# gbouritsas/GSN

Hardware: AMD Instinct MI355X
Metric: graphs/sec (orbit-count + GSN-e fwd), ZINC-shape batch; % HBM roofline (higher is better)
Workload: dtype int64 counts + f32 message passing (matrix products: fp16x3 -- two fp16 planes per fp32 operand, three plane products, f32 accumulate); 1 GPU; ZINC-shape x65536 graphs/GPU (N=1521515, E=3116498): integer atom / bond codes in -> cycle_graph k<=6 GSN-e (id_scope=local) orbit count (int64 identifiers written) + one-hot encoding (atoms, bonds and identifiers as exact fp16 operand rows: the layer kernel's input form; no fp32 one-hot tensor is materialised) + GSN_edge_sparse layer-0 forward (general, d_in=28, d_ef=4, d_id=12, d=128, bn, eval) ; inputs=int64 atom codes [N], bond codes [E], edge_index [2, E], graph pointers, outputs=int64 identifiers [E, 4], fp32 layer rows [N, 128], parallelism=graph-shard x1, no data-path collective

## Files before the change

gsn_amd/_abi.py:

```python
from __future__ import annotations

import ctypes
import os
import subprocess

_HERE = os.path.dirname(os.path.abspath(__file__))
LIB_PATH = os.environ.get("GSN_LIB_PATH") or os.path.join(_HERE, "lib", "libgsn_hip.so")
_lib = None

c_i64 = ctypes.c_int64
c_i32 = ctypes.c_int32
c_int = ctypes.c_int
c_vp = ctypes.c_void_p


class GsnError(RuntimeError):
    """A libgsn_hip.so entry point returned a negative status."""


class gsn_block(ctypes.Structure):
    _fields_ = [("data", c_vp), ("idx", c_vp), ("width", c_i64), ("idx32", c_vp)]


class gsn_chain_stage(ctypes.Structure):
    _fields_ = [("blocks", ctypes.POINTER(gsn_block)), ("n_blocks", c_int), ("W", c_vp), ("bias", c_vp), ("n_out", c_i64),
                ("bn_mean", c_vp), ("bn_scale", c_vp), ("bn_shift", c_vp), ("act", c_int)]


class gsn_self_block(ctypes.Structure):
    _fields_ = [("data", c_vp), ("width", c_i64), ("row_stride", c_i64)]


class gsn_pack16(ctypes.Structure):
    _fields_ = [("node_rows", c_vp), ("edge_rows", c_vp)]


class gsn_count_side(ctypes.Structure):
    _fields_ = [("csr_row", c_int), ("seg_ptr", c_vp), ("perm", c_vp), ("sorted_target", c_vp), ("sorted_other", c_vp),
                ("n_nodes", c_i64), ("n_edges", c_i64), ("node_codes", c_vp), ("node_code_cols", c_int), ("node_n_classes", c_int * 4),
                ("node_clamp", c_int), ("node_pack", c_vp), ("edge_codes", c_vp), ("edge_code_cols", c_int), ("edge_n_classes", c_int * 4),
                ("edge_clamp", c_int), ("edge_col0", c_int), ("code_status", c_vp)]


class gsn_count_keys(ctypes.Structure):
    _fields_ = [("nkey", c_vp), ("ekeys", c_vp), ("idmask", c_vp)]


class gsn_count_call(ctypes.Structure):
    _fields_ = [("plan_host", c_vp), ("plan_dev", c_vp), ("plan_words", c_i64), ("n_graphs", c_i64), ("node_ptr", c_vp), ("edge_ptr", c_vp),
                ("edge_index", c_vp), ("edge_row_stride", c_i64), ("ids_are_global", c_int), ("max_nodes", c_i64), ("max_edges", c_i64),
                ("out", c_vp), ("status", c_vp), ("n_classes", c_vp), ("clamp", c_int), ("pack", c_vp), ("pack_stride", c_i64),
                ("pack_col0", c_i64), ("side", ctypes.POINTER(gsn_count_side))]


class gsn_layer_pack16_call(ctypes.Structure):
    _fields_ = [("n_nodes", c_i64), ("n_edges", c_i64), ("seg_ptr", c_vp), ("edge", ctypes.POINTER(gsn_chain_stage)), ("x", c_vp), ("d_x", c_i64),
                ("node0", ctypes.POINTER(gsn_chain_stage)), ("node1", ctypes.POINTER(gsn_chain_stage)), ("prepared", c_vp),
                ("pack", ctypes.POINTER(gsn_pack16)), ("edge_rows", c_i64), ("out", c_vp)]


class gsn_code_slot(ctypes.Structure):
    _fields_ = [("codes", ctypes.c_void_p), ("idx", ctypes.c_void_p), ("stride", ctypes.c_int32), ("col", ctypes.c_int32),
                ("w_off", ctypes.c_int32), ("n_classes", ctypes.c_int32), ("clamp", ctypes.c_int32), ("reserved", ctypes.c_int32)]


class gsn_dgn_agg(ctypes.Structure):
    _fields_ = [("kind", c_i32), ("col", c_i32), ("alpha", ctypes.c_float), ("slot", c_i32)]


SIGNATURES = {
    "gsn_last_error": (ctypes.c_char_p, []),
    "gsn_propagate_last_route": (ctypes.c_char_p, []),
    "gsn_version": (c_int, []),
    "gsn_device_count": (c_int, []),
    "gsn_stream_capture_id": (c_i64, [c_vp]),
    "gsn_fingerprint_hip": (c_int, [c_int, c_vp, c_i64, c_vp, c_vp, c_vp]),
    "gsn_pattern_orbits": (c_int, [c_i64, c_vp, c_int, c_vp, c_vp, c_vp, c_vp, c_vp, c_vp, c_vp, c_vp]),
    "gsn_graph_vertex_orbits": (c_int, [c_i64, c_i64, c_vp, c_vp, c_vp]),
    "gsn_count_plan_build": (c_int, [c_int, c_int, c_int, c_i64, c_vp, c_vp, c_vp, c_i64, c_vp, c_vp]),
    "gsn_count_hip": (c_int, [c_vp, c_vp, c_i64, c_i64, c_vp, c_vp, c_vp, c_i64, c_int, c_vp, c_i64, c_i64, c_i64,
                              c_vp, c_vp, c_vp]),
    "gsn_count_sparse_hip": (c_int, [c_vp, c_vp, c_i64, c_i64, c_vp, c_vp, c_vp, c_i64, c_int, c_vp, c_i64, c_i64, c_i64,
                                     c_vp, c_vp, c_vp, c_i64, c_vp]),
    "gsn_count_sparse_workspace_bytes": (c_i64, [c_i64, c_i64, c_i64]),
    "gsn_count_encode_hip": (c_int, [c_vp, c_vp, c_i64, c_i64, c_vp, c_vp, c_vp, c_i64, c_int, c_vp, c_i64, c_i64, c_i64,
                                     c_vp, c_vp, c_vp, c_int, c_vp, c_vp]),
    "gsn_count_encode_pack16_hip": (c_int, [c_vp, c_vp, c_i64, c_i64, c_vp, c_vp, c_vp, c_i64, c_int, c_vp, c_i64, c_i64, c_i64,
                                            c_vp, c_vp, c_vp, c_int, c_vp, c_vp, c_i64, c_i64, c_vp]),
    "gsn_count_encode_pack16_side_hip": (c_int, [c_vp, c_vp, c_i64, c_i64, c_vp, c_vp, c_vp, c_i64, c_int, c_i64, c_i64, c_vp, c_vp, c_vp, c_int,
                                                 c_vp, c_i64, c_i64, ctypes.POINTER(gsn_count_side), c_vp]),
    "gsn_count_layer_step_hip": (c_int, [ctypes.POINTER(gsn_count_call), ctypes.POINTER(gsn_layer_pack16_call), c_vp, c_vp]),
    "gsn_count_encode_keys_side_hip": (c_int, [c_vp, c_vp, c_i64, c_i64, c_vp, c_vp, c_vp, c_i64, c_int, c_i64, c_i64, c_vp, c_vp, c_vp, c_int,
                                               c_i64, ctypes.POINTER(gsn_count_side), ctypes.POINTER(gsn_count_keys), c_vp]),
    "gsn_count_layer_step_keys_hip": (c_int, [ctypes.POINTER(gsn_count_call), ctypes.POINTER(gsn_layer_pack16_call), ctypes.POINTER(gsn_count_keys),
                                              c_vp, c_i64, c_vp, c_vp]),
    "gsn_layer_keys_byte_table": (c_int, [c_vp]),
    "gsn_pack16_rows_hip": (c_int, [c_vp, c_i64, c_i64, c_vp, c_i64, c_i64, c_i64, c_vp, c_vp]),
    "gsn_one_hot_pack16_hip": (c_int, [c_i64, c_int, c_vp, c_vp, c_int, c_vp, c_i64, c_i64, c_i64, c_vp, c_vp]),
    "gsn_csr_scratch_elems": (c_i64, [c_i64]),
    "gsn_csr_build_hip": (c_int, [c_i64, c_i64, c_vp, c_vp, c_vp, c_vp, c_vp, c_vp, c_vp, c_vp]),
    "gsn_linear_f16x3_kpad": (c_i64, [c_i64]),
    "gsn_linear_f16x3_mpad": (c_i64, [c_i64]),
    "gsn_linear_f16x3_scratch_bytes": (c_i64, [c_i64, c_i64]),
    "gsn_linear_f16x3_prepare_hip": (c_int, [c_vp, c_i64, c_i64, c_vp, c_vp, c_vp]),
    "gsn_linear_f16x3_prepare_strided_hip": (c_int, [c_vp, c_i64, c_i64, c_i64, c_i64, c_vp, c_vp, c_vp]),
    "gsn_linear_fwd_strided_hip": (c_int, [c_i64, c_int, ctypes.POINTER(gsn_block), c_vp, c_i64, c_i64, c_vp, c_i64, c_vp, c_vp, c_vp, c_int,
                                           c_vp, c_vp, c_vp]),
    "gsn_linear_splitk_plan": (c_int, [c_i64, c_i64, c_i64]),
    "gsn_linear_fwd_splitk_hip": (c_int, [c_i64, c_int, ctypes.POINTER(gsn_block), c_vp, c_i64, c_i64, c_vp, c_i64, c_vp, c_vp]),
    "gsn_linear_f16x3_fwd_hip": (c_int, [c_i64, c_int, c_vp, c_vp, c_vp, c_vp, c_i64, c_vp, c_vp, c_vp, c_int, c_vp, c_vp, c_vp]),
    "gsn_linear_f16x3_fwd_stats_hip": (c_int, [c_i64, c_int, c_vp, c_vp, c_vp, c_vp, c_i64, c_vp, c_vp, c_vp, c_vp]),
    "gsn_linear_f16x3_split_rows_hip": (c_int, [c_i64, c_int, c_vp, c_vp, c_vp]),
    "gsn_linear_f16x3_fwd_presplit_hip": (c_int, [c_i64, c_int, c_vp, c_vp, c_vp, c_vp, c_i64, c_vp, c_vp, c_vp, c_int, c_vp, c_vp, c_vp]),
    "gsn_wgrad_f16x3_hip": (c_int, [c_i64, c_i64, c_i64, c_vp, c_vp, c_vp, c_vp]),
    "gsn_linear_f16x3_fwd_stats_presplit_hip": (c_int, [c_i64, c_int, c_vp, c_vp, c_vp, c_vp, c_i64, c_vp, c_vp, c_vp, c_vp]),
    "gsn_bn_act_planes_hip": (c_int, [c_i64, c_i64, c_vp, c_vp, c_vp, c_vp, c_int, c_vp, c_vp, c_vp]),
    "gsn_edge_split_sum_hip": (c_int, [c_i64, c_i64, c_vp, c_vp, c_vp, c_vp, c_vp, c_i64, c_vp, c_i64, c_vp, c_i64, c_vp, c_i64, c_int, c_vp, c_vp]),
    "gsn_csr_build_graphs_hip": (c_int, [c_i64, c_vp, c_vp, c_i64, c_i64, c_i64, c_i64, c_vp, c_vp, c_vp, c_vp, c_vp, c_vp, c_vp, c_vp]),
    "gsn_segsum_prepare_hip": (c_int, [c_i64, c_i64, c_vp, c_vp, c_i64, c_vp, c_vp]),
    "gsn_segment_sum_rows_hip": (c_int, [c_i64, c_i64, c_vp, c_vp, c_vp, c_vp, c_vp, c_i64, c_i64, c_vp, c_vp]),
    "gsn_propagate_fwd_hip": (c_int, [c_int, c_i64, c_i64, c_vp, c_vp, c_vp, c_vp, c_vp, c_i64, c_vp, c_i64, c_int, c_vp,
                                      c_i64, c_vp, c_vp]),
    "gsn_propagate_bwd_hip": (c_int, [c_int, c_i64, c_i64, c_vp, c_vp, c_vp, c_vp, c_vp, c_i64, c_vp, c_i64, c_int,
                                      c_vp, c_i64, c_vp, c_vp, c_vp, c_vp, c_vp]),
    "gsn_propagate_self_fwd_hip": (c_int, [c_int, c_i64, c_i64, c_vp, c_vp, c_vp, c_vp, c_vp, c_i64, c_vp, c_i64, c_int, c_vp,
                                           c_i64, c_i64, c_i64, c_int, ctypes.POINTER(gsn_self_block), c_vp, c_vp, c_vp]),
    "gsn_add_gathered_hip": (c_int, [c_i64, c_i64, c_vp, c_vp, c_vp, c_i64, c_vp, c_vp]),
    "gsn_propagate_self_bwd_hip": (c_int, [c_int, c_i64, c_i64, c_vp, c_int, ctypes.POINTER(gsn_self_block), ctypes.POINTER(c_vp), c_vp, c_vp,
                                           c_vp, c_vp]),
    "gsn_propagate_pad_bwd_hip": (c_int, [c_int, c_i64, c_i64, c_vp, c_vp, c_vp, c_vp, c_vp, c_i64, c_vp, c_i64, c_int,
                                          c_vp, c_i64, c_i64, c_i64, c_vp, c_vp, c_vp, c_vp, c_vp]),
    "gsn_propagate_bwd_fold_self_hip": (c_int, [c_i64, c_i64, c_vp, c_vp, c_vp, c_vp, c_vp, c_i64, c_vp, c_i64, c_vp, c_i64, c_vp, c_vp, c_vp, c_vp,
                                                c_vp, c_vp, c_vp]),
    "gsn_linear_fwd_hip": (c_int, [c_i64, c_int, ctypes.POINTER(gsn_block), c_vp, c_vp, c_i64, c_vp, c_vp, c_vp, c_int,
                                   c_vp, c_vp, c_vp, c_vp]),
    "gsn_one_hot_hip": (c_int, [c_i64, c_int, c_vp, c_vp, c_int, c_vp, c_vp]),
    "gsn_column_range_hip": (c_int, [c_i64, c_int, c_vp, c_vp, c_vp, c_vp]),
    "gsn_column_ranks_hip": (c_int, [c_i64, c_int, c_vp, c_vp, c_vp, c_i64, c_vp, c_vp, c_vp, c_vp]),
    "gsn_unique_sort_scratch_bytes": (c_i64, [c_i64, c_i64]),
    "gsn_unique_sort_hip": (c_int, [c_i64, c_i64, c_vp, c_vp, c_vp, c_vp, c_vp, c_i64, c_vp]),
    "gsn_lookup_codes_hip": (c_int, [c_i64, c_i64, c_vp, c_vp, c_vp, c_int, c_vp, c_vp, c_vp, c_vp]),
    "gsn_embed_fwd_hip": (c_int, [c_i64, c_int, c_int, c_int, c_vp, c_vp, c_vp, c_vp, c_vp, c_vp]),
    "gsn_embed_bwd_hip": (c_int, [c_i64, c_int, c_int, c_int, c_vp, c_vp, c_vp, c_vp, c_vp]),
    "gsn_embed_bwd_flat_supported": (c_int, [c_i64, c_int, c_int, c_vp]),
    "gsn_embed_bwd_flat_hip": (c_int, [c_i64, c_int, c_int, c_int, c_vp, c_vp, c_vp, c_vp, c_vp, c_vp]),
    "gsn_code_stage_supported": (c_int, [c_int, c_i64, c_i64]),
    "gsn_code_stage_fwd_hip": (c_int, [c_i64, c_int, ctypes.POINTER(gsn_code_slot), c_vp, c_i64, c_vp, c_i64, c_vp, c_vp, c_vp,
                                       c_int, c_vp, c_vp, c_vp, c_vp, c_vp]),
    "gsn_bn_act_hip": (c_int, [c_i64, c_i64, c_vp, c_vp, c_vp, c_vp, c_int, c_vp, c_vp]),
    "gsn_bn_act_bwd_hip": (c_int, [c_i64, c_i64, c_vp, c_vp, c_vp, c_vp, c_vp, c_vp, c_int, c_int, c_vp, c_vp, c_vp, c_vp]),
    "gsn_fold_weights_fwd_hip": (c_int, [c_i64, c_i64, c_i64, c_i64, c_i64, c_vp, c_i64, c_vp, c_i64, c_vp, c_vp, c_vp]),
    "gsn_fold_weights_bwd_hip": (c_int, [c_i64, c_i64, c_i64, c_i64, c_vp, c_i64, c_vp, c_i64, c_vp, c_i64, c_vp, c_vp, c_vp, c_vp, c_vp]),
    "gsn_bn_act_bwd_from_h_hip": (c_int, [c_i64, c_i64, c_vp, c_vp, c_vp, c_vp, c_vp, c_vp, c_int, c_int, c_vp, c_vp, c_vp, c_vp]),
    "gsn_bn_act_bwd_planes_hip": (c_int, [c_i64, c_i64, c_vp, c_vp, c_vp, c_vp, c_vp, c_vp, c_int, c_int, c_vp, c_vp, c_vp, c_vp]),
    "gsn_wgrad_hip": (c_int, [c_i64, c_i64, c_vp, c_int, ctypes.POINTER(gsn_block), c_vp, c_vp]),
    "gsn_gather_cat_hip": (c_int, [c_i64, c_int, ctypes.POINTER(gsn_block), c_vp, c_vp]),
    "gsn_bn_finalize_hip": (c_int, [c_i64, c_i64, ctypes.c_double, ctypes.c_double, c_vp, c_vp, c_vp, c_vp, c_vp, c_vp, c_vp, c_vp, c_vp, c_vp]),
    "gsn_bn_finalize_act_hip": (c_int, [c_i64, c_i64, ctypes.c_double, ctypes.c_double, c_vp, c_vp, c_vp, c_vp, c_vp, c_vp, c_vp, c_vp, c_vp, c_vp,
                                        c_vp, c_int, c_vp, c_vp]),
    "gsn_bn_finalize_count_hip": (c_int, [c_i64, c_i64, ctypes.c_double, ctypes.c_double, c_vp, c_vp, c_vp, c_vp, c_vp, c_vp, c_vp, c_vp, c_vp, c_vp,
                                          c_vp]),
    "gsn_column_stats_hip": (c_int, [c_i64, c_i64, c_vp, c_vp, c_vp]),
    "gsn_mlp_chain_supported": (c_int, [c_int, ctypes.POINTER(gsn_chain_stage)]),
    "gsn_layer_fused_supported": (c_int, [ctypes.POINTER(gsn_chain_stage), c_i64, ctypes.POINTER(gsn_chain_stage), ctypes.POINTER(gsn_chain_stage)]),
    "gsn_layer_fused_prepared_bytes": (c_i64, [ctypes.POINTER(gsn_chain_stage), c_i64, ctypes.POINTER(gsn_chain_stage), ctypes.POINTER(gsn_chain_stage)]),
    "gsn_layer_fused_prepare_hip": (c_int, [ctypes.POINTER(gsn_chain_stage), c_i64, ctypes.POINTER(gsn_chain_stage), ctypes.POINTER(gsn_chain_stage),
                                            c_vp, c_vp]),
    "gsn_layer_fused_fwd_hip": (c_int, [c_i64, c_i64, c_vp, ctypes.POINTER(gsn_chain_stage), c_vp, c_i64, ctypes.POINTER(gsn_chain_stage),
                                        ctypes.POINTER(gsn_chain_stage), c_vp, c_vp, c_vp]),
    "gsn_layer_fused_pack16_supported": (c_int, [ctypes.POINTER(gsn_chain_stage), c_i64, ctypes.POINTER(gsn_chain_stage), ctypes.POINTER(gsn_chain_stage)]),
    "gsn_layer_fused_pack16_prepared_bytes": (c_i64, [ctypes.POINTER(gsn_chain_stage), c_i64, ctypes.POINTER(gsn_chain_stage), ctypes.POINTER(gsn_chain_stage)]),
    "gsn_layer_fused_pack16_prepare_hip": (c_int, [ctypes.POINTER(gsn_chain_stage), c_i64, ctypes.POINTER(gsn_chain_stage), ctypes.POINTER(gsn_chain_stage), c_vp, c_vp]),
    "gsn_layer_fused_fwd_pack16_hip": (c_int, [c_i64, c_i64, c_vp, ctypes.POINTER(gsn_chain_stage), c_vp, c_i64, ctypes.POINTER(gsn_chain_stage), ctypes.POINTER(gsn_chain_stage), c_vp, ctypes.POINTER(gsn_pack16), c_i64, c_vp, c_vp]),
    "gsn_layer_fused_workspace_bytes": (c_i64, [c_i64, ctypes.POINTER(gsn_chain_stage), c_i64, ctypes.POINTER(gsn_chain_stage), ctypes.POINTER(gsn_chain_stage)]),
    "gsn_layer_fused_fwd_ws_hip": (c_int, [c_i64, c_i64, c_vp, ctypes.POINTER(gsn_chain_stage), c_vp, c_i64, ctypes.POINTER(gsn_chain_stage),
                                           ctypes.POINTER(gsn_chain_stage), c_vp, c_vp, c_vp, c_i64, c_vp, c_vp, c_vp]),
    "gsn_layer_fused_graphs_supported": (c_int, [ctypes.POINTER(gsn_chain_stage), c_i64, ctypes.POINTER(gsn_chain_stage), ctypes.POINTER(gsn_chain_stage)]),
    "gsn_layer_fused_fwd_graphs_hip": (c_int, [c_i64, c_i64, c_vp, ctypes.POINTER(gsn_chain_stage), c_vp, c_i64, ctypes.POINTER(gsn_chain_stage),
                                               ctypes.POINTER(gsn_chain_stage), c_vp, c_i64, c_vp, c_i64, c_vp, c_vp]),
    "gsn_mlp_chain_fwd_hip": (c_int, [c_i64, c_int, ctypes.POINTER(gsn_chain_stage), c_vp, c_vp, c_vp, c_vp, c_vp]),
    "gsn_dgn_aggregate_fwd_hip": (c_int, [c_i64, c_i64, c_i64, c_vp, c_vp, c_vp, c_vp, c_vp, c_i64, c_i64, c_vp, c_i64, c_i64,
                                          ctypes.POINTER(gsn_dgn_agg), c_int, c_vp, c_int, ctypes.c_double, c_vp, c_vp]),
    "gsn_dgn_aggregate_bwd_hip": (c_int, [c_i64, c_i64, c_i64, c_vp, c_vp, c_vp, c_vp, c_vp, c_vp, c_vp, c_i64, c_i64, c_vp, c_i64,
                                          c_i64, ctypes.POINTER(gsn_dgn_agg), c_int, c_vp, c_int, ctypes.c_double, c_vp, c_vp, c_vp, c_vp]),
    "gsn_laplacian_eig_hip": (c_int, [c_i64, c_vp, c_vp, c_vp, c_i64, c_vp, c_i64, c_int, c_int, c_int, c_int, c_vp, c_vp, c_vp, c_vp, c_vp,
                                      c_i64, c_vp]),
    "gsn_laplacian_eig_scratch_floats": (c_i64, [c_int, c_i64]),
    "gsn_adam_step_hip": (c_int, [c_int, c_vp, c_i64, c_vp, c_int, c_vp, c_vp, c_vp, c_vp, c_vp, c_i64, c_vp]),
    "gsn_masked_loss_scratch_bytes": (c_i64, [c_int, c_i64, c_i64]),
    "gsn_masked_loss_fwd_hip": (c_int, [c_int, c_i64, c_i64, c_vp, c_vp, c_vp, c_vp, c_vp, c_i64, c_vp]),
    "gsn_masked_loss_bwd_hip": (c_int, [c_int, c_i64, c_i64, c_vp, c_vp, c_vp, c_vp, c_vp, c_vp]),
    "gsn_eval_accumulate_scratch_bytes": (c_i64, [c_int, c_i64, c_i64]),
    "gsn_eval_accumulate_hip": (c_int, [c_int, c_int, c_i64, c_i64, c_i64, c_vp, c_vp, c_i64, c_vp, c_vp, c_vp, c_vp, c_i64, c_vp, c_vp, c_i64, c_vp]),
    "gsn_rank_metrics_scratch_bytes": (c_i64, [c_i64, c_i64]),
    "gsn_rank_metrics_hip": (c_int, [c_i64, c_i64, c_vp, c_vp, c_vp, c_vp, c_vp, c_vp, c_i64, c_vp]),
}


def build(verbose: bool = False) -> str:
    cmd = ["make", "-C", os.path.join(_HERE, "csrc"), "-j8"]
    res = subprocess.run(cmd, stdout=subprocess.PIPE, stderr=subprocess.STDOUT, text=True)
    if res.returncode != 0:
        raise RuntimeError("building libgsn_hip.so failed:\n" + res.stdout)
    if verbose:
        print(res.stdout)
    return LIB_PATH


def lib():
    global _lib
    if _lib is None:
        if not os.path.exists(LIB_PATH):
            raise ImportError(
                "gsn_amd: %s not found. Build the HIP extension first (python -c 'import __graft_entry__ as g; "
                "g.build()' or make -C gsn_amd/csrc). There is no CPU fallback." % LIB_PATH)
        import torch
        handle = ctypes.CDLL(LIB_PATH)
        for name, (res, args) in SIGNATURES.items():
            fn = getattr(handle, name)
            fn.restype = res
            fn.argtypes = args
        if handle.gsn_version() != 1:
            raise ImportError("gsn_amd: libgsn_hip.so ABI version %d != 1" % handle.gsn_version())
        _lib = handle
    return _lib


def check(rc: int, what: str = "") -> None:
    if rc != 0:
        msg = lib().gsn_last_error()
        raise GsnError("%s failed (%d): %s" % (what or "libgsn_hip", rc, msg.decode() if msg else ""))


_GPU_SEEN = False


def require_gpu() -> None:
    global _GPU_SEEN
    if _GPU_SEEN:
        return
    import torch
    if not torch.cuda.is_available():
        raise RuntimeError("gsn_amd: no GPU visible to PyTorch-ROCm; the counting / message-passing kernels are "
                           "HIP-only (gfx950) and there is no CPU fallback.")
    _GPU_SEEN = True


def ptr(t) -> int:
    if t is None:
        return None
    if hasattr(t, "data_ptr"):
        return t.data_ptr()
    return t.ctypes.data


def current_stream() -> int:
    import torch
    return torch._C._cuda_getCurrentRawStream(torch._C._cuda_getDevice())


class _NullGuard:
    def __enter__(self):
        return self

    def __exit__(self, *exc):
        return False


_NULL_GUARD = _NullGuard()


def device_guard(device):
    import torch
    idx = device.index
    if idx is None or idx == torch._C._cuda_getDevice():
        return _NULL_GUARD
    return torch.cuda.device(device)
```

gsn_amd/_dense.py:

```python
from __future__ import annotations

import ctypes
import os

import torch

from . import _abi, flags
from ._caches import _note_cache
from ._runtime import _ACT_CODE, _MAX_BLOCKS, _f32c, _timed, _zeros



def _f16x3_weights(weight, w32):
    key = (weight._version, w32.data_ptr(), tuple(w32.shape))
    hit = getattr(weight, "_gsn_f16x3", None)
    if hit is not None and hit[0] == key:
        return hit[1], hit[2]
    n_out, k = w32.shape
    L = _abi.lib()
    kpad = int(L.gsn_linear_f16x3_kpad(k))
    planes = torch.empty(2 * n_out * kpad, dtype=torch.float16, device=w32.device)
    col_inv = torch.empty(n_out, dtype=torch.float32, device=w32.device)
    with _abi.device_guard(w32.device):
        if w32.is_contiguous():
            _abi.check(L.gsn_linear_f16x3_prepare_hip(w32.data_ptr(), n_out, k, planes.data_ptr(), col_inv.data_ptr(), _abi.current_stream()),
                       "gsn_linear_f16x3_prepare_hip")
        else:
            _abi.check(L.gsn_linear_f16x3_prepare_strided_hip(w32.data_ptr(), n_out, k, w32.stride(0), w32.stride(1), planes.data_ptr(), col_inv.data_ptr(),
                                                              _abi.current_stream()), "gsn_linear_f16x3_prepare_strided_hip")
    try:
        weight._gsn_f16x3 = (key, planes, col_inv)
        _note_cache(weight, "_gsn_f16x3")
    except (AttributeError, RuntimeError):
        pass
    return planes, col_inv


def _block_array(blocks, keep, widths_only=False):
    arr = (_abi.gsn_block * max(len(blocks), 1))()
    for b, (d, idx) in enumerate(blocks):
        arr[b].width = d.shape[1]
        if widths_only:
            arr[b].data = 1
            continue
        d = _f32c(d); keep.append(d)
        arr[b].data = d.data_ptr()
        arr[b].idx = None; arr[b].idx32 = None
        if idx is not None:
            idx = idx.contiguous(); keep.append(idx)
            if idx.dtype == torch.int32:
                arr[b].idx32 = idx.data_ptr()
            else:
                arr[b].idx = idx.data_ptr()
    keep.append(arr)
    return arr


def _f16x3_takes(m_rows, n_out, widths, aligned=True, direct=True, out=True, stats=False, bn=False, act=0):
    return (flags.LINEAR_F16X3 and out and (not stats or (flags.LINEAR_F16X3_STATS and not bn and act == 0 and n_out % 4 == 0))
            and m_rows > 0 and n_out > flags.LINEAR_F16X3_MIN_N and ((m_rows + 127) // 128) * ((n_out + 127) // 128) > flags.LINEAR_F16X3_MIN_TILES
            and direct and aligned and all(w % 4 == 0 for w in widths))


def _linear_hip(blocks, weight, bias, bn_mean, bn_scale, bn_shift, act, m_rows, out=True, stats=None, split_k=False, scratch_out=None, presplit=None):
    if len(blocks) > _MAX_BLOCKS:
        raise NotImplementedError("more than %d input blocks" % _MAX_BLOCKS)
    dev = weight.device
    keep = []
    arr = _block_array(blocks, keep)
    n_out = weight.shape[0]
    y = torch.empty((m_rows, n_out), dtype=torch.float32, device=dev) if out else None
    if m_rows == 0:
        return y
    w_view = (weight.dim() == 2 and weight.dtype is torch.float32 and not weight.is_contiguous() and weight.stride(0) == 1
              and weight.stride(1) >= weight.shape[0] and flags.STRIDED_WEIGHTS)
    w = (weight.detach() if weight.requires_grad else weight) if w_view else _f32c(weight)
    vecs = [None if v is None else _f32c(v) for v in (bias, bn_mean, bn_scale, bn_shift)]
    nb = len(blocks)
    takes16 = _f16x3_takes(m_rows, n_out, [d.shape[1] for d, _ in blocks], aligned=all((arr[i].data or 0) % 16 == 0 for i in range(nb)),
                           direct=all(idx is None for _, idx in blocks), out=out, stats=stats is not None, bn=bn_mean is not None, act=act)
    if presplit is not None and not takes16:
        raise RuntimeError("presplit rows given to a product that does not run on the fp16x3 kernel (_f16x3_takes decides)")
    if takes16:
        planes, col_inv = _f16x3_weights(weight, w)
        scratch = presplit if presplit is not None else torch.empty(int(_abi.lib().gsn_linear_f16x3_scratch_bytes(m_rows, w.shape[1])), dtype=torch.uint8, device=dev)
        name = "gsn_linear_f16x3_fwd%s%s_hip" % ("_stats" if stats is not None else "", "_presplit" if presplit is not None else "")
        epilogue = () if stats is not None else (_abi.ptr(vecs[1]), _abi.ptr(vecs[2]), _abi.ptr(vecs[3]), act)
        tail = () if stats is None else (stats.data_ptr(),)
        with _abi.device_guard(dev), _timed("linear_fwd", 2.0 * m_rows * w.shape[1] * n_out):
            rc = getattr(_abi.lib(), name)(m_rows, nb, arr, planes.data_ptr(), col_inv.data_ptr(), _abi.ptr(vecs[0]), n_out, *epilogue,
                                           scratch.data_ptr(), y.data_ptr(), *tail, _abi.current_stream())
        _abi.check(rc, name)
        if scratch_out is not None:
            scratch_out.append(scratch)
        return y
    if split_k and out and stats is None and act == 0 and bn_mean is None and bn_scale is None and flags.LINEAR_SPLITK:
        splits = int(_abi.lib().gsn_linear_splitk_plan(m_rows, w.shape[1], n_out))
        if splits > 1:
            y = _zeros(m_rows * n_out, torch.float32, dev).view(m_rows, n_out)
            with _abi.device_guard(dev), _timed("linear_fwd", 2.0 * m_rows * w.shape[1] * n_out):
                rc = _abi.lib().gsn_linear_fwd_splitk_hip(m_rows, len(blocks), arr, w.data_ptr(), w.stride(0) if w_view else 0, w.stride(1) if w_view else 0,
                                                          _abi.ptr(vecs[0]), n_out, y.data_ptr(), _abi.current_stream())
            _abi.check(rc, "gsn_linear_fwd_splitk_hip")
            return y
    if w_view:
        with _abi.device_guard(dev), _timed("linear_fwd", 2.0 * m_rows * w.shape[1] * n_out):
            rc = _abi.lib().gsn_linear_fwd_strided_hip(m_rows, len(blocks), arr, w.data_ptr(), w.stride(0), w.stride(1), _abi.ptr(vecs[0]), n_out,
                                                       _abi.ptr(vecs[1]), _abi.ptr(vecs[2]), _abi.ptr(vecs[3]), act, _abi.ptr(y), _abi.ptr(stats),
                                                       _abi.current_stream())
        if rc != -2:
            _abi.check(rc, "gsn_linear_fwd_strided_hip")
            return y
        w = w.contiguous()
    with _abi.device_guard(dev), _timed("linear_fwd", 2.0 * m_rows * w.shape[1] * n_out):
        rc = _abi.lib().gsn_linear_fwd_hip(m_rows, len(blocks), arr, w.data_ptr(), _abi.ptr(vecs[0]), n_out, _abi.ptr(vecs[1]),
                                           _abi.ptr(vecs[2]), _abi.ptr(vecs[3]), act, None, _abi.ptr(y), _abi.ptr(stats),
                                           _abi.current_stream())
    _abi.check(rc, "gsn_linear_fwd_hip")
    return y


class _Stage:
    __slots__ = ("blocks", "weight", "bias", "bn", "act", "bn_params", "bn_invstd")

    def __init__(self, weight, bias, bn=None, act="identity", blocks=()):
        self.blocks, self.weight, self.bias, self.bn, self.act = list(blocks), weight, bias, bn, act
        self.bn_params = None
        self.bn_invstd = None


def _launch_stages(stages, m_rows, stats=None, csr=None):
    L = _abi.lib()
    dev = stages[0].weight.device
    if m_rows == 0:
        n_last = stages[-1].weight.shape[0]
        if csr is not None:
            return torch.zeros((csr.seg_ptr.numel() - 1, n_last), dtype=torch.float32, device=dev)
        return torch.empty((0, n_last), dtype=torch.float32, device=dev) if stats is None else None
    y = None
    i = 0
    while i < len(stages):
        group = None
        for n in (2, 1):
            cand = stages[i:i + n]
            if len(cand) < n:
                continue
            carry = [(y, None)] if y is not None else []
            arr = (_abi.gsn_chain_stage * n)()
            keep = []
            for j, st in enumerate(cand):
                arr[j] = _stage_struct(st, st.blocks + carry if j == 0 else st.blocks, keep)
            if L.gsn_mlp_chain_supported(n, arr):
                group = (n, arr, keep, cand)
                break
        last_group = group is not None and i + group[0] == len(stages)
        if csr is not None and not (last_group and i == 0):
            return None
        if group is not None:
            n, arr, keep, cand = group
            want_stats = stats is not None and last_group
            n_out = cand[-1].weight.shape[0]
            seg = csr is not None and not want_stats
            if seg:
                n_seg = csr.seg_ptr.numel() - 1
                out = torch.empty((n_seg, n_out), dtype=torch.float32, device=dev)
                with _abi.device_guard(dev), _timed("segsum_prepare"):
                    _abi.check(L.gsn_segsum_prepare_hip(n_seg, m_rows, csr.seg_ptr.data_ptr(), csr.tgt.data_ptr(), n_out,
                                                        out.data_ptr(), _abi.current_stream()), "gsn_segsum_prepare_hip")
            else:
                out = None if want_stats else torch.empty((m_rows, n_out), dtype=torch.float32, device=dev)
            flops = sum(2.0 * m_rows * st.weight.shape[1] * st.weight.shape[0] for st in cand)
            with _abi.device_guard(dev), _timed("mlp_chain%d" % n, flops):
                rc = L.gsn_mlp_chain_fwd_hip(m_rows, n, arr, None,
                                             csr.tgt.data_ptr() if seg else None, _abi.ptr(out),
                                             _abi.ptr(stats) if want_stats else None, _abi.current_stream())
            _abi.check(rc, "gsn_mlp_chain_fwd_hip")
            y = out
            i += n
        else:
            st = stages[i]
            blks = st.blocks + ([(y, None)] if y is not None else [])
            last = i == len(stages) - 1
            bp = st.bn_params or (None, None, None)
            if last and stats is not None:
                _linear_hip(blks, st.weight, st.bias, None, None, None, 0, m_rows, out=False, stats=stats)
                y = None
            else:
                y = _linear_hip(blks, st.weight, st.bias, bp[0], bp[1], bp[2], _ACT_CODE[st.act], m_rows)
            i += 1
    return y


def _chain_fits(stages):
    n = len(stages)
    if n < 1 or n > 2:
        return False
    arr = (_abi.gsn_chain_stage * n)()
    keep = []
    for j, st in enumerate(stages):
        arr[j].blocks = _block_array(st.blocks, keep, widths_only=True); arr[j].n_blocks = len(st.blocks)
        arr[j].W = 1; arr[j].n_out = st.weight.shape[0]; arr[j].act = _ACT_CODE[st.act]
    return bool(_abi.lib().gsn_mlp_chain_supported(n, arr))


def _stage_struct(st, blocks, keep, rows_keep=None):
    g = _abi.gsn_chain_stage()
    g.blocks = _block_array(blocks, keep if rows_keep is None else rows_keep); g.n_blocks = len(blocks)
    w = _f32c(st.weight); keep.append(w)
    g.W = w.data_ptr(); g.n_out = w.shape[0]
    vecs = [None if v is None else _f32c(v) for v in ((st.bias,) + (st.bn_params or (None, None, None)))]
    keep.extend(vecs)
    g.bias, g.bn_mean, g.bn_scale, g.bn_shift = [_abi.ptr(v) for v in vecs]
    g.act = _ACT_CODE[st.act]
    return g


def _prep_key(st):
    bn = st.bn
    bk = None
    if bn is not None:
        bk = (bn.running_mean._version, bn.running_var._version, bn.running_mean.data_ptr(),
              (bn.weight._version, bn.bias._version) if bn.affine else None)
    return (st.weight.data_ptr(), st.weight._version, tuple(st.weight.shape), bk)


def _prepared(kind, ge, g0, g1, d_x, dev, owner=None, attr=None, key=None):
    hit = getattr(owner, attr, None) if owner is not None else None
    if hit is not None and hit[0] == key:
        return hit[1]
    L = _abi.lib()
    nbytes = int(getattr(L, "gsn_layer_fused%s_prepared_bytes" % kind)(ctypes.byref(ge), d_x, ctypes.byref(g0), ctypes.byref(g1)))
    prep = torch.empty(nbytes // 4, dtype=torch.int32, device=dev)
    name = "gsn_layer_fused%s_prepare_hip" % kind
    with _abi.device_guard(dev):
        _abi.check(getattr(L, name)(ctypes.byref(ge), d_x, ctypes.byref(g0), ctypes.byref(g1), prep.data_ptr(), _abi.current_stream()), name)
    if owner is not None:
        setattr(owner, attr, (key, prep))
        _note_cache(owner, attr)
    return prep


def _layer_fused(x, csr, edge_stages, node_stages, training, owner=None, gen=0, pack16=None, pack_only=False, record=None):
    if not flags.FUSED_LAYER or len(edge_stages) != 1 or len(node_stages) != 2:
        return None
    stages = edge_stages + node_stages
    for st in stages:
        if st.act not in ("identity", "relu"):
            return None
        if st.bn is not None and (training or st.bn.training or st.bn.running_mean is None):
            return None
    if x.data_ptr() % 16:
        return None
    if len(node_stages[0].blocks) != 1 or node_stages[1].blocks:
        return None
    for st in stages:
        _bn_resolve(st, None, 0, False)
    keep, rows = [], []
    eb = edge_stages[0].blocks
    ge = _stage_struct(edge_stages[0], eb, keep, rows)
    g0 = _stage_struct(node_stages[0], [], keep)
    g1 = _stage_struct(node_stages[1], [], keep)
    d_x = x.shape[1]
    if node_stages[0].weight.shape[1] != d_x + edge_stages[0].weight.shape[0] + 4:
        return None
    L = _abi.lib()
    fl = (2.0 * edge_stages[0].weight.shape[1] * edge_stages[0].weight.shape[0],
          2.0 * (node_stages[0].weight.shape[1] * node_stages[0].weight.shape[0] + node_stages[1].weight.shape[1] * node_stages[1].weight.shape[0]))
    pkey = (tuple(_prep_key(st) for st in stages), d_x, gen)
    if pack16 is not None and flags.PACK16_LAYER and L.gsn_layer_fused_pack16_supported(ctypes.byref(ge), d_x, ctypes.byref(g0), ctypes.byref(g1)):
        prep = _prepared("_pack16", ge, g0, g1, d_x, x.device, owner, "_fused_prep16", pkey + ("pack16",))
        launch16 = _pack16_launch(ge, g0, g1, d_x, prep, fl, keep)
        out = launch16(x.data_ptr(), x.shape[0], x.device, csr, [idx for _, idx in eb], pack16)
        if out is not None:
            if record is not None and owner is not None and all(idx is not None and idx.dtype == torch.int32 for _, idx in eb):
                owner._fplan = (record, "pack16", launch16)
                _note_cache(owner, "_fplan")
            return out
    if pack_only:
        return None
    if not L.gsn_layer_fused_supported(ctypes.byref(ge), d_x, ctypes.byref(g0), ctypes.byref(g1)):
        return None
    nbytes = int(L.gsn_layer_fused_prepared_bytes(ctypes.byref(ge), d_x, ctypes.byref(g0), ctypes.byref(g1)))
    prep = _prepared("", ge, g0, g1, d_x, x.device, owner, "_fused_prep", pkey + (nbytes,))
    if (flags.GRAPH_ALIGNED_LAYER and getattr(csr, "part", None) is not None and d_x == 128
            and L.gsn_layer_fused_graphs_supported(ctypes.byref(ge), d_x, ctypes.byref(g0), ctypes.byref(g1))):
        launch_g = _graphs_launch(ge, g0, g1, d_x, prep, fl, keep)
        out = launch_g(x, csr, eb)
        if out is not None:
            if (record is not None and owner is not None
                    and all(idx is not None and idx.dtype == torch.int32 and d.dtype == torch.float32 and d.is_contiguous() for d, idx in eb)):
                owner._fplan = (record, "graphs", launch_g)
                _note_cache(owner, "_fplan")
            return out
    return _rows_forward(x, csr, ge, g0, g1, d_x, prep, fl)


def _pack16_launch(ge, g0, g1, d_x, prep, fl, keep):
    L = _abi.lib()
    n_out = g1.n_out
    pk = _abi.gsn_pack16()

    def launch16(x_ptr, n_rows, dev, csr_now, idx_now, pack_now):
        for i in range(ge.n_blocks):
            ge.blocks[i].data = x_ptr if i < 2 else pack_now[1].data_ptr()
            ge.blocks[i].idx32 = idx_now[i].data_ptr()
        y = torch.empty((n_rows, n_out), dtype=torch.float32, device=dev)
        pk.node_rows = pack_now[0].data_ptr()
        pk.edge_rows = None if pack_now[1] is None else pack_now[1].data_ptr()
        e_now = csr_now.tgt.numel()
        with _abi.device_guard(dev), _timed("layer_fused", fl[0] * e_now + fl[1] * n_rows):
            rc16 = L.gsn_layer_fused_fwd_pack16_hip(n_rows, e_now, csr_now.seg_ptr.data_ptr(), ctypes.byref(ge), x_ptr, d_x, ctypes.byref(g0), ctypes.byref(g1),
                                                    prep.data_ptr(), ctypes.byref(pk), 0 if pack_now[1] is None else pack_now[1].shape[0], y.data_ptr(),
                                                    _abi.current_stream())
        if rc16 == -2:
            return None
        _abi.check(rc16, "gsn_layer_fused_fwd_pack16_hip")
        return y
    launch16._keep = keep
    return launch16


def _graphs_launch(ge, g0, g1, d_x, prep, fl, keep):
    L = _abi.lib()
    n_out = g1.n_out

    def launch_g(x_now, csr_now, blocks_now, y=None):
        part_now = getattr(csr_now, "part", None)
        if part_now is None or part_now[2] > 128 or int(part_now[0].numel()) <= 1 or x_now.data_ptr() % 16:
            return None
        for i in range(ge.n_blocks):
            d_i, idx_i = blocks_now[i]
            ge.blocks[i].data = d_i.data_ptr()
            ge.blocks[i].idx = None
            ge.blocks[i].idx32 = idx_i.data_ptr()
        n_now, e_now = x_now.shape[0], csr_now.tgt.numel()
        if y is None:
            y = torch.empty((n_now, n_out), dtype=torch.float32, device=x_now.device)
        with _abi.device_guard(x_now.device), _timed("layer_fused", fl[0] * e_now + fl[1] * n_now):
            rcg = L.gsn_layer_fused_fwd_graphs_hip(n_now, e_now, csr_now.seg_ptr.data_ptr(), ctypes.byref(ge), x_now.data_ptr(), d_x, ctypes.byref(g0),
                                                   ctypes.byref(g1), prep.data_ptr(), int(part_now[0].numel()) - 1, part_now[0].data_ptr(), int(part_now[2]),
                                                   y.data_ptr(), _abi.current_stream())
        if rcg == -2:
            return None
        _abi.check(rcg, "gsn_layer_fused_fwd_graphs_hip")
        return y
    launch_g._keep = keep
    return launch_g


def _rows_forward(x, csr, ge, g0, g1, d_x, prep, fl):
    L = _abi.lib()
    n, E = x.shape[0], csr.tgt.numel()
    out = torch.empty((n, g1.n_out), dtype=torch.float32, device=x.device)
    x_exp = None
    hit = getattr(x, "_gsn_row_exp", None)
    if hit is not None and hit[1] == x._version and hit[0].numel() == n and hit[0].device == x.device and not flags.VALIDATE_CACHES:
        x_exp = hit[0]
    out_exp = torch.empty(n, dtype=torch.int32, device=x.device) if d_x == 128 and out.shape[1] == 128 and flags.CHAIN_ROW_EXPONENTS else None
    ws_bytes = 0 if x_exp is not None else int(L.gsn_layer_fused_workspace_bytes(n, ctypes.byref(ge), d_x, ctypes.byref(g0), ctypes.byref(g1)))
    ws = torch.empty(ws_bytes // 4, dtype=torch.int32, device=x.device) if ws_bytes else None
    with _abi.device_guard(x.device), _timed("layer_fused", fl[0] * E + fl[1] * n):
        rc = L.gsn_layer_fused_fwd_ws_hip(n, E, csr.seg_ptr.data_ptr(), ctypes.byref(ge), x.data_ptr(), d_x, ctypes.byref(g0),
                                          ctypes.byref(g1), prep.data_ptr(), out.data_ptr(), _abi.ptr(ws), ws_bytes, _abi.ptr(x_exp),
                                          _abi.ptr(out_exp), _abi.current_stream())
    if rc == 0 and out_exp is not None:
        out._gsn_row_exp = (out_exp, out._version)
    if rc == -2:
        if os.environ.get("GSN_CHAIN_TRACE"):
            import sys
            msg = L.gsn_last_error()
            print("gsn chain: one-launch layer declined: %s" % (msg.decode() if msg else ""), file=sys.stderr)
        return None
    _abi.check(rc, "gsn_layer_fused_fwd_hip")
    return out


def _bn_resolve(stage, stats_fn, m_rows, training, fuse_act=None):
    bn = stage.bn
    if bn is None:
        stage.bn_params = None
        return
    if training or bn.running_mean is None:
        if training and m_rows == 1:
            raise ValueError("Expected more than 1 value per channel when training, got input size torch.Size([%d, %d])" % (m_rows, bn.num_features))
        if m_rows == 0:
            n_out, dev = bn.num_features, stage.weight.device
            if training and bn.track_running_stats and bn.num_batches_tracked is not None:
                bn.num_batches_tracked += 1
                if flags.RAW_WRITTEN is not None:
                    flags.RAW_WRITTEN.append(bn.num_batches_tracked)
            vec = torch.zeros((4, n_out), dtype=torch.float32, device=dev)
            vec[1:3] = 1.0
            stage.bn_params = (vec[0], vec[2], vec[3])
            stage.bn_invstd = vec[1]
            return
        stats = stats_fn()
        n_out = stats.shape[1]
        dev = stats.device
        vec = torch.empty((4, n_out), dtype=torch.float32, device=dev)
        track = training and bn.track_running_stats and bn.running_mean is not None
        mom = 0.0
        nbt = None
        if track:
            if bn.momentum is not None and bn.num_batches_tracked.is_cuda and bn.num_batches_tracked.dtype == torch.int64:
                mom, nbt = bn.momentum, bn.num_batches_tracked
            else:
                bn.num_batches_tracked += 1
                mom = bn.momentum if bn.momentum is not None else 1.0 / float(bn.num_batches_tracked)
        gamma = _f32c(bn.weight) if bn.affine else None
        beta = _f32c(bn.bias) if bn.affine else None
        v0, v1, v2, v3 = vec.unbind(0)
        p0 = vec.data_ptr()
        with _abi.device_guard(dev):
            if fuse_act is not None:
                fh, fact, fout = fuse_act
                rc = _abi.lib().gsn_bn_finalize_act_hip(n_out, m_rows, float(bn.eps), float(mom), stats.data_ptr(), _abi.ptr(gamma), _abi.ptr(beta),
                                                        bn.running_mean.data_ptr() if track else None, bn.running_var.data_ptr() if track else None,
                                                        p0, p0 + 4 * n_out, p0 + 8 * n_out, p0 + 12 * n_out, _abi.ptr(nbt),
                                                        fh.data_ptr(), int(fact), fout.data_ptr(), _abi.current_stream())
            else:
                rc = _abi.lib().gsn_bn_finalize_count_hip(n_out, m_rows, float(bn.eps), float(mom), stats.data_ptr(), _abi.ptr(gamma), _abi.ptr(beta),
                                                          bn.running_mean.data_ptr() if track else None, bn.running_var.data_ptr() if track else None,
                                                          p0, p0 + 4 * n_out, p0 + 8 * n_out, p0 + 12 * n_out,
                                                          _abi.ptr(nbt), _abi.current_stream())
        _abi.check(rc, "gsn_bn_finalize_act_hip" if fuse_act is not None else "gsn_bn_finalize_count_hip")
        if track:
            touched = [bn.running_mean, bn.running_var] + ([nbt] if nbt is not None else [])
            torch.autograd.graph.increment_version(touched)
            if flags.RAW_WRITTEN is not None:
                flags.RAW_WRITTEN.extend(touched)
        stage.bn_params = (v0, v2, v3)
        stage.bn_invstd = v1
        return
    else:
        key = (bn.running_mean._version, bn.running_var._version, bn.running_mean.data_ptr(), bn.running_var.data_ptr(),
               (bn.weight._version, bn.bias._version, bn.weight.data_ptr(), bn.bias.data_ptr()) if bn.affine else None)
        hit = getattr(bn, "_gsn_eval_cache", None)
        if hit is not None and hit[0] == key:
            stage.bn_params = hit[1]
            stage.bn_invstd = hit[2]
            return
        mean32 = bn.running_mean
        invstd = torch.rsqrt(bn.running_var.to(torch.float64) + bn.eps).to(torch.float32)
        scale = invstd * bn.weight.detach() if bn.affine else invstd
        shift = bn.bias.detach() if bn.affine else torch.zeros_like(invstd)
        stage.bn_params = (mean32.contiguous(), scale.contiguous(), shift.contiguous())
        stage.bn_invstd = invstd.contiguous()
        bn._gsn_eval_cache = (key, stage.bn_params, stage.bn_invstd)
        _note_cache(bn, "_gsn_eval_cache")


def run_stages(stages, m_rows, training, csr=None):
    if csr is not None and not _chain_fits(stages):
        return None
    needs_stats = any(st.bn is not None and (training or st.bn.running_mean is None) for st in stages)
    if csr is None and needs_stats and not _chain_fits(stages):
        return _run_stages_materialised(stages, m_rows, training)
    for i, st in enumerate(stages):
        if st.bn is not None:
            def stats_fn(i=i):
                n_out = stages[i].weight.shape[0]
                stats = _zeros(2 * n_out, torch.float64, stages[i].weight.device).view(2, n_out)
                probe = _Stage(stages[i].weight, stages[i].bias, None, "identity", stages[i].blocks)
                _launch_stages(stages[:i] + [probe], m_rows, stats=stats)
                return stats
            _bn_resolve(st, stats_fn, m_rows, training)
    return _launch_stages(stages, m_rows, csr=csr)


def _bn_act_hip(h, bn_params, act):
    vecs = [None if v is None else _f32c(v) for v in (bn_params or (None, None, None))]
    with _abi.device_guard(h.device), _timed("bn_act", 8.0 * h.numel()):
        rc = _abi.lib().gsn_bn_act_hip(h.shape[0], h.shape[1], h.data_ptr(), _abi.ptr(vecs[0]), _abi.ptr(vecs[1]), _abi.ptr(vecs[2]),
                                       _ACT_CODE[act], h.data_ptr(), _abi.current_stream())
    _abi.check(rc, "gsn_bn_act_hip")
    return h


def _run_stages_materialised(stages, m_rows, training):
    y = None
    for st in stages:
        blks = st.blocks + ([(y, None)] if y is not None else [])
        if st.bn is not None and (training or st.bn.running_mean is None):
            n_out = st.weight.shape[0]
            stats = _zeros(2 * n_out, torch.float64, st.weight.device).view(2, n_out)
            h = _linear_hip(blks, st.weight, st.bias, None, None, None, 0, m_rows, out=True, stats=stats)
            _bn_resolve(st, lambda: stats, m_rows, training)
            y = _bn_act_hip(h, st.bn_params, st.act)
        else:
            _bn_resolve(st, None, m_rows, training)
            bp = st.bn_params or (None, None, None)
            y = _linear_hip(blks, st.weight, st.bias, bp[0], bp[1], bp[2], _ACT_CODE[st.act], m_rows)
    return y
```

gsn_amd/csrc/abi.cpp:

```cpp
#include <hip/hip_runtime.h>

#include <cstring>

#include "gsn_internal.h"
#include "layer_rr.h"

namespace gsn {

static thread_local char g_err[512] = "";

int set_error(int code, const char *fmt, ...) {
    va_list ap;
    va_start(ap, fmt);
    vsnprintf(g_err, sizeof(g_err), fmt, ap);
    va_end(ap);
    return code;
}

}

extern "C" const char *gsn_last_error(void) { return gsn::g_err; }

extern "C" int gsn_version(void) { return GSN_ABI_VERSION; }

extern "C" int gsn_device_count(void) {
    int n = 0;
    if (hipGetDeviceCount(&n) != hipSuccess) {
        (void)hipGetLastError();
        return 0;
    }
    int good = 0;
    for (int i = 0; i < n; ++i) {
        hipDeviceProp_t p;
        if (hipGetDeviceProperties(&p, i) == hipSuccess && std::strncmp(p.gcnArchName, "gfx950", 6) == 0) ++good;
    }
    return good;
}

extern "C" int64_t gsn_stream_capture_id(void *stream) {
    hipStreamCaptureStatus st = hipStreamCaptureStatusNone;
    unsigned long long id = 0;
    if (hipStreamGetCaptureInfo(reinterpret_cast<hipStream_t>(stream), &st, &id) != hipSuccess) {
        (void)hipGetLastError();
        return 0;
    }
    if (st == hipStreamCaptureStatusNone) return 0;
    return (int64_t)(id ? id : 1);
}

namespace gsn {
int current_device() {
    int dev = -1;
    if (hipGetDevice(&dev) != hipSuccess) return -1;
    return dev;
}

int lds_limit(DeviceOnce *once, std::initializer_list<const void *> kernels, const char *label, int bytes) {
    const int dev = once ? current_device() : -1;
    if (once && once->done(dev)) return GSN_OK;
    char sized[32];
    if (!label) { snprintf(sized, sizeof(sized), "%d B LDS", bytes); label = sized; }
    for (const void *k : kernels) {
        const hipError_t e = hipFuncSetAttribute(k, hipFuncAttributeMaxDynamicSharedMemorySize, bytes);
        if (e != hipSuccess) return set_error(GSN_E_HIP, "hipFuncSetAttribute(%s): %s", label, hipGetErrorString(e));
    }
    if (once) once->mark(dev);
    return GSN_OK;
}

int launch_check(const char *label_fmt, ...) {
    const hipError_t e = hipGetLastError();
    if (e == hipSuccess) return GSN_OK;
    char label[256];
    va_list ap;
    va_start(ap, label_fmt);
    vsnprintf(label, sizeof(label), label_fmt, ap);
    va_end(ap);
    return set_error(GSN_E_HIP, "%s: %s", label, hipGetErrorString(e));
}

void trace(const char *fmt, ...) {
    if (!sw_present(SW_CHAIN_TRACE)) return;
    va_list ap;
    va_start(ap, fmt);
    vfprintf(stderr, fmt, ap);
    va_end(ap);
}

ProfCounters::ProfCounters(size_t n, void *stream) {
    n_ = n;
    if (n == 0 || hipMalloc(&dev_, n * sizeof(unsigned long long)) != hipSuccess) { dev_ = nullptr; return; }
    (void)hipMemsetAsync(dev_, 0, n * sizeof(unsigned long long), reinterpret_cast<hipStream_t>(stream));
}
ProfCounters::~ProfCounters() { if (dev_) (void)hipFree(dev_); }
std::vector<unsigned long long> ProfCounters::fetch(void *stream) {
    std::vector<unsigned long long> h(n_, 0ull);
    (void)hipStreamSynchronize(reinterpret_cast<hipStream_t>(stream));
    if (dev_) {
        (void)hipMemcpy(h.data(), dev_, n_ * sizeof(unsigned long long), hipMemcpyDeviceToHost);
        (void)hipFree(dev_);
        dev_ = nullptr;
    }
    return h;
}
}

extern "C" int gsn_count_layer_step_hip(const gsn_count_call *c, const gsn_layer_pack16_call *l, void *event_between, void *stream) {
    if (!c || !l) return gsn::set_error(GSN_E_INVALID, "gsn_count_layer_step_hip: null call struct");
    const int rc = gsn_count_encode_pack16_side_hip(c->plan_host, c->plan_dev, c->plan_words, c->n_graphs, c->node_ptr, c->edge_ptr, c->edge_index,
                                                    c->edge_row_stride, c->ids_are_global, c->max_nodes, c->max_edges, c->out, c->status, c->n_classes,
                                                    c->clamp, c->pack, c->pack_stride, c->pack_col0, c->side, stream);
    if (rc != GSN_OK) return rc;
    if (event_between && hipEventRecord(reinterpret_cast<hipEvent_t>(event_between), reinterpret_cast<hipStream_t>(stream)) != hipSuccess)
        return gsn::set_error(GSN_E_HIP, "gsn_count_layer_step_hip: hipEventRecord(event_between)");
    return gsn_layer_fused_fwd_pack16_hip(l->n_nodes, l->n_edges, l->seg_ptr, l->edge, l->x, l->d_x, l->node0, l->node1, l->prepared, l->pack,
                                          l->edge_rows, l->out, stream);
}

extern "C" int gsn_count_layer_step_keys_hip(const gsn_count_call *c, const gsn_layer_pack16_call *l, const gsn_count_keys *keys, const uint16_t *node_dict,
                                             int64_t dict_rows, void *event_between, void *stream) {
    if (!c || !l || !keys || !c->side) return gsn::set_error(GSN_E_INVALID, "gsn_count_layer_step_keys_hip: null call struct / keys / side");
    if (!keys->nkey || !keys->ekeys || !keys->idmask || !node_dict) return gsn::set_error(GSN_E_INVALID, "gsn_count_layer_step_keys_hip: null key array / node dictionary");
    if (!c->side->node_codes || !c->side->edge_codes) return gsn::set_error(GSN_E_INVALID, "gsn_count_layer_step_keys_hip: node and edge codes are both needed");
    if (!gsn_layer_fused_pack16_supported(l->edge, l->d_x, l->node0, l->node1))
        return gsn::set_error(GSN_E_UNSUPPORTED, "gsn_count_layer_step_keys_hip: shape outside the packed-row layer kernel");
    if (!l->seg_ptr || !l->out || !l->prepared || (reinterpret_cast<uintptr_t>(l->prepared) & 15) || l->n_nodes <= 0 || l->n_nodes > (int64_t)2000000000 ||
        l->n_edges > (int64_t)2000000000)
        return gsn::set_error(GSN_E_INVALID, "gsn_count_layer_step_keys_hip: null seg_ptr / out / prepared (16-byte aligned), or sizes outside 32-bit row arithmetic");
    if (l->edge->n_blocks < 3 || l->edge->blocks[0].idx32 != c->side->sorted_target || l->edge->blocks[1].idx32 != c->side->sorted_other ||
        l->edge->blocks[2].idx32 != c->side->perm || l->seg_ptr != c->side->seg_ptr || l->n_edges != c->side->n_edges || l->n_nodes != c->side->n_nodes)
        return gsn::set_error(GSN_E_INVALID, "gsn_count_layer_step_keys_hip: the layer's seg_ptr / block indices must be the counting launch's CSR arrays");
    int rc = gsn_count_encode_keys_side_hip(c->plan_host, c->plan_dev, c->plan_words, c->n_graphs, c->node_ptr, c->edge_ptr, c->edge_index, c->edge_row_stride,
                                            c->ids_are_global, c->max_nodes, c->max_edges, c->out, c->status, c->n_classes, c->clamp, c->pack_col0, c->side, keys, stream);
    if (rc != GSN_OK) return rc;
    if (event_between && hipEventRecord(reinterpret_cast<hipEvent_t>(event_between), reinterpret_cast<hipStream_t>(stream)) != hipSuccess)
        return gsn::set_error(GSN_E_HIP, "gsn_count_layer_step_keys_hip: hipEventRecord(event_between)");
    const gsn::RpKeys k{keys->ekeys, keys->nkey, keys->idmask, node_dict, dict_rows, c->side->edge_col0};
    rc = gsn::rp_forward(l->n_nodes, l->n_edges, l->seg_ptr, l->edge, l->x, l->d_x, l->node0, l->node1, l->prepared, nullptr, l->edge_rows, l->out,
                         reinterpret_cast<hipStream_t>(stream), &k);
    if (rc == 1) return gsn::set_error(GSN_E_UNSUPPORTED, "gsn_count_layer_step_keys_hip: key arrays beyond 2 GiB (32-bit buffer offsets)");
    return rc;
}
```

gsn_amd/csrc/layer_rp.hip:

```cpp
#include <hip/hip_runtime.h>

#include <cstdint>
#include <cstdio>
#include <cstdlib>
#include <type_traits>
#include <vector>

#include "chain_common.h"
#include "layer_rr.h"
#include "layer_rr_inl.h"
#include "layer_rr_core.h"

namespace gsn {

struct RpArgs {
    int n_nodes, n_edges;
    const int32_t *seg_ptr;
    const int32_t *role_idx[3];
    const uint16_t *node16, *edge16;
    unsigned node_bytes, edge_bytes;
    int edge_shift;
    int d_x;
    float *out;
    const unsigned *prep;
    int n_ranges;
    int n_split;
    const uint32_t *ekeys;
    const uint8_t *nkey;
    int edge_col0;
};

struct RpIdx { int r[3]; int pt, pt1; int nk; };

template <bool KEYS>
__device__ __forceinline__ void rp_idx_load(const RpArgs &a, const RrDesc &d, int li, RpIdx &ix) {
    const int ne = d.ne();
    if (d.valid() && ne > 0) {
        const int e = d.e0 + (li < ne ? li : ne - 1);
        if constexpr (KEYS) {
            ix.r[0] = (int)a.ekeys[e];
            ix.r[2] = a.role_idx[2][e];
        } else {
#pragma unroll
            for (int q = 0; q < 3; ++q) ix.r[q] = a.role_idx[q][e];
        }
    }
    if (d.valid()) {
        int t = d.m0 + li;
        t = t < a.n_nodes ? t : a.n_nodes - 1;
        ix.pt = a.seg_ptr[t];
        ix.pt1 = a.seg_ptr[t + 1];
        if constexpr (KEYS) ix.nk = (int)a.nkey[t];
    }
}

constexpr int RP_BYTE_TAB_BYTES = 256 * 16;
__device__ __host__ __forceinline__ unsigned rp_byte_tab_word(unsigned b, int q) {
    return ((b >> (2 * q)) & 1u ? 0x3c00u : 0u) | ((b >> (2 * q + 1)) & 1u ? 0x3c000000u : 0u);
}

#define RP_LOAD(RS, VOFF, IMM) __builtin_bit_cast(rr_u4, __builtin_amdgcn_raw_buffer_load_b128(RS, (int)((VOFF) + (IMM)), 0, 0))

__device__ __forceinline__ unsigned rp_scale_pair(unsigned pair, float s) {
    unsigned r;
    asm("v_fma_mixlo_f16 %0, %1, %2, 0 op_sel_hi:[1,0,0]" : "=v"(r) : "v"(pair), "v"(s));
    asm("v_fma_mixhi_f16 %0, %1, %2, 0 op_sel:[1,0,0] op_sel_hi:[1,0,0]" : "+v"(r) : "v"(pair), "v"(s));
    return r;
}
__device__ __forceinline__ unsigned rp_hi_lo_word(float a, float s) {
    unsigned r;
    asm("v_fma_mixlo_f16 %0, %1, %2, 0" : "=v"(r) : "v"(a), "v"(s));
    asm("v_fma_mixhi_f16 %0, %1, %2, -%0 op_sel_hi:[0,0,1]" : "+v"(r) : "v"(a), "v"(s));
    return r;
}
__device__ __forceinline__ unsigned rp_pk_max_u16(unsigned a, unsigned b) { unsigned r; asm("v_pk_max_u16 %0, %1, %2" : "=v"(r) : "v"(a), "v"(b)); return r; }

#ifndef RP_GATHER_AT
#define RP_GATHER_AT 3
#endif
#ifndef RP_STORE_AUX
#define RP_STORE_AUX 2
#endif
#ifndef RP_PD
#define RP_PD 8
#endif
#ifndef RP_STAGGER
#define RP_STAGGER 0
#endif
#ifndef RP_S1T
#define RP_S1T 0
#endif
#ifndef RP_DRAIN
#define RP_DRAIN 0
#endif
#ifndef RP_S1E
#define RP_S1E 1
#endif

template <int WB, int NKX, bool PROF, bool KEYS = false>
__global__ __launch_bounds__(64 * RR_NW) __attribute__((amdgpu_waves_per_eu(RR_NW / 4, RR_NW / 4))) void layer_fused_kernel_rp(RpArgs a, unsigned long long *prof) {
    auto clk = [&]() -> unsigned {
        if (!PROF) return 0u;
        __builtin_amdgcn_sched_barrier(0);
        const unsigned v = (unsigned)__builtin_amdgcn_s_memtime();
        __builtin_amdgcn_sched_barrier(0);
        return v;
    };
    unsigned pc[8] = {0, 0, 0, 0, 0, 0, 0, 0};
    using SH = RrShape<WB, NKX>;
    constexpr int NKS = SH::NKS, NK0 = SH::NK0;
    static_assert(WB == 4 && NKX == 2, "two pairs of feature blocks; the node pack is two chunks wide");
    extern __shared__ __attribute__((aligned(16))) unsigned char smem[];

    const int tid = threadIdx.x;
    const int lane0 = tid & 63, wave = __builtin_amdgcn_readfirstlane(tid >> 6);
    const int li0 = lane0 & 31, lh0 = lane0 >> 5;
    unsigned ldsb[3];
    ldsb[0] = (unsigned)(uintptr_t)(__attribute__((address_space(3))) unsigned char *)smem + 16u * (unsigned)lane0;
    ldsb[1] = ldsb[0] + 0x10000u; ldsb[2] = ldsb[0] + 0x20000u;
    asm volatile("" : "+v"(ldsb[1]), "+v"(ldsb[2]));

    {
        const rr_u4 *src = reinterpret_cast<const rr_u4 *>(a.prep + RR_HDR);
        rr_u4 *dst = reinterpret_cast<rr_u4 *>(smem);
        for (int i = tid; i < SH::F_LDS * 64; i += 64 * RR_NW) dst[i] = src[i];
        const float *tsrc = reinterpret_cast<const float *>(a.prep + RR_HDR + SH::F_ALL * 256);
        float *tdst = reinterpret_cast<float *>(smem + SH::F_LDS * 1024);
        for (int i = tid; i < SH::TAB_WORDS; i += 64 * RR_NW) tdst[i] = tsrc[i];
        if constexpr (KEYS) {
            rr_u4 *bt = reinterpret_cast<rr_u4 *>(smem + SH::LDS_BYTES);
            for (int b = tid; b < 256; b += 64 * RR_NW) bt[b] = rr_u4{rp_byte_tab_word(b, 0), rp_byte_tab_word(b, 1), rp_byte_tab_word(b, 2), rp_byte_tab_word(b, 3)};
        }
    }
    __syncthreads();
    auto hdr = [&](int i) { return (int)__builtin_amdgcn_readfirstlane(a.prep[i]); };
    const int Ee = hdr(RRH_EE), E0 = hdr(RRH_E0), E1 = hdr(RRH_E1), e_min = hdr(RRH_EMIN);
    const bool w_bad = hdr(RRH_BAD) != 0;
    if (a.prep[RRH_PACK] != 1u) __builtin_trap();
    const unsigned acts = (unsigned)hdr(RRH_ACT);
    const int lo_e = __builtin_amdgcn_readfirstlane((acts & 1) ? 0 : (int)0x80000000), lo_0 = __builtin_amdgcn_readfirstlane((acts & 2) ? 0 : (int)0x80000000);
    const int lo_1 = __builtin_amdgcn_readfirstlane((acts & 4) ? 0 : (int)0x80000000);
    const __amdgpu_buffer_rsrc_t wstream = __builtin_amdgcn_make_buffer_rsrc(const_cast<unsigned *>(a.prep) + RR_HDR + SH::F_W0SL * 256, 0, NKS * WB * 1024, 0x00020000);
    const __amdgpu_buffer_rsrc_t rs_n = __builtin_amdgcn_make_buffer_rsrc(const_cast<uint16_t *>(a.node16), 0, (int)a.node_bytes, 0x00020000);
    const __amdgpu_buffer_rsrc_t rs_e = __builtin_amdgcn_make_buffer_rsrc(const_cast<uint16_t *>(a.edge16), 0, (int)a.edge_bytes, 0x00020000);
    const int esh = a.edge_shift;
    int sbase[8];
#pragma unroll
    for (int k = 0; k < 8; ++k) { sbase[k] = 4096 * k; asm volatile("" : "+s"(sbase[k])); }
    const int ec0 = a.edge_col0;
    const int deg_c = a.d_x >> 4, deg_h = (a.d_x >> 3) & 1, deg_w = (a.d_x >> 1) & 3;

    const int range = wave * (int)gridDim.x + (int)blockIdx.x;
    if (range >= a.n_ranges) return;
    const unsigned long long wave_t0 = PROF ? __builtin_amdgcn_s_memrealtime() : 0ull;
#if RP_STAGGER > 0
    if (wave >= RR_NW / 2) {
#pragma unroll 1
        for (int i = 0; i < RP_STAGGER; ++i) __builtin_amdgcn_s_sleep(64);
    }
#endif
    RrIter it;
    it.seg = a.seg_ptr; it.n_nodes = a.n_nodes;
    {
        const int half_n = a.n_ranges >> 1;
        if (a.n_split > 0 && half_n > 0 && (a.n_ranges & 1) == 0 && (int)gridDim.x * (RR_NW / 2) == half_n) {
            const int young = wave >= RR_NW / 2 ? 1 : 0;
            const int idx = range - young * half_n;
            const int64_t base = young ? a.n_split : 0, cnt = young ? a.n_nodes - a.n_split : a.n_split;
            it.m_next = (int)(base + cnt * idx / half_n);
            it.m_end = (int)(base + cnt * (idx + 1) / half_n);
        } else {
            it.m_next = (int)((int64_t)a.n_nodes * range / a.n_ranges);
            it.m_end = (int)((int64_t)a.n_nodes * (range + 1) / a.n_ranges);
        }
    }
    it.m0 = 0; it.nn = 0; it.eb = 0; it.ee = 0; it.ec = 0; it.pending = 0; it.win = 0;
    rr_iter_load(it, lane0);
    RrDesc cur = rr_iter_next(it, lane0);
    RpIdx ixc, ixn;
#pragma unroll
    for (int q = 0; q < 3; ++q) { ixc.r[q] = 0; ixn.r[q] = 0; }
    ixc.pt = ixc.pt1 = ixn.pt = ixn.pt1 = 0;
    ixc.nk = ixn.nk = 0;
    rp_idx_load<KEYS>(a, cur, li0, ixc);
    RrDesc nxt = rr_iter_next(it, lane0);
    rp_idx_load<KEYS>(a, nxt, li0, ixn);
    rr_u4 gA[RR_NKE], gB[RR_NKE];
    auto gather = [&](rr_u4 (&g)[RR_NKE], const int (&r)[3], int lh) {
        if constexpr (KEYS) {
            const unsigned k = (unsigned)r[0];
            const unsigned vt = ((k & 0xffu) << 6) | ((unsigned)lh << 4), vs = (((k >> 8) & 0xffu) << 6) | ((unsigned)lh << 4);
            g[0] = RP_LOAD(rs_n, vt, 0); g[1] = RP_LOAD(rs_n, vt, 32);
            g[2] = RP_LOAD(rs_n, vs, 0); g[3] = RP_LOAD(rs_n, vs, 32);
            g[4][0] = (unsigned)__builtin_amdgcn_raw_buffer_load_b16(rs_e, (int)((unsigned)r[2] << 1), 0, 0);
        } else {
        const unsigned vt = ((unsigned)r[0] << 6) | ((unsigned)lh << 4), vs = ((unsigned)r[1] << 6) | ((unsigned)lh << 4);
        const unsigned ve = ((unsigned)r[2] << esh) | ((unsigned)lh << 4);
        g[0] = RP_LOAD(rs_n, vt, 0); g[1] = RP_LOAD(rs_n, vt, 32);
        g[2] = RP_LOAD(rs_n, vs, 0); g[3] = RP_LOAD(rs_n, vs, 32);
        g[4] = RP_LOAD(rs_e, ve, 0);
        }
    };
    gather(gA, ixc.r, lh0);
    int pt = ixc.pt, pt1 = ixc.pt1;
    int nk = ixc.nk;
    unsigned kc = (unsigned)ixc.r[0];

    const unsigned t_start = clk();
    while (cur.valid()) {
        asm volatile("" : "+v"(ldsb[0]), "+v"(ldsb[1]), "+v"(ldsb[2]));
        int li = li0, lh = lh0;
        asm volatile("" : "+v"(li), "+v"(lh));
        const int lane = li + 32 * lh;
        const float *tab = reinterpret_cast<const float *>(rr_lds_generic(ldsb[0] - 16u * (unsigned)lane + SH::F_LDS * 1024));
        const int m0 = cur.m0, nn = cur.nn();
        rr_u4 X[NKX];
        auto load_x = [&]() {
            const unsigned vx = ((unsigned)(KEYS ? nk : m0 + (li < nn ? li : nn - 1)) << 6) | ((unsigned)lh << 4);
#pragma unroll
            for (int c = 0; c < NKX; ++c) X[c] = RP_LOAD(rs_n, vx, 32 * c);
        };
        f32x16 sacc[WB];
        int tpt = 0, tpt1 = 0;
        int rnext[3] = {0, 0, 0};
        auto block = [&](auto first_c, rr_u4 (&gc)[RR_NKE], rr_u4 (&gn)[RR_NKE]) __attribute__((always_inline)) -> bool {
            constexpr bool FIRST = decltype(first_c)::value;
            const unsigned t0 = clk();
            const int ne = cur.ne();
            if (li >= nn) { pt = 0; pt1 = 0; }
            tpt = pt; tpt1 = pt1;
            rr_u4 Ah[RR_NKE];
#pragma unroll
            for (int c = 0; c < RR_NKE; ++c) Ah[c] = gc[c];
            if constexpr (KEYS) {
                const unsigned m16 = gc[RR_NKE - 1][0] | ((kc >> 16) << ec0);
                const unsigned byte = (m16 >> (8 * lh)) & 0xffu;
                Ah[RR_NKE - 1] = *reinterpret_cast<rr_ldsp>(ldsb[2] - 16u * (unsigned)lane + 16u * byte + (unsigned)(SH::LDS_BYTES - 0x20000));
            }
            const bool last = cur.last() != 0;
            if (!last) gather(gn, ixn.r, lh);
#pragma unroll
            for (int q = 0; q < 3; ++q) rnext[q] = ixn.r[q];
            kc = (unsigned)ixn.r[0];
            const int npt = ixn.pt, npt1 = ixn.pt1, nnk = ixn.nk;
            const RrDesc nn2 = rr_iter_next(it, lane);
            rp_idx_load<KEYS>(a, nn2, li, ixn);
            const unsigned t1 = clk();
            unsigned t2 = t1;
            if (!FIRST || ne > 0) {
                const unsigned bm = rr_edge_mask(pt, pt1, cur.e0);
                rr_u4 M[2];
                rr_incidence(bm, lh, M);
                auto frag4 = [&](int fp, int c, rr_u4 &h0, rr_u4 &l0, rr_u4 &h1, rr_u4 &l1) {
                    h0 = rr_lds_frag(ldsb, SH::F_WE + 2 * (fp * RR_NKE + c)); l0 = rr_lds_frag(ldsb, SH::F_WE + 2 * (fp * RR_NKE + c) + 1);
                    h1 = rr_lds_frag(ldsb, SH::F_WE + 2 * ((fp + 1) * RR_NKE + c)); l1 = rr_lds_frag(ldsb, SH::F_WE + 2 * ((fp + 1) * RR_NKE + c) + 1);
                };
                auto ep_half = [&](const f32x16 &acc, int h, unsigned (&yh)[8], unsigned (&yl)[8]) {
#pragma unroll
                    for (int q = 0; q < 2; ++q) {
                        const int r = 8 * h + 4 * q;
                        rr_split4(rr_imax(acc[r], lo_e), rr_imax(acc[r + 1], lo_e), rr_imax(acc[r + 2], lo_e), rr_imax(acc[r + 3], lo_e),
                                  yh[4 * h + 2 * q], yl[4 * h + 2 * q], yh[4 * h + 2 * q + 1], yl[4 * h + 2 * q + 1]);
                    }
                };
                auto incid = [&](f32x16 &sv, const unsigned (&yh)[8], const unsigned (&yl)[8], const rr_u4 (&MM)[2], int h) {
                    const rr_u4 pl = rr_u4{yl[4 * h], yl[4 * h + 1], yl[4 * h + 2], yl[4 * h + 3]};
                    const rr_u4 ph = rr_u4{yh[4 * h], yh[4 * h + 1], yh[4 * h + 2], yh[4 * h + 3]};
                    if (FIRST && h == 0) {
                        f32x16 z;
#pragma unroll
                        for (int r = 0; r < 16; ++r) z[r] = 0.f;
                        RR_MFH(pl, MM[h], z);
                        sv = z;
                    } else {
                        RR_MFH(pl, MM[h], sv);
                    }
                    RR_MFH(ph, MM[h], sv);
                };
                unsigned yh0[8], yl0[8], yh1[8], yl1[8];
                auto ep_step = [&](int c, const f32x16 &A0, const f32x16 &A1, f32x16 &S0, f32x16 &S1, const rr_u4 (&MM)[2]) {
                    if (c == 0) ep_half(A0, 0, yh0, yl0);
                    if (c == 1) { ep_half(A0, 1, yh0, yl0); incid(S0, yh0, yl0, MM, 0); }
                    if (c == 2) { ep_half(A1, 0, yh1, yl1); incid(S0, yh0, yl0, MM, 1); }
                    if (c == 3) { ep_half(A1, 1, yh1, yl1); incid(S1, yh1, yl1, MM, 0); }
                    if (c == 4) incid(S1, yh1, yl1, MM, 1);
                };
                auto products = [&](int fp, f32x16 &acc0, f32x16 &acc1, auto &&under) {
#pragma unroll
                    for (int r = 0; r < 16; ++r) { acc0[r] = 0.f; acc1[r] = 0.f; }
                    rr_u4 f0h, f0l, f1h, f1l;
                    frag4(fp, 0, f0h, f0l, f1h, f1l);
#pragma unroll
                    for (int c = 0; c < RR_NKE; ++c) {
                        rr_u4 n0h = f0h, n0l = f0l, n1h = f1h, n1l = f1l;
                        if (c + 1 < RR_NKE) frag4(fp, c + 1, n0h, n0l, n1h, n1l);
                        RR_MFH(Ah[c], f0l, acc0);
                        RR_MFH(Ah[c], f1l, acc1);
                        under(c);
                        RR_MFH(Ah[c], f0h, acc0);
                        RR_MFH(Ah[c], f1h, acc1);
                        RR_SB();
                        f0h = n0h; f0l = n0l; f1h = n1h; f1l = n1l;
                    }
                };
                f32x16 qa0, qa1, ra0, ra1;
                products(0, qa0, qa1, [&](int) {});
                products(2, ra0, ra1, [&](int c) { ep_step(c, qa0, qa1, sacc[0], sacc[1], M); });
                t2 = clk();
                load_x();
#pragma unroll
                for (int c = 0; c < RR_NKE; ++c) ep_step(c, ra0, ra1, sacc[2], sacc[3], M);
                RR_SB();
            } else {
#pragma unroll
                for (int fb = 0; fb < WB; ++fb)
#pragma unroll
                    for (int r = 0; r < 16; ++r) sacc[fb][r] = 0.f;
                load_x();
            }
            const unsigned t3 = clk();
            if (PROF) { pc[0] += t1 - t0; pc[1] += t2 - t1; pc[2] += t3 - t2; pc[6] += 1; }
            cur = nxt; nxt = nn2;
            pt = npt; pt1 = npt1; nk = nnk;
            return last;
        };
        {
            bool last = block(std::true_type{}, gA, gB);
#pragma unroll 1
            while (!last) {
                last = block(std::false_type{}, gB, gA);
                if (!last) last = block(std::false_type{}, gA, gB);
            }
        }
#pragma unroll
        for (int c = 0; c < NKX; ++c) asm volatile("" : "+v"(X[c]));
        const unsigned t3 = clk();
        f32x16 hacc[WB];
        float ms = 0.f;
#pragma unroll
        for (int fb = 0; fb < WB; ++fb)
#pragma unroll
            for (int r = 0; r < 16; r += 2) ms = fmaxf(fmaxf(fabsf(sacc[fb][r]), fabsf(sacc[fb][r + 1])), ms);
        X[NKX - 1][3] = lh ? X[NKX - 1][3] & 0xffffu : X[NKX - 1][3];
        unsigned m16 = 0;
#pragma unroll
        for (int c = 0; c < NKX; ++c)
#pragma unroll
            for (int q = 0; q < 4; ++q) m16 = rp_pk_max_u16(m16, X[c][q] & 0x7fff7fffu);
        m16 = max(m16 & 0xffffu, m16 >> 16);
        const unsigned fld_x = m16 ? (m16 >> 10) + 112u : 0u;
        const float degf = (float)(tpt1 - tpt);
        const unsigned msb = __float_as_uint(ms);
        int es = (int)(msb >> 23) - 1 - Ee;
        es = msb == 0 ? 0 : es;
        unsigned fld = (unsigned)max(max(es, (int)max(fld_x, __float_as_uint(degf) >> 23)), 0);
        fld = rr_xhalf_max(fld);
        bool badrow = msb >= 0x7f800000u || m16 >= 0x7c00u || w_bad;
        badrow = rr_xhalf_or(badrow ? 1u : 0u) != 0;
        int e_t = (int)fld;
        e_t = e_t < e_min ? e_min : (e_t > 254 ? 254 : e_t);
        const float rs = __uint_as_float((unsigned)(268 - e_t) << 23);
        float fs = rr_pow2(267 - e_t - Ee);
        const float sc = rr_pow2(E0 + 268 - e_t);
        if (badrow) fs = __uint_as_float(0x7fc00000u);
        rr_u4 Xh[NKX];
#pragma unroll
        for (int c = 0; c < NKX; ++c)
#pragma unroll
            for (int q = 0; q < 4; ++q) Xh[c][q] = rp_scale_pair(X[c][q], rs);
        {
            const unsigned dw = rp_hi_lo_word(degf, rs);
#pragma unroll
            for (int c = 0; c < NKX; ++c)
#pragma unroll
                for (int q = 0; q < 4; q += 2) Xh[c][q] = (c == deg_c && q == deg_w && lh == deg_h) ? dw : Xh[c][q];
        }
        {
            const rr_f2 sc2 = rr_f2{sc, sc};
#pragma unroll
            for (int fbo = 0; fbo < WB; ++fbo)
#pragma unroll
                for (int i = 0; i < 4; ++i) {
                    const float4 cv = *reinterpret_cast<const float4 *>(tab + 32 * WB + 32 * fbo + 8 * i + 4 * lh);
                    const rr_f2 p0 = rr_f2{cv.x, cv.y} * sc2, p1 = rr_f2{cv.z, cv.w} * sc2;
                    hacc[fbo][4 * i] = p0[0]; hacc[fbo][4 * i + 1] = p0[1]; hacc[fbo][4 * i + 2] = p1[0]; hacc[fbo][4 * i + 3] = p1[1];
                }
        }
        {
            auto fr = [&](int i, rr_u4 &h0, rr_u4 &l0, rr_u4 &h1, rr_u4 &l1) {
                const int cq = i / (WB / 2), fa = 2 * (i % (WB / 2));
                h0 = rr_lds_frag(ldsb, SH::F_W0H + fa * NK0 + NKS + cq); l0 = rr_lds_frag(ldsb, SH::F_W0XL + fa * NKX + cq);
                h1 = rr_lds_frag(ldsb, SH::F_W0H + (fa + 1) * NK0 + NKS + cq); l1 = rr_lds_frag(ldsb, SH::F_W0XL + (fa + 1) * NKX + cq);
            };
            rr_u4 a0h, a0l, a1h, a1l;
            fr(0, a0h, a0l, a1h, a1l);
#pragma unroll
            for (int i = 0; i < NKX * (WB / 2); ++i) {
                const int cq = i / (WB / 2), fa = 2 * (i % (WB / 2));
                rr_u4 n0h = a0h, n0l = a0l, n1h = a1h, n1l = a1l;
                if (i + 1 < NKX * (WB / 2)) fr(i + 1, n0h, n0l, n1h, n1l);
                RR_MFH(a0l, Xh[cq], hacc[fa]);
                RR_MFH(a1l, Xh[cq], hacc[fa + 1]);
                RR_MFH(a0h, Xh[cq], hacc[fa]);
                RR_MFH(a1h, Xh[cq], hacc[fa + 1]);
                RR_SB();
                a0h = n0h; a0l = n0l; a1h = n1h; a1l = n1l;
            }
        }
#ifdef RR_ABL_NOSTREAM
#define RP_STREAM(I) rr_u4{(unsigned)(I), (unsigned)lane, 0x3c003c00u, 0u}
#elif defined(RR_ABL_STREAM1)
#define RP_STREAM(I) __builtin_bit_cast(rr_u4, __builtin_amdgcn_raw_buffer_load_b128(wstream, 16 * lane, ((I) & 1) * 1024, 0))
#else
#define RP_STREAM(I) __builtin_bit_cast(rr_u4, __builtin_amdgcn_raw_buffer_load_b128(wstream, 16 * lane + ((I) & 3) * 1024, sbase[(I) >> 2], 0))
#endif
        constexpr int PD = RP_PD, NSL = NKS * WB;
        static_assert(PD % 2 == 0, "the stream is consumed two fragments per step");
        float m2 = 0.f;
        {
            rr_u4 ql[PD];
#pragma unroll
            for (int i = 0; i < PD; ++i) ql[i] = RP_STREAM(i);
            unsigned ph[NKS][4], pl[NKS][4];
            auto ssplit = [&](int c) {
                const int fb = c >> 1, cc = c & 1;
#pragma unroll
                for (int q = 0; q < 2; ++q)
                    rr_split4s(sacc[fb][8 * cc + 4 * q], sacc[fb][8 * cc + 4 * q + 1], sacc[fb][8 * cc + 4 * q + 2], sacc[fb][8 * cc + 4 * q + 3], fs,
                               ph[c][2 * q], pl[c][2 * q], ph[c][2 * q + 1], pl[c][2 * q + 1]);
            };
            ssplit(0);
#pragma unroll
            for (int pass = 0; pass < WB / 2; ++pass) {
                const int fa = 2 * pass;
                rr_u4 a0h = rr_lds_frag(ldsb, SH::F_W0H + fa * NK0), a1h = rr_lds_frag(ldsb, SH::F_W0H + (fa + 1) * NK0);
#pragma unroll
                for (int c = 0; c < NKS; ++c) {
                    const int i = pass * 2 * NKS + 2 * c;
                    const rr_u4 bh = rr_u4{ph[c][0], ph[c][1], ph[c][2], ph[c][3]}, bl = rr_u4{pl[c][0], pl[c][1], pl[c][2], pl[c][3]};
                    rr_u4 n0h = a0h, n1h = a1h;
                    if (c + 1 < NKS) { n0h = rr_lds_frag(ldsb, SH::F_W0H + fa * NK0 + c + 1); n1h = rr_lds_frag(ldsb, SH::F_W0H + (fa + 1) * NK0 + c + 1); }
                    const rr_u4 a0l = ql[i % PD], a1l = ql[(i + 1) % PD];
                    RR_MFH(a0h, bl, hacc[fa]);
                    RR_MFH(a1h, bl, hacc[fa + 1]);
                    RR_MFH(a0l, bh, hacc[fa]);
                    RR_MFH(a1l, bh, hacc[fa + 1]);
                    RR_MFH(a0h, bh, hacc[fa]);
                    RR_MFH(a1h, bh, hacc[fa + 1]);
                    if (i + PD < NSL) {
                        ql[i % PD] = RP_STREAM(i + PD);
                        ql[(i + 1) % PD] = RP_STREAM(i + 1 + PD);
                    }
                    if (pass == 0 && c + 1 < NKS) ssplit(c + 1);
                    if (pass > 0) {
#pragma unroll
                        for (int u = 0; u < 2; ++u)
#pragma unroll
                            for (int r = 2 * c; r < 2 * c + 2; ++r) {
                                hacc[fa - 2 + u][r] = rr_imax(hacc[fa - 2 + u][r], lo_0);
                            }
                        m2 = fmaxf(fmaxf(fabsf(hacc[fa - 2][2 * c]), fabsf(hacc[fa - 2][2 * c + 1])), m2);
                        m2 = fmaxf(fmaxf(fabsf(hacc[fa - 1][2 * c]), fabsf(hacc[fa - 1][2 * c + 1])), m2);
                    }
                    RR_SB();
                    a0h = n0h; a1h = n1h;
                }
            }
        }
        const unsigned t4 = clk();
#pragma unroll
        for (int fbo = WB - 2; fbo < WB; ++fbo)
#pragma unroll
            for (int r = 0; r < 16; ++r) hacc[fbo][r] = rr_imax(hacc[fbo][r], lo_0);
#pragma unroll
        for (int fbo = WB - 2; fbo < WB; ++fbo)
#pragma unroll
            for (int r = 0; r < 16; r += 2) m2 = fmaxf(fmaxf(fabsf(hacc[fbo][r]), fabsf(hacc[fbo][r + 1])), m2);
        const unsigned m2b = rr_xhalf_max(__float_as_uint(m2));
        int e2 = (int)(m2b >> 23) + (e_t - 141 - E0);
        e2 = e2 < 15 ? 15 : (e2 > 254 ? 254 : e2);
        float f2 = rr_pow2(e_t - e2 - E0 + 127);
        float inv2 = rr_pow2(e2 - 14 - E1);
        if (m2b >= 0x7f800000u || badrow) { f2 = __uint_as_float(0x7fc00000u); inv2 = f2; badrow = true; }
        const bool anybad = __builtin_amdgcn_ballot_w64(badrow) != 0ull;
        rr_u4 Hh[NKS], Hl[NKS];
        auto hsplit = [&](int c) {
            const int fbo = c >> 1, cc = c & 1;
            unsigned h[4], l[4];
#pragma unroll
            for (int q = 0; q < 2; ++q)
                rr_split4s(hacc[fbo][8 * cc + 4 * q], hacc[fbo][8 * cc + 4 * q + 1], hacc[fbo][8 * cc + 4 * q + 2], hacc[fbo][8 * cc + 4 * q + 3], f2,
                           h[2 * q], l[2 * q], h[2 * q + 1], l[2 * q + 1]);
            Hh[c] = rr_u4{h[0], h[1], h[2], h[3]};
            Hl[c] = rr_u4{l[0], l[1], l[2], l[3]};
        };
        hsplit(0);
        const unsigned t5 = clk();
#if RP_S1T
        const int voff_lane = (li * (32 * WB) + 4 * lh) * 4;
        const __amdgpu_buffer_rsrc_t orow = __builtin_amdgcn_make_buffer_rsrc(a.out + (int64_t)m0 * (32 * WB), 0, nn * (32 * WB * 4), 0x00020000);
        const rr_f2 inv22 = rr_f2{inv2, inv2};
        auto put4 = [&](const f32x16 &o, int fbn, int j) {
            int lic = 4 * lh;
            asm volatile("" : "+v"(lic));
            const float4 cv = *reinterpret_cast<const float4 *>(tab + 2 * 32 * WB + 32 * fbn + 8 * j + lic);
            const rr_f2 t0 = __builtin_elementwise_fma(rr_f2{o[4 * j], o[4 * j + 1]}, inv22, rr_f2{cv.x, cv.y});
            const rr_f2 t1 = __builtin_elementwise_fma(rr_f2{o[4 * j + 2], o[4 * j + 3]}, inv22, rr_f2{cv.z, cv.w});
            const rr_u4 y = rr_u4{(unsigned)max(__float_as_int(t0[0]), lo_1), (unsigned)max(__float_as_int(t0[1]), lo_1),
                                  (unsigned)max(__float_as_int(t1[0]), lo_1), (unsigned)max(__float_as_int(t1[1]), lo_1)};
#ifdef RR_ABL_NOSTORE
            asm volatile("" :: "v"(y));
#else
            __builtin_amdgcn_raw_buffer_store_b128(__builtin_bit_cast(__attribute__((__vector_size__(4 * sizeof(unsigned)))) unsigned, y), orow, voff_lane, (32 * fbn + 8 * j) * 4, RP_STORE_AUX);
#endif
        };
        f32x16 po0, po1;
#pragma unroll
        for (int r = 0; r < 16; ++r) { po0[r] = 0.f; po1[r] = 0.f; }
        {
#pragma unroll
            for (int fp = 0; fp < WB; fp += 2) {
                f32x16 o0, o1;
#pragma unroll
                for (int r = 0; r < 16; ++r) { o0[r] = 0.f; o1[r] = 0.f; }
                rr_u4 b0h = rr_lds_frag(ldsb, SH::F_W1 + 2 * (fp * NKS)), b0l = rr_lds_frag(ldsb, SH::F_W1 + 2 * (fp * NKS) + 1);
                rr_u4 b1h = rr_lds_frag(ldsb, SH::F_W1 + 2 * ((fp + 1) * NKS)), b1l = rr_lds_frag(ldsb, SH::F_W1 + 2 * ((fp + 1) * NKS) + 1);
                if (RP_DRAIN && fp == (RP_S1E ? 2 : 0)) __builtin_amdgcn_s_waitcnt(0x0f70);
#pragma unroll
                for (int c = 0; c < NKS; ++c) {
                    rr_u4 n0h = b0h, n0l = b0l, n1h = b1h, n1l = b1l;
                    if (c + 1 < NKS) {
                        n0h = rr_lds_frag(ldsb, SH::F_W1 + 2 * (fp * NKS + c + 1)); n0l = rr_lds_frag(ldsb, SH::F_W1 + 2 * (fp * NKS + c + 1) + 1);
                        n1h = rr_lds_frag(ldsb, SH::F_W1 + 2 * ((fp + 1) * NKS + c + 1)); n1l = rr_lds_frag(ldsb, SH::F_W1 + 2 * ((fp + 1) * NKS + c + 1) + 1);
                    }
                    RR_MFH(b0h, Hl[c], o0);
                    RR_MFH(b1h, Hl[c], o1);
                    RR_MFH(b0l, Hh[c], o0);
                    RR_MFH(b1l, Hh[c], o1);
                    RR_MFH(b0h, Hh[c], o0);
                    RR_MFH(b1h, Hh[c], o1);
                    if (fp == 0 && c + 1 < NKS) hsplit(c + 1);
                    if (fp == 0 && c == RP_GATHER_AT) gather(gA, rnext, lh);
                    if (fp > 0 && RP_S1E) { if (c < 4) put4(po0, fp - 2, c); else put4(po1, fp - 1, c - 4); }
                    RR_SB();
                    b0h = n0h; b0l = n0l; b1h = n1h; b1l = n1l;
                }
                if (fp + 2 < WB && RP_S1E) { po0 = o0; po1 = o1; continue; }
#pragma unroll
                for (int j = 0; j < 4; ++j) put4(o0, fp, j);
#pragma unroll
                for (int j = 0; j < 4; ++j) put4(o1, fp + 1, j);
                RR_SB();
            }
        }
        if (anybad) {
            asm volatile("s_waitcnt vmcnt(0)" ::: "memory");
            if (badrow) {
                const rr_u4 qn = rr_u4{0x7fc00000u, 0x7fc00000u, 0x7fc00000u, 0x7fc00000u};
#pragma unroll
                for (int q = 0; q < 4 * WB; ++q)
                    __builtin_amdgcn_raw_buffer_store_b128(__builtin_bit_cast(__attribute__((__vector_size__(4 * sizeof(unsigned)))) unsigned, qn), orow, voff_lane, 8 * q * 4, 0);
            }
        }
#else
        float invr[16];
        const int voff_lane = (4 * lh * 32 * WB + li) * 4;
        const __amdgpu_buffer_rsrc_t orow = __builtin_amdgcn_make_buffer_rsrc(a.out + (int64_t)m0 * (32 * WB), 0, nn * (32 * WB * 4), 0x00020000);
        auto put4 = [&](const f32x16 &o, int fbn, float cb, int j) {
            const rr_f2 cb2 = rr_f2{cb, cb};
#ifdef RR_ABL_STORE4
            {
                unsigned v4[4];
#pragma unroll
                for (int r = 4 * j; r < 4 * j + 4; r += 2) {
                    const rr_f2 t = __builtin_elementwise_fma(rr_f2{o[r], o[r + 1]}, rr_f2{invr[r], invr[r + 1]}, cb2);
                    v4[r - 4 * j] = (unsigned)max(__float_as_int(t[0]), lo_1); v4[r - 4 * j + 1] = (unsigned)max(__float_as_int(t[1]), lo_1);
                }
                typedef unsigned u4s __attribute__((__vector_size__(4 * sizeof(unsigned))));
                __builtin_amdgcn_raw_buffer_store_b128(u4s{v4[0], v4[1], v4[2], v4[3]}, orow, (lh * 32 * WB + 4 * li) * 4, (2 * (4 * fbn + j)) * (32 * WB * 4), RP_STORE_AUX);
                return;
            }
#endif
#pragma unroll
            for (int r = 4 * j; r < 4 * j + 4; r += 2) {
                const rr_f2 t = __builtin_elementwise_fma(rr_f2{o[r], o[r + 1]}, rr_f2{invr[r], invr[r + 1]}, cb2);
#pragma unroll
                for (int u = 0; u < 2; ++u)
#ifdef RR_ABL_NOSTORE
                    asm volatile("" :: "v"(max(__float_as_int(t[u]), lo_1)));
#else
                    __builtin_amdgcn_raw_buffer_store_b32((unsigned)max(__float_as_int(t[u]), lo_1), orow, voff_lane + ((r + u) & 3) * (32 * WB * 4) + 32 * fbn * 4,
                                                          sbase[(r + u) >> 2], RP_STORE_AUX);
#endif
            }
        };
        f32x16 po0, po1;
#pragma unroll
        for (int r = 0; r < 16; ++r) { po0[r] = 0.f; po1[r] = 0.f; }
        {
#pragma unroll
            for (int fp = 0; fp < WB; fp += 2) {
                f32x16 o0, o1;
#pragma unroll
                for (int r = 0; r < 16; ++r) { o0[r] = 0.f; o1[r] = 0.f; }
                rr_u4 b0h = rr_lds_frag(ldsb, SH::F_W1 + 2 * (fp * NKS)), b0l = rr_lds_frag(ldsb, SH::F_W1 + 2 * (fp * NKS) + 1);
                rr_u4 b1h = rr_lds_frag(ldsb, SH::F_W1 + 2 * ((fp + 1) * NKS)), b1l = rr_lds_frag(ldsb, SH::F_W1 + 2 * ((fp + 1) * NKS) + 1);
                if (RP_DRAIN && fp == (RP_S1E ? 2 : 0)) __builtin_amdgcn_s_waitcnt(0x0f70);
                int lic = li;
                asm volatile("" : "+v"(lic));
                const float cbp0 = fp > 0 ? tab[2 * 32 * WB + 32 * (fp - 2) + lic] : 0.f, cbp1 = fp > 0 ? tab[2 * 32 * WB + 32 * (fp - 1) + lic] : 0.f;
#pragma unroll
                for (int c = 0; c < NKS; ++c) {
                    rr_u4 n0h = b0h, n0l = b0l, n1h = b1h, n1l = b1l;
                    if (c + 1 < NKS) {
                        n0h = rr_lds_frag(ldsb, SH::F_W1 + 2 * (fp * NKS + c + 1)); n0l = rr_lds_frag(ldsb, SH::F_W1 + 2 * (fp * NKS + c + 1) + 1);
                        n1h = rr_lds_frag(ldsb, SH::F_W1 + 2 * ((fp + 1) * NKS + c + 1)); n1l = rr_lds_frag(ldsb, SH::F_W1 + 2 * ((fp + 1) * NKS + c + 1) + 1);
                    }
                    RR_MFH(Hl[c], b0h, o0);
                    RR_MFH(Hl[c], b1h, o1);
                    RR_MFH(Hh[c], b0l, o0);
                    RR_MFH(Hh[c], b1l, o1);
                    RR_MFH(Hh[c], b0h, o0);
                    RR_MFH(Hh[c], b1h, o1);
                    if (fp == 0 && c + 1 < NKS) hsplit(c + 1);
                    if (fp == 0 && c == RP_GATHER_AT) gather(gA, rnext, lh);
                    if (fp == 0 && c + 1 == NKS) {
                        int inv2l = __float_as_int(inv2);
                        asm volatile("" : "+v"(inv2l));
#pragma unroll
                        for (int r = 0; r < 16; ++r) invr[r] = __int_as_float(__builtin_amdgcn_ds_bpermute(4 * rr_crow(r, lh), inv2l));
                    }
                    if (fp > 0 && RP_S1E) { if (c < 4) put4(po0, fp - 2, cbp0, c); else put4(po1, fp - 1, cbp1, c - 4); }
                    RR_SB();
                    b0h = n0h; b0l = n0l; b1h = n1h; b1l = n1l;
                }
                if (fp + 2 < WB && RP_S1E) { po0 = o0; po1 = o1; continue; }
                int lid = li;
                asm volatile("" : "+v"(lid));
                const float cb0 = tab[2 * 32 * WB + 32 * fp + lid], cb1 = tab[2 * 32 * WB + 32 * (fp + 1) + lid];
#pragma unroll
                for (int j = 0; j < 4; ++j) put4(o0, fp, cb0, j);
#pragma unroll
                for (int j = 0; j < 4; ++j) put4(o1, fp + 1, cb1, j);
                RR_SB();
            }
        }
        if (anybad) {
            asm volatile("s_waitcnt vmcnt(0)" ::: "memory");
#pragma unroll
            for (int r = 0; r < 16; ++r)
                if (invr[r] != invr[r]) {
#pragma unroll
                    for (int fb = 0; fb < WB; ++fb)
                        __builtin_amdgcn_raw_buffer_store_b32(0x7fc00000u, orow, voff_lane, ((r & 3) + 8 * (r >> 2)) * (32 * WB * 4) + 32 * fb * 4, 0);
                }
        }
#endif
        if (PROF) { const unsigned t6 = clk(); pc[7] += 1; pc[3] += t4 - t3; pc[4] += t5 - t4; pc[5] += t6 - t5; }
    }
    if (PROF && prof && lane0 == 0 && (range == 0 || range == a.n_ranges / 2)) {
        unsigned long long *o = prof + (range == 0 ? 0 : 16);
        for (int q = 0; q < 8; ++q) o[q] = pc[q];
        o[8] = clk() - t_start;
    }
    if (PROF && prof && lane0 == 0) {
        prof[32 + 2 * range] = wave_t0;
        prof[32 + 2 * range + 1] = __builtin_amdgcn_s_memrealtime();
    }
}

__global__ void pack16_rows_kernel(const float *src, int64_t rows, int width, uint16_t *dst, int dst_stride, int col0, int one_col, int *status) {
    const int64_t gq = (int64_t)blockIdx.x * blockDim.x + threadIdx.x;
    const int wq = width > 0 ? (width + 3) >> 2 : 1;
    const int64_t row = gq / wq;
    const int q = (int)(gq % wq);
    if (row >= rows) return;
    bool bad = false;
#pragma unroll
    for (int j = 0; j < 4; ++j) {
        const int c = 4 * q + j;
        if (c >= width) break;
        const float v = src[row * width + c];
        const _Float16 h = (_Float16)v;
        bad = bad || !((float)h == v) || !(fabsf(v) < 2.f);
        dst[row * dst_stride + col0 + c] = __builtin_bit_cast(uint16_t, h);
    }
    if (q == 0 && one_col >= 0) dst[row * dst_stride + one_col] = 0x3c00;
    if (bad) atomicOr(status, 1);
}

static int rp_blocks(const gsn_chain_stage *edge, int64_t d_x, const float *x, int *edge_cols) {
    if (edge->n_blocks < 2 || edge->n_blocks > 6 || !edge->blocks) return 0;
    const gsn_block *b = edge->blocks;
    if (b[0].width != d_x || b[1].width != d_x || !b[0].idx32 || !b[1].idx32 || b[0].idx || b[1].idx) return 0;
    if (x && (b[0].data != x || b[1].data != x)) return 0;
    if (b[0].data != b[1].data) return 0;
    int64_t cols = 0;
    for (int i = 2; i < edge->n_blocks; ++i) {
        if (!b[i].idx32 || b[i].idx || b[i].idx32 != b[2].idx32 || b[i].width <= 0) return 0;
        cols += b[i].width;
    }
    if (cols > 16) return 0;
    *edge_cols = (int)cols;
    return 1;
}

int rp_supported(const gsn_chain_stage *edge, int64_t d_x, const gsn_chain_stage *node0, const gsn_chain_stage *node1) {
    if (!rr_shape_ok(edge, d_x, node0, node1)) return 0;
    int cols = 0;
    return rp_blocks(edge, d_x, nullptr, &cols);
}

int rp_forward(int64_t n_nodes, int64_t n_edges, const int32_t *seg_ptr, const gsn_chain_stage *edge, const float *x, int64_t d_x,
               const gsn_chain_stage *node0, const gsn_chain_stage *node1, const void *prepared, const gsn_pack16 *pack, int64_t edge_rows,
               float *out, hipStream_t st, const RpKeys *keys) {
    using SH = RrShape<4, 2>;
    int cols = 0;
    if (!rp_blocks(edge, d_x, x, &cols)) return set_error(GSN_E_INVALID, "gsn_layer_fused_fwd_pack16_hip: the edge stage is not cat(x[i], x[j], edge-level blocks through one index)");
    if (keys) {
        if (!keys->ekeys || !keys->nkey || !keys->idmask || !keys->node_dict || (reinterpret_cast<uintptr_t>(keys->node_dict) & 15) || (reinterpret_cast<uintptr_t>(keys->idmask) & 1))
            return set_error(GSN_E_INVALID, "gsn_count_layer_step_keys_hip: null / misaligned key arrays or node dictionary");
        if (keys->dict_rows < 1 || keys->dict_rows > 256 || cols < 1 || keys->edge_col0 < 0 || keys->edge_col0 > 16 || edge_rows != n_edges)
            return set_error(GSN_E_INVALID, "gsn_count_layer_step_keys_hip: node dictionary of %lld rows (1 .. 256), %d edge-level columns (>= 1), edge codes at column %d, %lld edge rows",
                             (long long)keys->dict_rows, cols, keys->edge_col0, (long long)edge_rows);
        if (edge_rows * 2 > 0x7fffffffll) return 1;
    } else {
    if (!pack || !pack->node_rows || (cols > 0 && !pack->edge_rows)) return set_error(GSN_E_INVALID, "gsn_layer_fused_fwd_pack16_hip: null pack");
    if ((reinterpret_cast<uintptr_t>(pack->node_rows) | reinterpret_cast<uintptr_t>(pack->edge_rows)) & 15) return set_error(GSN_E_INVALID, "gsn_layer_fused_fwd_pack16_hip: packs must be 16-byte aligned");
    if (n_nodes * 64 > 0x7fffffffll || edge_rows * 32 > 0x7fffffffll) return 1;
    }
    if (reinterpret_cast<const unsigned *>(prepared) == nullptr) return set_error(GSN_E_INVALID, "gsn_layer_fused_fwd_pack16_hip: null prepared");
    RpArgs a{};
    a.n_nodes = (int)n_nodes; a.n_edges = (int)n_edges; a.seg_ptr = seg_ptr;
    a.role_idx[0] = edge->blocks[0].idx32; a.role_idx[1] = edge->blocks[1].idx32;
    a.role_idx[2] = cols > 0 ? edge->blocks[2].idx32 : edge->blocks[0].idx32;
    if (keys) {
        a.node16 = keys->node_dict; a.node_bytes = (unsigned)(keys->dict_rows * 64);
        a.edge16 = keys->idmask; a.edge_bytes = (unsigned)(edge_rows * 2); a.edge_shift = 1;
        a.ekeys = keys->ekeys; a.nkey = keys->nkey; a.edge_col0 = keys->edge_col0;
    } else {
        a.node16 = pack->node_rows; a.node_bytes = (unsigned)(n_nodes * 64);
    }
    if (keys) {}
    else if (cols > 0) { a.edge16 = pack->edge_rows; a.edge_bytes = (unsigned)(edge_rows * 32); a.edge_shift = 5; }
    else { a.edge16 = pack->node_rows; a.edge_bytes = a.node_bytes; a.edge_shift = 6; }
    a.d_x = (int)d_x; a.out = out; a.prep = reinterpret_cast<const unsigned *>(prepared);
    const int64_t n_tiles = (n_nodes + RR_TN - 1) / RR_TN;
    int64_t gx = 256;
    if (const int g = sw_int(SW_FUSED_GRID, 0); g > 0) gx = g;
    int64_t ranges = gx * RR_NW;
    if (ranges > n_tiles) ranges = n_tiles;
    if (gx > ranges) gx = ranges;
    a.n_ranges = (int)ranges;
    {
        const char *d = sw_str(SW_RP_OLD_SHARE);
        const double share = d ? atof(d) : 0.6;
        a.n_split = (ranges == gx * RR_NW && share > 0.0 && share < 1.0) ? (int)((double)n_nodes * share) : 0;
    }
    static const bool prof_on = sw_on(SW_FUSED_PROF, false);
    const int lds_bytes = SH::LDS_BYTES + (keys ? RP_BYTE_TAB_BYTES : 0);
    static_assert(SH::LDS_BYTES % 16 == 0 && SH::LDS_BYTES + RP_BYTE_TAB_BYTES <= 160 * 1024, "the byte table fits behind the weights");
    if (keys) {
        const void *fn = prof_on ? reinterpret_cast<const void *>(&layer_fused_kernel_rp<4, 2, true, true>) : reinterpret_cast<const void *>(&layer_fused_kernel_rp<4, 2, false, true>);
        static DeviceOnce attr_set_keys;
        if (int rc = lds_limit(&attr_set_keys, {fn}, "layer_fused_kernel_rp keys", lds_bytes)) return rc;
    } else {
        const void *fn = prof_on ? reinterpret_cast<const void *>(&layer_fused_kernel_rp<4, 2, true>) : reinterpret_cast<const void *>(&layer_fused_kernel_rp<4, 2, false>);
        static DeviceOnce attr_set;
        if (int rc = lds_limit(&attr_set, {fn}, "layer_fused_kernel_rp")) return rc;
    }
    trace("gsn chain: layer_fused_kernel_rp<4,2>%s nodes %d edges %d grid %lld ranges %d\n", keys ? " keys" : "", a.n_nodes, a.n_edges, (long long)gx, a.n_ranges);
    if (prof_on) {
        ProfCounters prof(32 + 2 * (size_t)a.n_ranges, st);
        if (keys) hipLaunchKernelGGL((layer_fused_kernel_rp<4, 2, true, true>), dim3((unsigned)gx), dim3(64 * RR_NW), lds_bytes, st, a, prof.ptr());
        else
        hipLaunchKernelGGL((layer_fused_kernel_rp<4, 2, true>), dim3((unsigned)gx), dim3(64 * RR_NW), SH::LDS_BYTES, st, a, prof.ptr());
        const std::vector<unsigned long long> hv = prof.fetch(st);
        const unsigned long long *h = hv.data();
        static EveryNth show_nth{8};
        const bool show = show_nth();
        if (show) {
            unsigned long long t_lo = ~0ull, t_hi = 0, e_lo = ~0ull;
            double life = 0.0, lmin = 1e30, lmax = 0.0;
            for (int r = 0; r < a.n_ranges; ++r) {
                const unsigned long long s0 = h[32 + 2 * r], s1 = h[32 + 2 * r + 1];
                t_lo = s0 < t_lo ? s0 : t_lo; t_hi = s1 > t_hi ? s1 : t_hi; e_lo = s1 < e_lo ? s1 : e_lo;
                const double l = (double)(s1 - s0);
                life += l; lmin = l < lmin ? l : lmin; lmax = l > lmax ? l : lmax;
            }
            fprintf(stderr, "rpprof waves %d: first start -> last end %.1f us | wave life mean %.1f min %.1f max %.1f us | first end after %.1f us | mean life / span %.3f\n",
                    a.n_ranges, (t_hi - t_lo) / 100.0, life / a.n_ranges / 100.0, lmin / 100.0, lmax / 100.0, (e_lo - t_lo) / 100.0,
                    life / a.n_ranges / (double)(t_hi - t_lo));
        }
        if (show)
            for (int w = 0; w < 2; ++w) {
                const unsigned long long *o = h + 16 * w;
                const double nb = o[6] ? (double)o[6] : 1.0, nt = o[7] ? (double)o[7] : 1.0;
                fprintf(stderr, "rpprof range %s: blocks %llu tiles %llu total %llu cycles | per block: top %.0f edge %.0f | per tile: exposed edge epilogue %.0f stage0 %.0f split %.0f stage1 %.0f\n",
                        w ? "mid" : "0", o[6], o[7], o[8], o[0] / nb, o[1] / nb, o[2] / nt, o[3] / nt, o[4] / nt, o[5] / nt);
            }
    } else if (keys) {
        hipLaunchKernelGGL((layer_fused_kernel_rp<4, 2, false, true>), dim3((unsigned)gx), dim3(64 * RR_NW), lds_bytes, st, a, (unsigned long long *)nullptr);
    } else {
        hipLaunchKernelGGL((layer_fused_kernel_rp<4, 2, false>), dim3((unsigned)gx), dim3(64 * RR_NW), SH::LDS_BYTES, st, a, (unsigned long long *)nullptr);
    }
    return launch_check("layer_fused_kernel_rp");
}

}

using namespace gsn;

extern "C" int gsn_pack16_rows_hip(const float *src, int64_t rows, int64_t width, uint16_t *dst, int64_t dst_stride, int64_t col0,
                                   int64_t one_col, int32_t *status, void *stream) {
    if (rows < 0 || width < 0 || dst_stride <= 0 || col0 < 0 || col0 + width > dst_stride || one_col >= dst_stride)
        return set_error(GSN_E_INVALID, "gsn_pack16_rows_hip: rows %lld width %lld stride %lld col0 %lld one_col %lld", (long long)rows, (long long)width,
                         (long long)dst_stride, (long long)col0, (long long)one_col);
    if (rows == 0 || (width == 0 && one_col < 0)) return GSN_OK;
    if (!dst || !status || (width > 0 && !src)) return set_error(GSN_E_INVALID, "gsn_pack16_rows_hip: null pointer");
    const int wq = (int)((width + 3) >> 2) > 0 ? (int)((width + 3) >> 2) : 1;
    const int64_t total = rows * wq;
    hipLaunchKernelGGL(pack16_rows_kernel, dim3((unsigned)((total + 255) / 256)), dim3(256), 0, reinterpret_cast<hipStream_t>(stream), src, rows, (int)width, dst,
                       (int)dst_stride, (int)col0, (int)(one_col < 0 ? -1 : one_col), status);
    return launch_check("pack16_rows_kernel");
}

extern "C" int gsn_layer_keys_byte_table(uint16_t *dst) {
    if (!dst) return set_error(GSN_E_INVALID, "gsn_layer_keys_byte_table: dst is null");
    for (unsigned b = 0; b < 256; ++b)
        for (int q = 0; q < 4; ++q) {
            const unsigned w = rp_byte_tab_word(b, q);
            dst[8 * b + 2 * q] = (uint16_t)(w & 0xffffu);
            dst[8 * b + 2 * q + 1] = (uint16_t)(w >> 16);
        }
    return GSN_OK;
}
```

gsn_amd/csrc/layer_rr.h:

```cpp
#pragma once

#include <hip/hip_runtime.h>

#include "gsn_internal.h"

namespace gsn {

int rr_shape_ok(const gsn_chain_stage *edge, int64_t d_x, const gsn_chain_stage *node0, const gsn_chain_stage *node1);
int rr_supported(const gsn_chain_stage *edge, int64_t d_x, const gsn_chain_stage *node0, const gsn_chain_stage *node1);
int64_t rr_prepared_bytes(const gsn_chain_stage *edge, int64_t d_x, const gsn_chain_stage *node0, const gsn_chain_stage *node1);
int rr_prepare(const gsn_chain_stage *edge, int64_t d_x, const gsn_chain_stage *node0, const gsn_chain_stage *node1, void *prepared, hipStream_t st,
               bool pack16 = false);
int rr_forward(int64_t n_nodes, int64_t n_edges, const int32_t *seg_ptr, const gsn_chain_stage *edge, const float *x, int64_t d_x,
               const gsn_chain_stage *node0, const gsn_chain_stage *node1, const void *prepared, float *out, hipStream_t st);

struct RpKeys;
int rp_supported(const gsn_chain_stage *edge, int64_t d_x, const gsn_chain_stage *node0, const gsn_chain_stage *node1);
int rp_forward(int64_t n_nodes, int64_t n_edges, const int32_t *seg_ptr, const gsn_chain_stage *edge, const float *x, int64_t d_x,
               const gsn_chain_stage *node0, const gsn_chain_stage *node1, const void *prepared, const gsn_pack16 *pack, int64_t edge_rows,
               float *out, hipStream_t st, const RpKeys *keys = nullptr);
struct RpKeys {
    const uint32_t *ekeys;
    const uint8_t *nkey;
    const uint16_t *idmask;
    const uint16_t *node_dict;
    int64_t dict_rows;
    int edge_col0;
};

}
```

gsn_amd/csrc/switches.h:

```cpp
#pragma once

#include <cstdint>

namespace gsn {

enum SwitchLife { ONCE, LIVE };

#define GSN_SWITCH_TABLE(X)                                                                                                                \
                                                                                                                              \
    X(CHAIN_TRACE, LIVE, "present: every launcher names the kernel it takes on stderr (gsn::trace)")                                       \
                                                                                                                        \
    X(CHAIN_PERCU, LIVE, "int: workgroups per CU of mlp_chain_kernel (default 2 for small LDS footprints, else 1)")                        \
    X(CHAIN_DBG, LIVE, "int, default 0: ChainArgs::dbg ablation bits of mlp_chain_kernel")                                                 \
    X(CHAIN_PIPE, LIVE, "on/off, default on: 0 refuses the two-stage pipelined chain kernel")                                              \
    X(CHAIN_BF16X6, LIVE, "0 refuses the bf16x6 chain kernels; in chain_seg_bf16 the value is also the row tile (default 64)")             \
    X(CHAIN_SEGPIPE, LIVE, "int: row tile of the fp32 segment chain kernel, 0 refuses it")                                                 \
    X(PIPE_VEC4, LIVE, "on/off, default on: 16-byte staging loads of the bf16 pipe kernel")                                                \
    X(PIPE_PROF, LIVE, "on/off, default off: in-kernel phase clocks of the bf16 pipe kernel")                                              \
    X(SEG_PRIO, LIVE, "int: wave priority of the matrix phases; default 3 in chain_seg.hip, 0 in chain_seg_bf16.hip")                      \
    X(SEG_PROF, LIVE, "on/off, default off: in-kernel phase clocks of the segment chain kernels")                                          \
    X(SEG_VEC4, LIVE, "on/off, default on: 16-byte staging loads of the fp32 segment chain kernel")                                        \
                                                                                                             \
    X(FUSED_GRID, LIVE, "int > 0: grid size of the layer kernels (fused, rr, rp, w, g) instead of their own choice")                       \
    X(FUSED_PRIO, ONCE, "int, default 1: wave priority of layer_fused_kernel's matrix phases")                                             \
    X(FUSED_ABLATE, LIVE, "int: ablation bits of layer_fused_kernel's profiling build (read with GSN_FUSED_PROF only)")                    \
    X(FUSED_GENERIC, LIVE, "present: layer_fused takes its generic instantiation")                                                         \
    X(FUSED_PROF, LIVE, "on/off, default off: in-kernel phase clocks; layer_rr / rp / w / g latch it at their first launch")               \
    X(FUSED_RR, ONCE, "int, default 1: 0 refuses layer_fused_kernel_rr")                                                                   \
    X(FUSED_W, ONCE, "int, default 1: 0 refuses layer_fused_kernel_w")                                                                     \
    X(FUSED_G, ONCE, "int, default 1: 0 refuses layer_fused_kernel_g")                                                                     \
    X(RP_OLD_SHARE, ONCE, "float, default 0.6: share of the grid that layer_fused_kernel_rp gives to its first range")                     \
                                                                                                                        \
    X(LINEAR_SPLITK_RANGES, ONCE, "int, default -1 (automatic): forced split-k range count of the small bf16x6 linear, 0 = never")         \
    X(LINEAR_SMALL_MAX, ONCE, "int, default 96: most 128-row tiles that still take the 32-row-tile kernel, 0 = never")                     \
    X(LINEAR_BF16X6, ONCE, "on/off, default on: 0 selects the fp32-MFMA linear kernel")                                                    \
    X(LINEAR_VEC4, LIVE, "on/off, default on: float4 staging of A and W in the linear kernels")                                            \
    X(L16_SPLIT_WGS, ONCE, "int64, default 1024: workgroups of the fp16x3 row-split kernel, 0 = one tile per workgroup")                   \
    X(L16_WIDE, LIVE, "text, first character '1': 128 x 320 tiles in the fp16x3 linear where they fit (default off)")                      \
    X(L16_NOVEC, LIVE, "present: fp16x3 linear without 16-byte output stores")                                                             \
    X(L16_REGSTAGE, LIVE, "present: fp16x3 slices staged through registers; the planes launcher latches it at its first launch")           \
    X(L16_PROF, LIVE, "present: in-kernel phase clocks of the fp16x3 linear; the planes launcher latches it at its first launch")          \
    X(L16_DBG, LIVE, "int, default 0: ablation bits of the fp16x3 linear (1 no stores, 2 no products, 4 no loads)")                        \
                                                                                               \
    X(BWD_PLANES_WGS, ONCE, "int64 > 0, default 2048: workgroups of the backward plane-split kernel")                                      \
    X(FWD_PLANES_WGS, ONCE, "int64 > 0, default 2048: workgroups of the forward plane-split kernel")                                       \
    X(WGRAD_WGS, ONCE, "int64 > 0, default 0 (automatic): workgroup target of a weight-gradient call's slabs")                             \
    X(WGRAD_FP32, ONCE, "on/off, default off: weight gradient by the fp32 kernel")                                                         \
    X(WGRAD_PIPE, ONCE, "int, default 6 (1 means 6): pipeline depth of the bf16 weight-gradient kernel, 0 = unpipelined")                  \
    X(WGRAD16_WGS, ONCE, "int64 > 0, default 0 (automatic): workgroup target of the fp16x3 weight gradient")                               \
    X(WGRAD16_VALU, ONCE, "int, default 3: VALU-side variant of the fp16x3 weight-gradient kernel")                                        \
    X(WGRAD16_DBG, LIVE, "int, default 0: ablation bits of the fp16x3 weight-gradient kernels")                                            \
    X(WGRAD16_DMA, LIVE, "text, first character '1': the LDS-DMA fp16x3 weight-gradient kernel (default off)")                             \
                                                                                                                             \
    X(COUNT_MOL, ONCE, "on/off, default on: molecule-sized instantiation of count_kernel")                                                 \
    X(COUNT_CYCLE, ONCE, "on/off, default on: cycle instantiation of count_kernel")                                                        \
    X(COUNT_PAIR, LIVE, "on/off, default on: two graphs per workgroup where the plan allows")                                              \
    X(COUNT_TAIL_LOOP, ONCE, "int, default -1 (by plan): forces the tail-loop instantiation on (1) or off (0)")                            \
    X(COUNT_SPLIT_TARGET, ONCE, "int64 > 0, default 2048: workgroup count below which large graphs are split")                             \
    X(COUNT_ENC_BYTES, ONCE, "present: keep the byte array beside staged counts")                                                          \
    X(PULL_BATCH, ONCE, "int, default 8, clamped to 1..64: cells a counting wave pulls at a time")                                         \
                                                                                                                             \
    X(EMBED_NOVEC4, ONCE, "present: embedding kernels without 16-byte accesses")                                                           \
    X(EMBED_PIPE, ONCE, "on/off, default on: pipelined embedding sum kernel")                                                              \
    X(EMBED_LDS_MIN_ROWS, ONCE, "int64, default 8192: fewest rows that take the LDS embedding kernel")                                     \
    X(EMBED_BWD_LDS, ONCE, "on/off, default off: embedding backward by the LDS kernel only")                                               \
                                                                                                                          \
    X(PROP_CP, LIVE, "list lpr,unr,blocks: forces one mapping of the pipelined propagate kernel, \"0\" the generic one")                   \
    X(PROP_RS, LIVE, "list lpr,unr,nt[,blocks]: forces one mapping of relu_sum3_kernel, \"0\" the generic kernel")                         \
    X(PROP_LPR, ONCE, "int, default 0 (by width): forced lanes per row of the propagate kernels")                                          \
    X(PROP_BWD_PIPE, ONCE, "on/off, default on: pipelined propagate backward kernels")                                                     \
    X(PROP_FOLD_SELF, ONCE, "on/off, default on: the self term folded into the propagate backward kernel")

enum Switch : int {
#define GSN_SWITCH_ENUM(id, life, what) SW_##id,
    GSN_SWITCH_TABLE(GSN_SWITCH_ENUM)
#undef GSN_SWITCH_ENUM
    SW_COUNT
};

struct SwitchRow {
    const char *name;
    SwitchLife life;
    const char *what;
};
const SwitchRow &switch_row(Switch s);

const char *sw_str(Switch s);
int sw_int(Switch s, int dflt);
int64_t sw_int64(Switch s, int64_t dflt);
bool sw_on(Switch s, bool dflt);
bool sw_present(Switch s);

}
```

gsn_amd/step.py:

```python
from __future__ import annotations

import ctypes

import numpy as np
import torch

from . import _abi, _dense, flags, packs
from ._index import Codes, _CSR


def node_key_radices(n_classes, clamp):
    return [int(c) + (0 if clamp else 1) for c in n_classes]


def node_key(codes, n_classes, clamp):
    key = 0
    for c, (ncls, radix) in enumerate(zip(n_classes, node_key_radices(n_classes, clamp))):
        x = codes[:, c]
        if clamp:
            x = x.clip(0, ncls - 1)
        digit = x * ((x >= 0) & (x < ncls)) + ncls * ((x < 0) | (x >= ncls))
        key = key * radix + digit
    return key


def node_dict_tuples(n_classes, clamp):
    radices = node_key_radices(n_classes, clamp)
    grids = np.meshgrid(*[np.arange(r, dtype=np.int64) for r in radices], indexing="ij")
    return np.stack([g.reshape(-1) for g in grids], axis=1)


def keys_path_ok(n_classes, clamp):
    return int(np.prod(node_key_radices(n_classes, clamp), dtype=np.int64)) <= 256


_NODE_DICTS = {}


def node_dictionary(n_classes, clamp, dev):
    key = (tuple(int(c) for c in n_classes), bool(clamp), str(dev))
    d = _NODE_DICTS.get(key)
    if d is None:
        tuples = torch.from_numpy(node_dict_tuples(n_classes, clamp)).to(dev)
        d = torch.empty((tuples.shape[0], packs.NODE_COLS), dtype=torch.float16, device=dev)
        ncls = np.asarray(key[0], dtype=np.int32)
        st = torch.zeros(1, dtype=torch.int32, device=dev)
        with _abi.device_guard(dev):
            _abi.check(_abi.lib().gsn_one_hot_pack16_hip(tuples.shape[0], tuples.shape[1], tuples.data_ptr(), _abi.ptr(ncls), 0, d.data_ptr(),
                                                         packs.NODE_COLS, 0, packs.NODE_COLS - 1, st.data_ptr(), _abi.current_stream()), "gsn_one_hot_pack16_hip")
        if torch.cuda.is_current_stream_capturing():
            return d
        torch.cuda.current_stream(dev).synchronize()
        _NODE_DICTS[key] = d
    return d


class _StepBuffers(dict):
    expand = None

    def __missing__(self, name):
        if name in ("npack", "epack") and self.expand is not None:
            return self.expand()[0 if name == "npack" else 1]
        raise KeyError(name)


class CountLayerStep:

    def __init__(self, plan, layer, id_classes, clamp=True, force_packs=False):
        if plan.mode != "edge":
            raise ValueError("CountLayerStep: an edge-mode plan (GSN-e identifiers)")
        if getattr(plan, "wide", False):
            raise ValueError("CountLayerStep: wide plans count only (patterns of at most 9 vertices here)")
        self.plan, self.layer = plan, layer
        self.id_classes = [int(c) for c in id_classes]
        if len(self.id_classes) != plan.n_cols or min(self.id_classes) < 1:
            raise ValueError("CountLayerStep: one class count >= 1 per identifier column (%d columns)" % plan.n_cols)
        self.clamp = bool(clamp)
        self._enc_tab = np.asarray(self.id_classes, dtype=np.int32)
        if not (layer._one_launch_shape() and layer.has_ids):
            raise ValueError("CountLayerStep: a `general` GSN_edge_sparse layer with id_scope='local' and a two-stage msg_fn")
        self._bufs = None
        self._lay = None
        self._count_call = _abi.gsn_count_call()
        self._side = _abi.gsn_count_side()
        self._layer_call = _abi.gsn_layer_pack16_call()
        self._pk = _abi.gsn_pack16()
        self._keys = _abi.gsn_count_keys()
        self._force_packs = bool(force_packs)
        self.on_keys = False
        self._dict = None
        self._bound = None

    def _buffers(self, N, E, G, dev, keys):
        key = (N, E, G, str(dev), keys)
        if self._bufs is None or self._bufs[0] != key:
            b = _StepBuffers()
            b.update({
                "seg_ptr": torch.empty(N + 1, dtype=torch.int32, device=dev), "perm": torch.empty(max(E, 1), dtype=torch.int32, device=dev),
                "tgt": torch.empty(max(E, 1), dtype=torch.int32, device=dev), "src": torch.empty(max(E, 1), dtype=torch.int32, device=dev),
                "status": torch.empty(max(G, 1), dtype=torch.int32, device=dev), "code_status": torch.zeros(1, dtype=torch.int32, device=dev),
            })
            if keys:
                b.expand = self.packs
                b["nkey"] = torch.empty(N, dtype=torch.uint8, device=dev)
                b["ekeys"] = torch.empty(max(E, 1), dtype=torch.int32, device=dev)
                b["idmask"] = torch.empty(max(E, 1), dtype=torch.int16, device=dev)
            else:
                b["npack"] = torch.empty((N, packs.NODE_COLS), dtype=torch.float16, device=dev)
                b["epack"] = torch.empty((max(E, 1), packs.EDGE_COLS), dtype=torch.float16, device=dev)
            self._bufs = (key, b)
            self._lay = None
            self._bound = None
        return self._bufs[1]

    def _layer_structs(self, b, N, E, d_x, w_e):
        layer = self.layer
        if layer.training:
            raise RuntimeError("CountLayerStep: the layer must be in eval mode (train-mode BatchNorm takes batch statistics: not this kernel)")
        mf, uf = layer.msg_fn, layer.update_fn
        w_first = layer._folded_first_weight(d_x)
        dev = b["seg_ptr"].device
        sb = [(torch.empty((0, d_x), dtype=torch.float32, device=dev), None)]
        edge_stages = mf.stages(sb, upto=len(mf.fc) - 1)
        node_stages = uf.stages(sb, first_weight=w_first, post=None)
        stages = edge_stages + node_stages
        for st in stages:
            if st.act not in ("identity", "relu"):
                raise ValueError("CountLayerStep: activation %r is outside the one-launch layer kernel" % st.act)
            if st.bn is not None and (st.bn.training or st.bn.running_mean is None):
                raise RuntimeError("CountLayerStep: a BatchNorm1d in train mode / without running statistics")
        key = (tuple(_dense._prep_key(st) for st in stages), d_x, getattr(layer, "_fold_gen", 0), N, E, self.on_keys, 0 if self._dict is None else self._dict.data_ptr())
        if self._lay is not None and self._lay[0] == key:
            return self._lay[1]
        for st in stages:
            _dense._bn_resolve(st, None, 0, False)
        keep = []
        ew = torch.empty((0, w_e), dtype=torch.float32, device=dev)
        ge = _dense._stage_struct(edge_stages[0], [(sb[0][0], b["tgt"]), (sb[0][0], b["src"]), (ew, b["perm"])], keep)
        for i in range(3):
            if self.on_keys:
                ge.blocks[i].data = self._dict.data_ptr() if i < 2 else b["idmask"].data_ptr()
            else:
                ge.blocks[i].data = b["npack"].data_ptr() if i < 2 else b["epack"].data_ptr()
        g0 = _dense._stage_struct(node_stages[0], [], keep)
        g1 = _dense._stage_struct(node_stages[1], [], keep)
        L = _abi.lib()
        if node_stages[0].weight.shape[1] != d_x + edge_stages[0].weight.shape[0] + 4 or edge_stages[0].weight.shape[1] != 2 * d_x + w_e:
            raise ValueError("CountLayerStep: the layer's widths do not match the codes (d_x %d, edge-level columns %d)" % (d_x, w_e))
        if not L.gsn_layer_fused_pack16_supported(ctypes.byref(ge), d_x, ctypes.byref(g0), ctypes.byref(g1)):
            raise ValueError("CountLayerStep: shape outside the packed-row layer kernel (every stage 128 wide, d_x + 4 <= 32, <= 16 edge-level columns)")
        prep = _dense._prepared("_pack16", ge, g0, g1, d_x, dev)
        d_out = node_stages[1].weight.shape[0]
        flops = 2.0 * E * edge_stages[0].weight.shape[1] * edge_stages[0].weight.shape[0]
        flops += 2.0 * N * (node_stages[0].weight.shape[1] * node_stages[0].weight.shape[0] + node_stages[1].weight.shape[1] * d_out)
        val = (ge, g0, g1, prep, keep, d_out, flops)
        self._lay = (key, val)
        self._bound = None
        return val

    def __call__(self, node_ptr, edge_ptr, edge_index, x_codes, ef_codes, max_nodes, max_edges, ids_out=None, ids_are_global=True, out=None):
        _abi.require_gpu()
        if not (isinstance(x_codes, Codes) and isinstance(ef_codes, Codes)):
            raise TypeError("CountLayerStep: x_codes / ef_codes are gsn_amd.layers.Codes (integer codes + class counts)")
        dev = edge_index.device
        N, E, G = x_codes.codes.shape[0], edge_index.shape[1], node_ptr.numel() - 1
        if ef_codes.codes.shape[0] != E or edge_index.dtype != torch.int64 or edge_index.shape[0] != 2 or edge_index.stride(1) != 1:
            raise ValueError("CountLayerStep: edge_index int64 [2, E] with unit column stride, one edge code row per column")
        if E == 0 or G == 0:
            raise ValueError("CountLayerStep: an edge-less batch has no GSN-e identifiers (use the layer's own forward)")
        d_x, w_ids, w_ef = sum(x_codes.n_classes), sum(self.id_classes), sum(ef_codes.n_classes)
        if d_x > packs.NODE_COLS - 4 or w_ids + w_ef > packs.EDGE_COLS or len(x_codes.n_classes) > 4 or len(ef_codes.n_classes) > 4 or w_ids % 4 or w_ef > 8:
            raise ValueError("CountLayerStep: code widths outside the packs (node %d <= 28, edge %d + %d <= 16, identifier classes a multiple of 4, "
                             "<= 8 edge code classes)" % (d_x, w_ids, w_ef))
        keys = not self._force_packs and keys_path_ok(x_codes.n_classes, x_codes.clamp)
        self.on_keys = keys
        self._dict = node_dictionary(x_codes.n_classes, x_codes.clamp, dev) if keys else None
        b = self._buffers(N, E, G, dev, keys)
        ge, g0, g1, prep, _keep, d_out, flops = self._layer_structs(b, N, E, d_x, w_ids + w_ef)
        if ids_out is None:
            ids_out = torch.empty((E, self.plan.n_cols), dtype=torch.int64, device=dev)
        y = out if out is not None else torch.empty((N, d_out), dtype=torch.float32, device=dev)
        c, s, l = self._count_call, self._side, self._layer_call
        bound = (node_ptr.data_ptr(), edge_ptr.data_ptr(), edge_index.data_ptr(), edge_index.stride(0), x_codes.codes.data_ptr(), ef_codes.codes.data_ptr(),
                 int(max_nodes), int(max_edges), bool(ids_are_global), tuple(x_codes.n_classes), tuple(ef_codes.n_classes), x_codes.clamp, ef_codes.clamp, id(prep),
                 keys)
        if self._bound != bound:
            tab = self.plan.device_table(dev)
            c.plan_host = _abi.ptr(self.plan.table); c.plan_dev = tab.data_ptr(); c.plan_words = len(self.plan.table); c.n_graphs = G
            c.node_ptr = node_ptr.data_ptr(); c.edge_ptr = edge_ptr.data_ptr(); c.edge_index = edge_index.data_ptr(); c.edge_row_stride = edge_index.stride(0)
            c.ids_are_global = int(bool(ids_are_global)); c.max_nodes = int(max_nodes); c.max_edges = int(max_edges)
            c.status = b["status"].data_ptr(); c.n_classes = _abi.ptr(self._enc_tab); c.clamp = int(self.clamp)
            c.pack = 0 if keys else b["epack"].data_ptr(); c.pack_stride = packs.EDGE_COLS; c.pack_col0 = 0
            s.csr_row = self.layer._sel(); s.seg_ptr = b["seg_ptr"].data_ptr(); s.perm = b["perm"].data_ptr()
            s.sorted_target = b["tgt"].data_ptr(); s.sorted_other = b["src"].data_ptr(); s.n_nodes = N; s.n_edges = E
            s.node_codes = x_codes.codes.data_ptr(); s.node_code_cols = len(x_codes.n_classes); s.node_clamp = int(x_codes.clamp)
            s.edge_codes = ef_codes.codes.data_ptr(); s.edge_code_cols = len(ef_codes.n_classes); s.edge_clamp = int(ef_codes.clamp)
            for i in range(4):
                s.node_n_classes[i] = x_codes.n_classes[i] if i < len(x_codes.n_classes) else 0
                s.edge_n_classes[i] = ef_codes.n_classes[i] if i < len(ef_codes.n_classes) else 0
            s.node_pack = 0 if keys else b["npack"].data_ptr(); s.edge_col0 = w_ids; s.code_status = b["code_status"].data_ptr()
            c.side = ctypes.pointer(s)
            if keys:
                k = self._keys
                k.nkey = b["nkey"].data_ptr(); k.ekeys = b["ekeys"].data_ptr(); k.idmask = b["idmask"].data_ptr()
                self._pk.node_rows = 0; self._pk.edge_rows = 0
            else:
                self._pk.node_rows = b["npack"].data_ptr(); self._pk.edge_rows = b["epack"].data_ptr()
            l.n_nodes = N; l.n_edges = E; l.seg_ptr = b["seg_ptr"].data_ptr(); l.edge = ctypes.pointer(ge); l.d_x = d_x
            l.x = self._dict.data_ptr() if keys else b["npack"].data_ptr()
            l.node0 = ctypes.pointer(g0); l.node1 = ctypes.pointer(g1); l.prepared = prep.data_ptr(); l.pack = ctypes.pointer(self._pk); l.edge_rows = E
            self._bound = bound
        c.out = ids_out.data_ptr()
        l.out = y.data_ptr()
        timer = flags.KERNEL_TIMER
        L = _abi.lib()
        if keys:
            kref, dptr, drows = ctypes.byref(self._keys), self._dict.data_ptr(), self._dict.shape[0]
            entry = "gsn_count_layer_step_keys_hip"

            def call(ev_between):
                return L.gsn_count_layer_step_keys_hip(ctypes.byref(c), ctypes.byref(l), kref, dptr, drows, ev_between, _abi.current_stream())
        else:
            entry = "gsn_count_layer_step_hip"

            def call(ev_between):
                return L.gsn_count_layer_step_hip(ctypes.byref(c), ctypes.byref(l), ev_between, _abi.current_stream())
        if timer is None:
            with _abi.device_guard(dev):
                rc = call(None)
        else:
            only = flags.KERNEL_TIMER_ONLY
            ev = [torch.cuda.Event(enable_timing=True) for _ in range(3)]
            with _abi.device_guard(dev):
                ev[1].record()
                if only is None or "count" in only:
                    ev[0].record()
                rc = call(ev[1].cuda_event)
                ev[2].record()
            if only is None or "count" in only:
                if keys:
                    nbytes = 16.0 * E + 8.0 * E * self.plan.n_cols + 2.0 * E + 16.0 * E + 9.0 * N + 12.0 * E + 12.0 * E + 4.0 * N
                else:
                    nbytes = 16.0 * E + 8.0 * E * self.plan.n_cols + 2.0 * E * w_ids + 16.0 * E + 72.0 * N + 16.0 * E + 12.0 * E + 4.0 * N
                timer.setdefault("count", []).append((ev[0], ev[1], nbytes))
            if only is None or "layer_fused" in only:
                timer.setdefault("layer_fused", []).append((ev[1], ev[2], flops))
        _abi.check(rc, entry)
        self._last = (w_ids, d_x)
        return ids_out, y, b["status"]

    def csr(self):
        b = self._bufs[1]
        c = _CSR()
        c.seg_ptr, c.perm, c.tgt, c.src, c.part = b["seg_ptr"], b["perm"], b["tgt"], b["src"], None
        c._deg = c._deg4 = None
        return c

    def packs(self):
        b = self._bufs[1]
        if "npack" in b:
            return b["npack"], b["epack"]
        w_ids = self._last[0]
        npack = self._dict[b["nkey"].long()]
        bond = torch.zeros_like(b["ekeys"])
        bond[b["perm"].long()] = (b["ekeys"] >> 16) & 0xff
        mask = (b["idmask"].to(torch.int32) & 0xffff) | (bond << w_ids)
        cols = torch.arange(packs.EDGE_COLS, dtype=torch.int32, device=mask.device)
        epack = ((mask.unsqueeze(1) >> cols.unsqueeze(0)) & 1).to(torch.float16)
        return npack, epack

    def check_status(self):
        from .counting import _raise_statuses
        b = self._bufs[1]
        _raise_statuses(b["status"])
        if int(b["code_status"].item()) != 0:
            raise IndexError("a code outside its column's classes (one-hot encoding of integer codes)")
```

include/gsn_abi.h:

```cpp
#ifndef GSN_ABI_H
#define GSN_ABI_H

#include <stdint.h>

#ifdef __cplusplus
extern "C" {
#endif

#define GSN_ABI_VERSION 1
#define GSN_KMAX 9
#define GSN_KMAX_WIDE 16
#define GSN_SEG_RANGE_ROWS 16

enum {
    GSN_OK = 0,
    GSN_E_INVALID = -1,
    GSN_E_UNSUPPORTED = -2,
    GSN_E_HIP = -3,
    GSN_E_NOSPACE = -4,
    GSN_E_NODEVICE = -5
};

enum { GSN_MODE_VERTEX = 0, GSN_MODE_EDGE = 1 };

enum {
    GSN_ST_OK = 0,
    GSN_ST_KEYERROR = 1,
    GSN_ST_TOO_LARGE = 2,
    GSN_ST_BAD_INDEX = 3,
    GSN_ST_ASYMMETRIC = 4,
    GSN_ST_NO_CONVERGENCE = 5,
    GSN_ST_UNSEEN = 6
};

enum { GSN_LOOKUP_STRICT = 0, GSN_LOOKUP_CLAMP = 1 };

const char *gsn_last_error(void);
const char *gsn_propagate_last_route(void);
int gsn_version(void);
int gsn_device_count(void);
int64_t gsn_stream_capture_id(void *stream);
int gsn_fingerprint_hip(int n_tensors, const int64_t *meta, int64_t max_words, unsigned long long *acc, unsigned long long *host_out,
                        void *stream);

#define GSN_FLAG_DIRECTED_ORBITS 1
#define GSN_FLAG_DIRECTED 2
#define GSN_FLAG_WIDE 4
int gsn_pattern_orbits(int64_t n_edges, const int64_t *edges, int directed_orbits, int64_t *out_k,
                       int64_t *out_vertex_orbit, int64_t *out_n_vertex_orbits, int64_t *out_arcs,
                       int64_t *out_arc_orbit, int64_t *out_n_arcs, int64_t *out_n_edge_orbits,
                       int64_t *out_aut_count);

int gsn_graph_vertex_orbits(int64_t n_vertices, int64_t n_edges, const int64_t *edges, int64_t *out_orbit,
                            int64_t *out_n_orbits);

int gsn_count_plan_build(int mode, int induced, int directed_orbits, int64_t n_patterns, const int64_t *pat_ptr,
                         const int64_t *pat_edges, uint32_t *plan, int64_t capacity, int64_t *out_words,
                         int64_t *out_n_cols);

int gsn_count_hip(const uint32_t *plan_host, const uint32_t *plan_dev, int64_t plan_words, int64_t n_graphs,
                  const int64_t *node_ptr, const int64_t *edge_ptr, const int64_t *edge_index,
                  int64_t edge_row_stride, int ids_are_global, const int32_t *graph_ids, int64_t n_items,
                  int64_t max_nodes, int64_t max_edges, int64_t *out, int32_t *status, void *stream);

int gsn_count_sparse_hip(const uint32_t *plan_host, const uint32_t *plan_dev, int64_t plan_words, int64_t n_graphs,
                         const int64_t *node_ptr, const int64_t *edge_ptr, const int64_t *edge_index,
                         int64_t edge_row_stride, int ids_are_global, const int32_t *graph_ids, int64_t n_items,
                         int64_t max_nodes, int64_t max_edges, int64_t *out, int32_t *status, void *workspace,
                         int64_t workspace_bytes, void *stream);
int64_t gsn_count_sparse_workspace_bytes(int64_t n_vertices_total, int64_t n_columns_processed, int64_t n_cols);

int gsn_count_encode_hip(const uint32_t *plan_host, const uint32_t *plan_dev, int64_t plan_words, int64_t n_graphs,
                         const int64_t *node_ptr, const int64_t *edge_ptr, const int64_t *edge_index,
                         int64_t edge_row_stride, int ids_are_global, const int32_t *graph_ids, int64_t n_items,
                         int64_t max_nodes, int64_t max_edges, int64_t *out, int32_t *status, const int32_t *n_classes,
                         int clamp, float *enc_out, void *stream);
int gsn_count_encode_pack16_hip(const uint32_t *plan_host, const uint32_t *plan_dev, int64_t plan_words, int64_t n_graphs,
                                const int64_t *node_ptr, const int64_t *edge_ptr, const int64_t *edge_index,
                                int64_t edge_row_stride, int ids_are_global, const int32_t *graph_ids, int64_t n_items,
                                int64_t max_nodes, int64_t max_edges, int64_t *out, int32_t *status, const int32_t *n_classes,
                                int clamp, float *enc_out, uint16_t *pack, int64_t pack_stride, int64_t pack_col0, void *stream);

typedef struct {
    int csr_row;
    int32_t *seg_ptr;
    int32_t *perm;
    int32_t *sorted_target;
    int32_t *sorted_other;
    int64_t n_nodes, n_edges;
    const int64_t *node_codes;
    int node_code_cols;
    int node_n_classes[4];
    int node_clamp;
    uint16_t *node_pack;
    const int64_t *edge_codes;
    int edge_code_cols;
    int edge_n_classes[4];
    int edge_clamp;
    int edge_col0;
    int32_t *code_status;
} gsn_count_side;
int gsn_count_encode_pack16_side_hip(const uint32_t *plan_host, const uint32_t *plan_dev, int64_t plan_words, int64_t n_graphs,
                                     const int64_t *node_ptr, const int64_t *edge_ptr, const int64_t *edge_index,
                                     int64_t edge_row_stride, int ids_are_global, int64_t max_nodes, int64_t max_edges, int64_t *out,
                                     int32_t *status, const int32_t *n_classes, int clamp, uint16_t *pack, int64_t pack_stride,
                                     int64_t pack_col0, const gsn_count_side *side, void *stream);

typedef struct {
    uint8_t *nkey;
    uint32_t *ekeys;
    uint16_t *idmask;
} gsn_count_keys;
int gsn_count_encode_keys_side_hip(const uint32_t *plan_host, const uint32_t *plan_dev, int64_t plan_words, int64_t n_graphs,
                                   const int64_t *node_ptr, const int64_t *edge_ptr, const int64_t *edge_index,
                                   int64_t edge_row_stride, int ids_are_global, int64_t max_nodes, int64_t max_edges, int64_t *out,
                                   int32_t *status, const int32_t *n_classes, int clamp, int64_t pack_col0, const gsn_count_side *side,
                                   const gsn_count_keys *keys, void *stream);

int64_t gsn_csr_scratch_elems(int64_t n_nodes);
int gsn_csr_build_hip(int64_t n_nodes, int64_t n_edges, const int64_t *index, const int64_t *other, int32_t *seg_ptr,
                      int32_t *perm, int32_t *sorted_target, int32_t *sorted_other, int32_t *scratch, void *stream);

enum { GSN_MSG_CAT = 0, GSN_MSG_RELU_SUM = 1 };

int gsn_propagate_fwd_hip(int kind, int64_t n_nodes, int64_t n_edges, const int64_t *src, const int32_t *seg_ptr,
                          const int32_t *perm, const int32_t *sorted_src, const float *a, int64_t da, const float *b, int64_t db,
                          int b_per_node, const float *c, int64_t dc, float *out, void *stream);

int gsn_segment_sum_rows_hip(int64_t n_nodes, int64_t n_edges, const int64_t *src, const int32_t *seg_ptr, const int32_t *perm,
                             const int32_t *sorted_src, const float *b, int64_t width, int64_t ld, float *out, void *stream);

int gsn_propagate_bwd_hip(int kind, int64_t n_nodes, int64_t n_edges, const int64_t *src, const int64_t *tgt,
                          const int32_t *seg_ptr_src, const int32_t *perm_src, const float *a, int64_t da,
                          const float *b, int64_t db, int b_per_node, const float *c, int64_t dc,
                          const float *g_out, float *g_a, float *g_b, float *g_c, void *stream);

typedef struct gsn_self_block {
    const float *data;
    int64_t width;
    int64_t row_stride;
} gsn_self_block;

int gsn_propagate_self_fwd_hip(int kind, int64_t n_nodes, int64_t n_edges, const int64_t *src, const int32_t *seg_ptr,
                               const int32_t *perm, const int32_t *sorted_src, const float *a, int64_t da, const float *b, int64_t db,
                               int b_per_node, const float *c, int64_t dc, int64_t pad_b, int64_t pad_c, int n_self,
                               const gsn_self_block *self_blocks, const float *eps, float *out, void *stream);

int gsn_propagate_self_bwd_hip(int kind, int64_t n_nodes, int64_t d_out, const float *g_out, int n_self,
                               const gsn_self_block *self_blocks, float *const *g_self, const float *eps, double *g_eps,
                               double *g_colsum, void *stream);

int gsn_propagate_pad_bwd_hip(int kind, int64_t n_nodes, int64_t n_edges, const int64_t *src, const int64_t *tgt,
                              const int32_t *seg_ptr_src, const int32_t *perm_src, const float *a, int64_t da,
                              const float *b, int64_t db, int b_per_node, const float *c, int64_t dc, int64_t pad_b, int64_t pad_c,
                              const float *g_out, float *g_a, float *g_b, float *g_c, void *stream);
int gsn_propagate_bwd_fold_self_hip(int64_t n_nodes, int64_t n_edges, const int64_t *src, const int64_t *tgt, const int32_t *seg_ptr_src,
                                    const int32_t *perm_src, const float *a, int64_t d, const float *b, int64_t db, const float *c, int64_t dc,
                                    const float *g_out, float *g_a, float *g_b, float *g_c, const float *eps, double *g_eps, void *stream);

typedef struct {
    const float *data;
    const int64_t *idx;
    int64_t width;
    const int32_t *idx32;
} gsn_block;

int gsn_linear_fwd_hip(int64_t m_rows, int n_blocks, const gsn_block *blocks, const float *W, const float *bias,
                       int64_t n_out, const float *bn_mean, const float *bn_scale, const float *bn_shift, int act,
                       const int32_t *row_perm, float *out, double *stats, void *stream);
int gsn_linear_fwd_strided_hip(int64_t m_rows, int n_blocks, const gsn_block *blocks, const float *W, int64_t w_row_stride,
                               int64_t w_col_stride, const float *bias, int64_t n_out, const float *bn_mean, const float *bn_scale,
                               const float *bn_shift, int act, float *out, double *stats, void *stream);

int gsn_linear_splitk_plan(int64_t m_rows, int64_t k_total, int64_t n_out);
int gsn_linear_fwd_splitk_hip(int64_t m_rows, int n_blocks, const gsn_block *blocks, const float *W, int64_t w_row_stride,
                              int64_t w_col_stride, const float *bias, int64_t n_out, float *out, void *stream);

typedef struct {
    const gsn_block *blocks;
    int n_blocks;
    const float *W;
    const float *bias;
    int64_t n_out;
    const float *bn_mean, *bn_scale, *bn_shift;
    int act;
} gsn_chain_stage;

int gsn_mlp_chain_supported(int n_stages, const gsn_chain_stage *stages);
int gsn_mlp_chain_fwd_hip(int64_t m_rows, int n_stages, const gsn_chain_stage *stages, const int32_t *row_perm,
                          const int32_t *seg_target, float *out, double *stats, void *stream);

int gsn_layer_fused_supported(const gsn_chain_stage *edge, int64_t d_x, const gsn_chain_stage *node0,
                              const gsn_chain_stage *node1);
int64_t gsn_layer_fused_prepared_bytes(const gsn_chain_stage *edge, int64_t d_x, const gsn_chain_stage *node0,
                                       const gsn_chain_stage *node1);
int gsn_layer_fused_prepare_hip(const gsn_chain_stage *edge, int64_t d_x, const gsn_chain_stage *node0,
                                const gsn_chain_stage *node1, void *prepared, void *stream);
int gsn_layer_fused_fwd_hip(int64_t n_nodes, int64_t n_edges, const int32_t *seg_ptr, const gsn_chain_stage *edge,
                            const float *x, int64_t d_x, const gsn_chain_stage *node0, const gsn_chain_stage *node1,
                            const void *prepared, float *out, void *stream);
int64_t gsn_layer_fused_workspace_bytes(int64_t n_nodes, const gsn_chain_stage *edge, int64_t d_x, const gsn_chain_stage *node0,
                                        const gsn_chain_stage *node1);
int gsn_layer_fused_fwd_ws_hip(int64_t n_nodes, int64_t n_edges, const int32_t *seg_ptr, const gsn_chain_stage *edge,
                               const float *x, int64_t d_x, const gsn_chain_stage *node0, const gsn_chain_stage *node1,
                               const void *prepared, float *out, void *workspace, int64_t workspace_bytes,
                               const int32_t *x_row_exp, int32_t *out_row_exp, void *stream);

int gsn_layer_fused_graphs_supported(const gsn_chain_stage *edge, int64_t d_x, const gsn_chain_stage *node0,
                                     const gsn_chain_stage *node1);
int gsn_layer_fused_fwd_graphs_hip(int64_t n_nodes, int64_t n_edges, const int32_t *seg_ptr, const gsn_chain_stage *edge,
                                   const float *x, int64_t d_x, const gsn_chain_stage *node0, const gsn_chain_stage *node1,
                                   const void *prepared, int64_t n_graphs, const int64_t *node_ptr, int64_t max_nodes,
                                   float *out, void *stream);

typedef struct {
    const uint16_t *node_rows;
    const uint16_t *edge_rows;
} gsn_pack16;
int gsn_pack16_rows_hip(const float *src, int64_t rows, int64_t width, uint16_t *dst, int64_t dst_stride, int64_t col0,
                        int64_t one_col, int32_t *status, void *stream);
int gsn_one_hot_pack16_hip(int64_t m_rows, int n_cols, const int64_t *values, const int32_t *n_classes, int clamp, uint16_t *dst,
                           int64_t dst_stride, int64_t col0, int64_t one_col, int32_t *status, void *stream);
int gsn_layer_fused_pack16_supported(const gsn_chain_stage *edge, int64_t d_x, const gsn_chain_stage *node0,
                                     const gsn_chain_stage *node1);
int64_t gsn_layer_fused_pack16_prepared_bytes(const gsn_chain_stage *edge, int64_t d_x, const gsn_chain_stage *node0,
                                              const gsn_chain_stage *node1);
int gsn_layer_fused_pack16_prepare_hip(const gsn_chain_stage *edge, int64_t d_x, const gsn_chain_stage *node0,
                                       const gsn_chain_stage *node1, void *prepared, void *stream);
int gsn_layer_fused_fwd_pack16_hip(int64_t n_nodes, int64_t n_edges, const int32_t *seg_ptr, const gsn_chain_stage *edge,
                                   const float *x, int64_t d_x, const gsn_chain_stage *node0, const gsn_chain_stage *node1,
                                   const void *prepared, const gsn_pack16 *pack, int64_t edge_rows, float *out, void *stream);

typedef struct {
    const uint32_t *plan_host, *plan_dev;
    int64_t plan_words, n_graphs;
    const int64_t *node_ptr, *edge_ptr, *edge_index;
    int64_t edge_row_stride;
    int ids_are_global;
    int64_t max_nodes, max_edges;
    int64_t *out;
    int32_t *status;
    const int32_t *n_classes;
    int clamp;
    uint16_t *pack;
    int64_t pack_stride, pack_col0;
    const gsn_count_side *side;
} gsn_count_call;
typedef struct {
    int64_t n_nodes, n_edges;
    const int32_t *seg_ptr;
    const gsn_chain_stage *edge;
    const float *x;
    int64_t d_x;
    const gsn_chain_stage *node0, *node1;
    const void *prepared;
    const gsn_pack16 *pack;
    int64_t edge_rows;
    float *out;
} gsn_layer_pack16_call;
int gsn_count_layer_step_hip(const gsn_count_call *count, const gsn_layer_pack16_call *layer, void *event_between, void *stream);
int gsn_layer_keys_byte_table(uint16_t *dst);
int gsn_count_layer_step_keys_hip(const gsn_count_call *count, const gsn_layer_pack16_call *layer, const gsn_count_keys *keys,
                                  const uint16_t *node_dict, int64_t dict_rows, void *event_between, void *stream);

int64_t gsn_linear_f16x3_kpad(int64_t k_total);
int64_t gsn_linear_f16x3_mpad(int64_t m_rows);
int64_t gsn_linear_f16x3_scratch_bytes(int64_t m_rows, int64_t k_total);
int gsn_linear_f16x3_prepare_hip(const float *W, int64_t n_out, int64_t k_total, void *planes, float *col_inv, void *stream);
int gsn_linear_f16x3_prepare_strided_hip(const float *W, int64_t n_out, int64_t k_total, int64_t w_row_stride, int64_t w_col_stride,
                                         void *planes, float *col_inv, void *stream);
int gsn_linear_f16x3_fwd_hip(int64_t m_rows, int n_blocks, const gsn_block *blocks, const void *planes, const float *col_inv,
                             const float *bias, int64_t n_out, const float *bn_mean, const float *bn_scale, const float *bn_shift,
                             int act, float *row_scratch, float *out, void *stream);
int gsn_linear_f16x3_fwd_stats_hip(int64_t m_rows, int n_blocks, const gsn_block *blocks, const void *planes, const float *col_inv,
                                   const float *bias, int64_t n_out, float *row_scratch, float *out, double *stats, void *stream);
int gsn_linear_f16x3_split_rows_hip(int64_t m_rows, int n_blocks, const gsn_block *blocks, float *row_scratch, void *stream);
int gsn_linear_f16x3_fwd_presplit_hip(int64_t m_rows, int n_blocks, const gsn_block *blocks, const void *planes, const float *col_inv,
                                      const float *bias, int64_t n_out, const float *bn_mean, const float *bn_scale, const float *bn_shift,
                                      int act, float *row_scratch, float *out, void *stream);
int gsn_linear_f16x3_fwd_stats_presplit_hip(int64_t m_rows, int n_blocks, const gsn_block *blocks, const void *planes, const float *col_inv,
                                            const float *bias, int64_t n_out, float *row_scratch, float *out, double *stats, void *stream);
int gsn_bn_act_planes_hip(int64_t m_rows, int64_t n_cols, const float *h, const float *mean, const float *scale, const float *shift, int act,
                          float *out, float *row_scratch, void *stream);
int gsn_wgrad_f16x3_hip(int64_t m_rows, int64_t n_out, int64_t k_total, const void *g_scratch, const void *x_scratch, float *grad_w,
                        void *stream);

int gsn_edge_split_sum_hip(int64_t n_nodes, int64_t n_edges, const int32_t *seg_ptr, const int32_t *sorted_src,
                           const int32_t *perm, const float *p_i, const float *p_j, int64_t pitch, const float *z0,
                           int64_t w0, const float *z1, int64_t w1, const float *wz_t, int64_t d, int act, float *out,
                           void *stream);

int gsn_csr_build_graphs_hip(int64_t n_graphs, const int64_t *node_ptr, const int64_t *edge_ptr, int64_t n_nodes,
                             int64_t n_edges, int64_t max_nodes, int64_t max_edges, const int64_t *index,
                             const int64_t *other, int32_t *seg_ptr, int32_t *perm, int32_t *sorted_target,
                             int32_t *sorted_other, int32_t *status, void *stream);

int gsn_segsum_prepare_hip(int64_t n_seg, int64_t n_rows, const int32_t *seg_ptr, const int32_t *row_target,
                           int64_t n_out, float *out, void *stream);

int gsn_one_hot_hip(int64_t m_rows, int n_cols, const int64_t *values, const int32_t *n_classes, int clamp, float *out,
                    void *stream);

int gsn_column_range_hip(int64_t m_rows, int n_cols, const int64_t *values, int64_t *col_min, int64_t *col_max,
                         void *stream);
int gsn_column_ranks_hip(int64_t m_rows, int n_cols, const int64_t *values, const int64_t *col_min,
                         const int64_t *col_base, int64_t table_elems, int32_t *table, int64_t *codes,
                         int64_t *n_distinct, void *stream);

int64_t gsn_unique_sort_scratch_bytes(int64_t m_rows, int64_t n_cols);
int gsn_unique_sort_hip(int64_t m_rows, int64_t n_cols, const int64_t *values, int64_t *uniques, int64_t *n_distinct,
                        int64_t *codes, void *scratch, int64_t scratch_bytes, void *stream);

int gsn_lookup_codes_hip(int64_t n_rows, int64_t n_cols, const int64_t *values, const int64_t *uniques, const int64_t *col_ptr,
                         int mode, int64_t *codes, int32_t *status, int64_t *first_unseen, void *stream);

int gsn_embed_fwd_hip(int64_t m_rows, int n_cols, int d, int concat, const int64_t *codes, const int64_t *meta,
                      const int64_t *table_rows, float *out, int32_t *status, void *stream);
int gsn_embed_bwd_hip(int64_t m_rows, int n_cols, int d, int concat, const int64_t *codes, const int64_t *grad_meta,
                      const int64_t *table_rows, const float *grad_out, void *stream);
int gsn_embed_bwd_flat_supported(int64_t m_rows, int n_cols, int concat, const int64_t *table_rows);
int gsn_embed_bwd_flat_hip(int64_t m_rows, int n_cols, int d, int concat, const int64_t *codes, float *grad_flat,
                           const int64_t *table_offsets, const int64_t *table_rows, const float *grad_out, void *stream);

#define GSN_MAX_CODE_SLOTS 16
typedef struct gsn_code_slot {
    const int64_t *codes;
    const int32_t *idx;
    int32_t stride, col;
    int32_t w_off;
    int32_t n_classes;
    int32_t clamp;
    int32_t reserved;
} gsn_code_slot;
int gsn_code_stage_supported(int n_slots, int64_t k_total, int64_t n_out);
int gsn_code_stage_fwd_hip(int64_t m_rows, int n_slots, const gsn_code_slot *slots, const float *WT, int64_t k_total,
                           const float *bias, int64_t n_out, const float *bn_mean, const float *bn_scale,
                           const float *bn_shift, int act, const int32_t *seg_target, float *out, double *stats,
                           int32_t *status, void *stream);

int gsn_bn_act_hip(int64_t m_rows, int64_t n_cols, const float *h, const float *mean, const float *scale,
                   const float *shift, int act, float *out, void *stream);
int gsn_column_stats_hip(int64_t m_rows, int64_t n_cols, const float *h, double *stats, void *stream);

int gsn_bn_act_bwd_hip(int64_t m_rows, int64_t n_cols, const float *grad_y, const float *y, const float *h,
                       const float *mean, const float *invstd, const float *coef, int train_bn, int act, double *sums,
                       float *grad_h, double *grad_bias, void *stream);
int gsn_bn_act_bwd_from_h_hip(int64_t m_rows, int64_t n_cols, const float *grad_y, const float *h, const float *mean,
                              const float *invstd, const float *coef, const float *shift, int train_bn, int act, double *sums,
                              float *grad_h, double *grad_bias, void *stream);
int gsn_bn_act_bwd_planes_hip(int64_t m_rows, int64_t n_cols, const float *grad_y, const float *h, const float *mean, const float *invstd,
                              const float *coef, const float *shift, int train_bn, int act, double *sums, float *row_scratch,
                              double *grad_bias, void *stream);
int gsn_wgrad_hip(int64_t m_rows, int64_t n_out, const float *grad_h, int n_blocks, const gsn_block *blocks, float *grad_w,
                  void *stream);
int gsn_fold_weights_fwd_hip(int64_t rows, int64_t d_x, int64_t a_cols, int64_t h_cols, int64_t pad_cols, const float *w3, int64_t ld3,
                             const float *w2, int64_t ld2, const float *b2, float *out, void *stream);
int gsn_fold_weights_bwd_hip(int64_t rows, int64_t d_x, int64_t a_cols, int64_t h_cols, const float *g, int64_t ldg, const float *w3,
                             int64_t ld3, const float *w2, int64_t ld2, const float *b2, float *g_w3, float *g_w2, float *g_b2,
                             void *stream);

int gsn_gather_cat_hip(int64_t m_rows, int n_blocks, const gsn_block *blocks, float *out, void *stream);

int gsn_add_gathered_hip(int64_t n_rows, int64_t d, const float *x, const float *table, const int64_t *idx, int64_t n_table, float *out,
                         void *stream);

int gsn_bn_finalize_hip(int64_t n_cols, int64_t m_rows, double eps, double momentum, const double *stats, const float *gamma,
                        const float *beta, float *running_mean, float *running_var, float *mean, float *invstd, float *scale,
                        float *shift, void *stream);
int gsn_bn_finalize_act_hip(int64_t n_cols, int64_t m_rows, double eps, double momentum, const double *stats, const float *gamma,
                            const float *beta, float *running_mean, float *running_var, float *mean, float *invstd, float *scale,
                            float *shift, int64_t *num_batches_tracked, const float *h, int act, float *out, void *stream);

int gsn_bn_finalize_count_hip(int64_t n_cols, int64_t m_rows, double eps, double momentum, const double *stats, const float *gamma,
                              const float *beta, float *running_mean, float *running_var, float *mean, float *invstd, float *scale,
                              float *shift, int64_t *num_batches_tracked, void *stream);

enum {
    GSN_DGN_MEAN = 0, GSN_DGN_SUM = 1, GSN_DGN_MAX = 2, GSN_DGN_MIN = 3, GSN_DGN_VAR = 4, GSN_DGN_STD = 5,
    GSN_DGN_DIR_AV = 6,
    GSN_DGN_DIR_SOFTMAX = 7,
    GSN_DGN_DIR_DX = 8,
    GSN_DGN_DIR_DX_NOABS = 9,
    GSN_DGN_DIR_DX_BALANCED = 10
};
enum { GSN_DGN_IDENTITY = 0, GSN_DGN_AMPLIFICATION = 1, GSN_DGN_ATTENUATION = 2 };
typedef struct {
    int32_t kind;
    int32_t col;
    float alpha;
    int32_t slot;
} gsn_dgn_agg;
int gsn_dgn_aggregate_fwd_hip(int64_t n_nodes, int64_t n_edges, int64_t d, const int32_t *seg_ptr, const int32_t *perm, const int32_t *src,
                              const float *h, const float *node_field, int64_t node_stride, int64_t node_width, const float *edge_field,
                              int64_t edge_stride, int64_t edge_width, const gsn_dgn_agg *aggs, int n_aggs, const int32_t *scalers,
                              int n_scalers, double avg_d_log, float *out, void *stream);
int gsn_dgn_aggregate_bwd_hip(int64_t n_nodes, int64_t n_edges, int64_t d, const int32_t *seg_ptr, const int32_t *perm, const int32_t *src,
                              const int32_t *src_seg_ptr, const int32_t *src_perm, const float *h, const float *node_field,
                              int64_t node_stride, int64_t node_width, const float *edge_field, int64_t edge_stride, int64_t edge_width,
                              const gsn_dgn_agg *aggs, int n_aggs, const int32_t *scalers, int n_scalers, double avg_d_log,
                              const float *grad_out, float *grad_msg, float *grad_h, void *stream);

#define GSN_EIG_KMAX 8
enum { GSN_EIG_NORM_NONE = 0, GSN_EIG_NORM_SYM = 1, GSN_EIG_NORM_WALK = 2 };
int gsn_laplacian_eig_hip(int64_t n_graphs_total, const int64_t *node_ptr, const int64_t *edge_ptr, const int64_t *edge_index,
                          int64_t n_edges, const int32_t *graph_ids, int64_t n_ids, int n_class, int norm, int k, int max_sweeps,
                          float *vec, float *val, int32_t *status, int32_t *sweeps_used, float *scratch, int64_t scratch_floats,
                          void *stream);
int64_t gsn_laplacian_eig_scratch_floats(int n_class, int64_t n_ids);

#define GSN_ADAM_CHUNK_ELEMS 8192
#define GSN_ADAM_TENSOR_WORDS 6
#define GSN_ADAM_GROUP_DOUBLES 8
int gsn_adam_step_hip(int n_tensors, const int64_t *tensors, int64_t n_chunks, const int32_t *chunks, int n_groups, const double *groups,
                      float *exp_avg, float *exp_avg_sq, float *steps, unsigned *done, int64_t max_elems, void *stream);

enum { GSN_LOSS_BCE = 0, GSN_LOSS_L1 = 1, GSN_LOSS_MSE = 2, GSN_LOSS_CE = 3 };
int64_t gsn_masked_loss_scratch_bytes(int kind, int64_t rows, int64_t cols);
int gsn_masked_loss_fwd_hip(int kind, int64_t rows, int64_t cols, const float *y_hat, const void *y, float *loss, int64_t *count,
                            void *scratch, int64_t scratch_bytes, void *stream);
int gsn_masked_loss_bwd_hip(int kind, int64_t rows, int64_t cols, const float *y_hat, const void *y, const float *grad_loss,
                            const int64_t *count, float *grad_y_hat, void *stream);

enum { GSN_METRIC_NONE = 0, GSN_METRIC_L1 = 1, GSN_METRIC_MSE = 2, GSN_METRIC_ACCURACY = 3 };
enum { GSN_EVAL_WEIGHTED_LOSS = 0, GSN_EVAL_BATCH_LOSS = 1, GSN_EVAL_METRIC = 2 };
enum { GSN_EVAL_CURSOR = 0, GSN_EVAL_BATCHES = 1, GSN_EVAL_CORRECT = 2, GSN_EVAL_STATUS = 3 };
#define GSN_EVAL_ACC_WORDS 4
#define GSN_EVAL_OVERFLOW 1
int64_t gsn_eval_accumulate_scratch_bytes(int kind, int64_t rows, int64_t cols);
int gsn_eval_accumulate_hip(int kind, int metric, int64_t rows, int64_t cols, int64_t y_cols, const float *y_hat, const void *y,
                            int64_t num_graphs, double *acc_f64, int64_t *acc_i64, float *pred_buf, void *true_buf, int64_t capacity,
                            float *loss_out, void *scratch, int64_t scratch_bytes, void *stream);

enum { GSN_RANK_ONE_CLASS = 1, GSN_RANK_NO_POSITIVE = 2, GSN_RANK_NONFINITE = 4, GSN_RANK_BAD_LABEL = 8 };
int64_t gsn_rank_metrics_scratch_bytes(int64_t m_rows, int64_t n_cols);
int gsn_rank_metrics_hip(int64_t m_rows, int64_t n_cols, const float *y_pred, const float *y_true, int64_t *out_i64, double *out_f64,
                         int32_t *status, void *scratch, int64_t scratch_bytes, void *stream);

#ifdef __cplusplus
}
#endif
#endif
```

Before: 133.7 million graphs/s.

## Replace target-node edge-weight products with precomputed per-key x_i tables in LDS

When the node dictionary has at most 31 rows, a one-block kernel precomputes the product of each dictionary row with the first two edge-weight chunks for the target-node slot. The fused layer kernel then stores these tables in LDS in place of the four weight fragments they replace, and gathers the per-row partial accumulators by key instead of loading the target node rows and issuing their MFMAs. This removes two global loads and part of the matrix work per edge tile. In exchange it adds LDS gathers, bpermutes and a new template arm, plus an extra setup launch whenever the cached layer state is rebuilt. The cache key now also tracks the bias version.

```diff
diff --git a/gsn_amd/_abi.py b/gsn_amd/_abi.py
--- a/gsn_amd/_abi.py
+++ b/gsn_amd/_abi.py
@@ -94,6 +94,11 @@
                                                c_i64, ctypes.POINTER(gsn_count_side), ctypes.POINTER(gsn_count_keys), c_vp]),
     "gsn_count_layer_step_keys_hip": (c_int, [ctypes.POINTER(gsn_count_call), ctypes.POINTER(gsn_layer_pack16_call), ctypes.POINTER(gsn_count_keys),
                                               c_vp, c_i64, c_vp, c_vp]),
+    "gsn_count_layer_step_tabs_hip": (c_int, [ctypes.POINTER(gsn_count_call), ctypes.POINTER(gsn_layer_pack16_call), ctypes.POINTER(gsn_count_keys),
+                                              c_vp, c_i64, c_vp, c_vp, c_vp]),
+    "gsn_layer_key_tables_words": (c_i64, []),
+    "gsn_layer_key_tables_max_rows": (c_i64, []),
+    "gsn_layer_key_tables_hip": (c_int, [c_vp, c_vp, c_i64, c_vp, c_vp]),
     "gsn_layer_keys_byte_table": (c_int, [c_vp]),
     "gsn_pack16_rows_hip": (c_int, [c_vp, c_i64, c_i64, c_vp, c_i64, c_i64, c_i64, c_vp, c_vp]),
     "gsn_one_hot_pack16_hip": (c_int, [c_i64, c_int, c_vp, c_vp, c_int, c_vp, c_i64, c_i64, c_i64, c_vp, c_vp]),
diff --git a/gsn_amd/_dense.py b/gsn_amd/_dense.py
--- a/gsn_amd/_dense.py
+++ b/gsn_amd/_dense.py
@@ -221,7 +221,7 @@
     if bn is not None:
         bk = (bn.running_mean._version, bn.running_var._version, bn.running_mean.data_ptr(),
               (bn.weight._version, bn.bias._version) if bn.affine else None)
-    return (st.weight.data_ptr(), st.weight._version, tuple(st.weight.shape), bk)
+    return (st.weight.data_ptr(), st.weight._version, tuple(st.weight.shape), bk, None if st.bias is None else st.bias._version)
 
 
 def _prepared(kind, ge, g0, g1, d_x, dev, owner=None, attr=None, key=None):
diff --git a/gsn_amd/csrc/abi.cpp b/gsn_amd/csrc/abi.cpp
--- a/gsn_amd/csrc/abi.cpp
+++ b/gsn_amd/csrc/abi.cpp
@@ -119,6 +119,11 @@
 
 extern "C" int gsn_count_layer_step_keys_hip(const gsn_count_call *c, const gsn_layer_pack16_call *l, const gsn_count_keys *keys, const uint16_t *node_dict,
                                              int64_t dict_rows, void *event_between, void *stream) {
+    return gsn_count_layer_step_tabs_hip(c, l, keys, node_dict, dict_rows, nullptr, event_between, stream);
+}
+
+extern "C" int gsn_count_layer_step_tabs_hip(const gsn_count_call *c, const gsn_layer_pack16_call *l, const gsn_count_keys *keys, const uint16_t *node_dict,
+                                             int64_t dict_rows, const float *tabs, void *event_between, void *stream) {
     if (!c || !l || !keys || !c->side) return gsn::set_error(GSN_E_INVALID, "gsn_count_layer_step_keys_hip: null call struct / keys / side");
     if (!keys->nkey || !keys->ekeys || !keys->idmask || !node_dict) return gsn::set_error(GSN_E_INVALID, "gsn_count_layer_step_keys_hip: null key array / node dictionary");
     if (!c->side->node_codes || !c->side->edge_codes) return gsn::set_error(GSN_E_INVALID, "gsn_count_layer_step_keys_hip: node and edge codes are both needed");
@@ -135,7 +140,7 @@
     if (rc != GSN_OK) return rc;
     if (event_between && hipEventRecord(reinterpret_cast<hipEvent_t>(event_between), reinterpret_cast<hipStream_t>(stream)) != hipSuccess)
         return gsn::set_error(GSN_E_HIP, "gsn_count_layer_step_keys_hip: hipEventRecord(event_between)");
-    const gsn::RpKeys k{keys->ekeys, keys->nkey, keys->idmask, node_dict, dict_rows, c->side->edge_col0};
+    const gsn::RpKeys k{keys->ekeys, keys->nkey, keys->idmask, node_dict, dict_rows, c->side->edge_col0, tabs};
     rc = gsn::rp_forward(l->n_nodes, l->n_edges, l->seg_ptr, l->edge, l->x, l->d_x, l->node0, l->node1, l->prepared, nullptr, l->edge_rows, l->out,
                          reinterpret_cast<hipStream_t>(stream), &k);
     if (rc == 1) return gsn::set_error(GSN_E_UNSUPPORTED, "gsn_count_layer_step_keys_hip: key arrays beyond 2 GiB (32-bit buffer offsets)");
diff --git a/gsn_amd/csrc/layer_rp.hip b/gsn_amd/csrc/layer_rp.hip
--- a/gsn_amd/csrc/layer_rp.hip
+++ b/gsn_amd/csrc/layer_rp.hip
@@ -28,6 +28,7 @@
     const uint32_t *ekeys;
     const uint8_t *nkey;
     int edge_col0;
+    const float *tabs;
 };
 
 struct RpIdx { int r[3]; int pt, pt1; int nk; };
@@ -59,6 +60,18 @@
     return ((b >> (2 * q)) & 1u ? 0x3c00u : 0u) | ((b >> (2 * q + 1)) & 1u ? 0x3c000000u : 0u);
 }
 
+constexpr int RP_TAB_ROWS = 31;
+constexpr int RP_TAB_WORDS = 4 * RP_TAB_ROWS * 32;
+
+template <class U>
+__device__ __forceinline__ void rp_edge_chunk(const rr_u4 &A, const rr_u4 &f0h, const rr_u4 &f0l, const rr_u4 &f1h, const rr_u4 &f1l, f32x16 &acc0, f32x16 &acc1, U &&under) {
+    RR_MFH(A, f0l, acc0);
+    RR_MFH(A, f1l, acc1);
+    under();
+    RR_MFH(A, f0h, acc0);
+    RR_MFH(A, f1h, acc1);
+}
+
 #define RP_LOAD(RS, VOFF, IMM) __builtin_bit_cast(rr_u4, __builtin_amdgcn_raw_buffer_load_b128(RS, (int)((VOFF) + (IMM)), 0, 0))
 
 __device__ __forceinline__ unsigned rp_scale_pair(unsigned pair, float s) {
@@ -97,7 +110,7 @@
 #define RP_S1E 1
 #endif
 
-template <int WB, int NKX, bool PROF, bool KEYS = false>
+template <int WB, int NKX, bool PROF, bool KEYS = false, bool TABS = false>
 __global__ __launch_bounds__(64 * RR_NW) __attribute__((amdgpu_waves_per_eu(RR_NW / 4, RR_NW / 4))) void layer_fused_kernel_rp(RpArgs a, unsigned long long *prof) {
     auto clk = [&]() -> unsigned {
         if (!PROF) return 0u;
@@ -110,6 +123,7 @@
     using SH = RrShape<WB, NKX>;
     constexpr int NKS = SH::NKS, NK0 = SH::NK0;
     static_assert(WB == 4 && NKX == 2, "two pairs of feature blocks; the node pack is two chunks wide");
+    static_assert(!TABS || KEYS, "the tables are indexed by the key words");
     extern __shared__ __attribute__((aligned(16))) unsigned char smem[];
 
     const int tid = threadIdx.x;
@@ -123,6 +137,15 @@
     {
         const rr_u4 *src = reinterpret_cast<const rr_u4 *>(a.prep + RR_HDR);
         rr_u4 *dst = reinterpret_cast<rr_u4 *>(smem);
+        if constexpr (TABS) {
+            static_assert(SH::F_WE == 0 && RP_TAB_ROWS * 128 <= 4096, "a table fits the room of the four fragments it replaces");
+            for (int i = tid; i < SH::F_LDS * 64; i += 64 * RR_NW) {
+                const int f = i >> 6;
+                if (!(f < 2 * WB * RR_NKE && f % (2 * RR_NKE) < 4)) dst[i] = src[i];
+            }
+            float *te = reinterpret_cast<float *>(smem);
+            for (int i = tid; i < RP_TAB_WORDS; i += 64 * RR_NW) te[(i / (RP_TAB_ROWS * 32)) * (2 * RR_NKE * 256) + i % (RP_TAB_ROWS * 32)] = a.tabs[i];
+        } else
         for (int i = tid; i < SH::F_LDS * 64; i += 64 * RR_NW) dst[i] = src[i];
         const float *tsrc = reinterpret_cast<const float *>(a.prep + RR_HDR + SH::F_ALL * 256);
         float *tdst = reinterpret_cast<float *>(smem + SH::F_LDS * 1024);
@@ -190,7 +213,7 @@
         if constexpr (KEYS) {
             const unsigned k = (unsigned)r[0];
             const unsigned vt = ((k & 0xffu) << 6) | ((unsigned)lh << 4), vs = (((k >> 8) & 0xffu) << 6) | ((unsigned)lh << 4);
-            g[0] = RP_LOAD(rs_n, vt, 0); g[1] = RP_LOAD(rs_n, vt, 32);
+            if constexpr (!TABS) { g[0] = RP_LOAD(rs_n, vt, 0); g[1] = RP_LOAD(rs_n, vt, 32); }
             g[2] = RP_LOAD(rs_n, vs, 0); g[3] = RP_LOAD(rs_n, vs, 32);
             g[4][0] = (unsigned)__builtin_amdgcn_raw_buffer_load_b16(rs_e, (int)((unsigned)r[2] << 1), 0, 0);
         } else {
@@ -231,7 +254,8 @@
             tpt = pt; tpt1 = pt1;
             rr_u4 Ah[RR_NKE];
 #pragma unroll
-            for (int c = 0; c < RR_NKE; ++c) Ah[c] = gc[c];
+            for (int c = TABS ? 2 : 0; c < RR_NKE; ++c) Ah[c] = gc[c];
+            const unsigned ko = (kc & 0xffu) << 7;
             if constexpr (KEYS) {
                 const unsigned m16 = gc[RR_NKE - 1][0] | ((kc >> 16) << ec0);
                 const unsigned byte = (m16 >> (8 * lh)) & 0xffu;
@@ -294,18 +318,49 @@
                     for (int c = 0; c < RR_NKE; ++c) {
                         rr_u4 n0h = f0h, n0l = f0l, n1h = f1h, n1l = f1l;
                         if (c + 1 < RR_NKE) frag4(fp, c + 1, n0h, n0l, n1h, n1l);
-                        RR_MFH(Ah[c], f0l, acc0);
-                        RR_MFH(Ah[c], f1l, acc1);
-                        under(c);
-                        RR_MFH(Ah[c], f0h, acc0);
-                        RR_MFH(Ah[c], f1h, acc1);
+                        rp_edge_chunk(Ah[c], f0h, f0l, f1h, f1l, acc0, acc1, [&]() { under(c); });
+                        RR_SB();
+                        f0h = n0h; f0l = n0l; f1h = n1h; f1l = n1l;
+                    }
+                };
+                auto products_t = [&](int fp, f32x16 &acc0, f32x16 &acc1, auto &&under) {
+                    rr_u4 f0h, f0l, f1h, f1l;
+                    frag4(fp, 2, f0h, f0l, f1h, f1l);
+#pragma unroll
+                    for (int c = 2; c < RR_NKE; ++c) {
+                        rr_u4 n0h = f0h, n0l = f0l, n1h = f1h, n1l = f1l;
+                        if (c + 1 < RR_NKE) frag4(fp, c + 1, n0h, n0l, n1h, n1l);
+                        rp_edge_chunk(Ah[c], f0h, f0l, f1h, f1l, acc0, acc1, [&]() { under(2 * (c - 2)); });
+                        under(2 * (c - 2) + 1);
                         RR_SB();
                         f0h = n0h; f0l = n0l; f1h = n1h; f1l = n1l;
                     }
                 };
                 f32x16 qa0, qa1, ra0, ra1;
+                if constexpr (TABS) {
+                    typedef const volatile __attribute__((address_space(3))) float *ldsf;
+                    const unsigned tb = ldsb[0] - 16u * (unsigned)lane + 4u * (unsigned)li;
+                    unsigned ta[16];
+#pragma unroll
+                    for (int r = 0; r < 16; ++r) ta[r] = (unsigned)__builtin_amdgcn_ds_bpermute(4 * rr_crow(r, lh), (int)ko) + tb;
+#pragma unroll
+                    for (int r = 0; r < 16; ++r) {
+                        qa0[r] = *reinterpret_cast<ldsf>(ta[r]);
+                        qa1[r] = *reinterpret_cast<ldsf>(ta[r] + 2 * RR_NKE * 1024);
+                    }
+                    RR_SB();
+                    products_t(0, qa0, qa1, [&](int s) {
+#pragma unroll
+                        for (int r = 3 * s; r < 3 * s + 3 && r < 16; ++r) {
+                            ra0[r] = *reinterpret_cast<ldsf>(ta[r] + 2 * 2 * RR_NKE * 1024);
+                            ra1[r] = *reinterpret_cast<ldsf>(ta[r] + 3 * 2 * RR_NKE * 1024);
+                        }
+                    });
+                    products_t(2, ra0, ra1, [&](int s) { if (s < RR_NKE) ep_step(s, qa0, qa1, sacc[0], sacc[1], M); });
+                } else {
                 products(0, qa0, qa1, [&](int) {});
                 products(2, ra0, ra1, [&](int c) { ep_step(c, qa0, qa1, sacc[0], sacc[1], M); });
+                }
                 t2 = clk();
                 load_x();
 #pragma unroll
@@ -689,6 +744,33 @@
     if (bad) atomicOr(status, 1);
 }
 
+__global__ __launch_bounds__(128) void rp_key_tables_kernel(const unsigned *prep, const uint16_t *dict, int dict_rows, float *tabs) {
+    using SH = RrShape<4, 2>;
+    const int lane = threadIdx.x & 63, fp = 2 * (int)(threadIdx.x >> 6);
+    const int li = lane & 31, lh = lane >> 5;
+    const __amdgpu_buffer_rsrc_t rs_n = __builtin_amdgcn_make_buffer_rsrc(const_cast<uint16_t *>(dict), 0, dict_rows * 64, 0x00020000);
+    const rr_u4 *frags = reinterpret_cast<const rr_u4 *>(prep + RR_HDR);
+    auto frag = [&](int f) { return frags[f * 64 + lane]; };
+    f32x16 acc0, acc1;
+#pragma unroll
+    for (int r = 0; r < 16; ++r) { acc0[r] = 0.f; acc1[r] = 0.f; }
+    const unsigned vt = ((unsigned)li << 6) | ((unsigned)lh << 4);
+#pragma unroll
+    for (int c = 0; c < 2; ++c) {
+        const rr_u4 A = RP_LOAD(rs_n, vt, 32 * c);
+        rp_edge_chunk(A, frag(SH::F_WE + 2 * (fp * RR_NKE + c)), frag(SH::F_WE + 2 * (fp * RR_NKE + c) + 1), frag(SH::F_WE + 2 * ((fp + 1) * RR_NKE + c)),
+                      frag(SH::F_WE + 2 * ((fp + 1) * RR_NKE + c) + 1), acc0, acc1, []() {});
+    }
+#pragma unroll
+    for (int r = 0; r < 16; ++r) {
+        const int k = rr_crow(r, lh);
+        if (k < RP_TAB_ROWS) {
+            tabs[(fp * RP_TAB_ROWS + k) * 32 + li] = acc0[r];
+            tabs[((fp + 1) * RP_TAB_ROWS + k) * 32 + li] = acc1[r];
+        }
+    }
+}
+
 static int rp_blocks(const gsn_chain_stage *edge, int64_t d_x, const float *x, int *edge_cols) {
     if (edge->n_blocks < 2 || edge->n_blocks > 6 || !edge->blocks) return 0;
     const gsn_block *b = edge->blocks;
@@ -724,6 +806,8 @@
             return set_error(GSN_E_INVALID, "gsn_count_layer_step_keys_hip: node dictionary of %lld rows (1 .. 256), %d edge-level columns (>= 1), edge codes at column %d, %lld edge rows",
                              (long long)keys->dict_rows, cols, keys->edge_col0, (long long)edge_rows);
         if (edge_rows * 2 > 0x7fffffffll) return 1;
+        if (keys->tabs && (keys->dict_rows > RP_TAB_ROWS || (reinterpret_cast<uintptr_t>(keys->tabs) & 3)))
+            return set_error(GSN_E_INVALID, "gsn_count_layer_step_tabs_hip: x_i tables with a node dictionary of %lld rows (<= %d)", (long long)keys->dict_rows, RP_TAB_ROWS);
     } else {
     if (!pack || !pack->node_rows || (cols > 0 && !pack->edge_rows)) return set_error(GSN_E_INVALID, "gsn_layer_fused_fwd_pack16_hip: null pack");
     if ((reinterpret_cast<uintptr_t>(pack->node_rows) | reinterpret_cast<uintptr_t>(pack->edge_rows)) & 15) return set_error(GSN_E_INVALID, "gsn_layer_fused_fwd_pack16_hip: packs must be 16-byte aligned");
@@ -738,6 +822,7 @@
         a.node16 = keys->node_dict; a.node_bytes = (unsigned)(keys->dict_rows * 64);
         a.edge16 = keys->idmask; a.edge_bytes = (unsigned)(edge_rows * 2); a.edge_shift = 1;
         a.ekeys = keys->ekeys; a.nkey = keys->nkey; a.edge_col0 = keys->edge_col0;
+        a.tabs = sw_on(SW_RP_TABLES, true) ? keys->tabs : nullptr;
     } else {
         a.node16 = pack->node_rows; a.node_bytes = (unsigned)(n_nodes * 64);
     }
@@ -760,6 +845,11 @@
     static const bool prof_on = sw_on(SW_FUSED_PROF, false);
     const int lds_bytes = SH::LDS_BYTES + (keys ? RP_BYTE_TAB_BYTES : 0);
     static_assert(SH::LDS_BYTES % 16 == 0 && SH::LDS_BYTES + RP_BYTE_TAB_BYTES <= 160 * 1024, "the byte table fits behind the weights");
+    const bool tabs = a.tabs != nullptr;
+    if (tabs) {
+        static DeviceOnce attr_set_tabs;
+        if (int rc = lds_limit(&attr_set_tabs, {reinterpret_cast<const void *>(&layer_fused_kernel_rp<4, 2, false, true, true>)}, "layer_fused_kernel_rp tabs", lds_bytes)) return rc;
+    }
     if (keys) {
         const void *fn = prof_on ? reinterpret_cast<const void *>(&layer_fused_kernel_rp<4, 2, true, true>) : reinterpret_cast<const void *>(&layer_fused_kernel_rp<4, 2, false, true>);
         static DeviceOnce attr_set_keys;
@@ -769,7 +859,8 @@
         static DeviceOnce attr_set;
         if (int rc = lds_limit(&attr_set, {fn}, "layer_fused_kernel_rp")) return rc;
     }
-    trace("gsn chain: layer_fused_kernel_rp<4,2>%s nodes %d edges %d grid %lld ranges %d\n", keys ? " keys" : "", a.n_nodes, a.n_edges, (long long)gx, a.n_ranges);
+    trace("gsn chain: layer_fused_kernel_rp<4,2>%s nodes %d edges %d grid %lld ranges %d%s\n", keys ? " keys" : "", a.n_nodes, a.n_edges, (long long)gx, a.n_ranges,
+          tabs && !prof_on ? " x_i tables" : "");
     if (prof_on) {
         ProfCounters prof(32 + 2 * (size_t)a.n_ranges, st);
         if (keys) hipLaunchKernelGGL((layer_fused_kernel_rp<4, 2, true, true>), dim3((unsigned)gx), dim3(64 * RR_NW), lds_bytes, st, a, prof.ptr());
@@ -799,6 +890,8 @@
                 fprintf(stderr, "rpprof range %s: blocks %llu tiles %llu total %llu cycles | per block: top %.0f edge %.0f | per tile: exposed edge epilogue %.0f stage0 %.0f split %.0f stage1 %.0f\n",
                         w ? "mid" : "0", o[6], o[7], o[8], o[0] / nb, o[1] / nb, o[2] / nt, o[3] / nt, o[4] / nt, o[5] / nt);
             }
+    } else if (tabs) {
+        hipLaunchKernelGGL((layer_fused_kernel_rp<4, 2, false, true, true>), dim3((unsigned)gx), dim3(64 * RR_NW), lds_bytes, st, a, (unsigned long long *)nullptr);
     } else if (keys) {
         hipLaunchKernelGGL((layer_fused_kernel_rp<4, 2, false, true>), dim3((unsigned)gx), dim3(64 * RR_NW), lds_bytes, st, a, (unsigned long long *)nullptr);
     } else {
@@ -825,6 +918,18 @@
     return launch_check("pack16_rows_kernel");
 }
 
+extern "C" int64_t gsn_layer_key_tables_words(void) { return RP_TAB_WORDS; }
+extern "C" int64_t gsn_layer_key_tables_max_rows(void) { return RP_TAB_ROWS; }
+extern "C" int gsn_layer_key_tables_hip(const void *prepared, const uint16_t *node_dict, int64_t dict_rows, float *tabs, void *stream) {
+    if (!prepared || !node_dict || !tabs || ((reinterpret_cast<uintptr_t>(prepared) | reinterpret_cast<uintptr_t>(node_dict)) & 15) || (reinterpret_cast<uintptr_t>(tabs) & 3))
+        return set_error(GSN_E_INVALID, "gsn_layer_key_tables_hip: null / misaligned prepared buffer, node dictionary or tables");
+    if (dict_rows < 1 || dict_rows > RP_TAB_ROWS)
+        return set_error(GSN_E_UNSUPPORTED, "gsn_layer_key_tables_hip: node dictionary of %lld rows (1 .. %d)", (long long)dict_rows, RP_TAB_ROWS);
+    hipLaunchKernelGGL(rp_key_tables_kernel, dim3(1), dim3(128), 0, reinterpret_cast<hipStream_t>(stream), reinterpret_cast<const unsigned *>(prepared), node_dict,
+                       (int)dict_rows, tabs);
+    return launch_check("rp_key_tables_kernel");
+}
+
 extern "C" int gsn_layer_keys_byte_table(uint16_t *dst) {
     if (!dst) return set_error(GSN_E_INVALID, "gsn_layer_keys_byte_table: dst is null");
     for (unsigned b = 0; b < 256; ++b)
diff --git a/gsn_amd/csrc/layer_rr.h b/gsn_amd/csrc/layer_rr.h
--- a/gsn_amd/csrc/layer_rr.h
+++ b/gsn_amd/csrc/layer_rr.h
@@ -26,6 +26,7 @@
     const uint16_t *node_dict;
     int64_t dict_rows;
     int edge_col0;
+    const float *tabs = nullptr;
 };
 
 }
diff --git a/gsn_amd/csrc/switches.h b/gsn_amd/csrc/switches.h
--- a/gsn_amd/csrc/switches.h
+++ b/gsn_amd/csrc/switches.h
@@ -30,6 +30,7 @@
     X(FUSED_W, ONCE, "int, default 1: 0 refuses layer_fused_kernel_w")                                                                     \
     X(FUSED_G, ONCE, "int, default 1: 0 refuses layer_fused_kernel_g")                                                                     \
     X(RP_OLD_SHARE, ONCE, "float, default 0.6: share of the grid that layer_fused_kernel_rp gives to its first range")                     \
+    X(RP_TABLES, LIVE, "on/off, default on: 0 keeps layer_fused_kernel_rp on its KEYS arm where the step hands it x_i tables")             \
                                                                                                                         \
     X(LINEAR_SPLITK_RANGES, ONCE, "int, default -1 (automatic): forced split-k range count of the small bf16x6 linear, 0 = never")         \
     X(LINEAR_SMALL_MAX, ONCE, "int, default 96: most 128-row tiles that still take the 32-row-tile kernel, 0 = never")                     \
diff --git a/gsn_amd/step.py b/gsn_amd/step.py
--- a/gsn_amd/step.py
+++ b/gsn_amd/step.py
@@ -1,6 +1,7 @@
 from __future__ import annotations
 
 import ctypes
+import os
 
 import numpy as np
 import torch
@@ -32,6 +33,23 @@
 
 def keys_path_ok(n_classes, clamp):
     return int(np.prod(node_key_radices(n_classes, clamp), dtype=np.int64)) <= 256
+
+
+TABLE_ROWS = 31
+
+
+def tables_path_ok(n_classes, clamp):
+    return keys_path_ok(n_classes, clamp) and int(np.prod(node_key_radices(n_classes, clamp), dtype=np.int64)) <= TABLE_ROWS
+
+
+def _tables_switch():
+    v = os.environ.get("GSN_RP_TABLES")
+    if v is None:
+        return True
+    try:
+        return int(v) != 0
+    except ValueError:
+        return False
 
 
 _NODE_DICTS = {}
@@ -88,6 +106,7 @@
         self._keys = _abi.gsn_count_keys()
         self._force_packs = bool(force_packs)
         self.on_keys = False
+        self.on_tables = False
         self._dict = None
         self._bound = None
 
@@ -129,7 +148,8 @@
                 raise ValueError("CountLayerStep: activation %r is outside the one-launch layer kernel" % st.act)
             if st.bn is not None and (st.bn.training or st.bn.running_mean is None):
                 raise RuntimeError("CountLayerStep: a BatchNorm1d in train mode / without running statistics")
-        key = (tuple(_dense._prep_key(st) for st in stages), d_x, getattr(layer, "_fold_gen", 0), N, E, self.on_keys, 0 if self._dict is None else self._dict.data_ptr())
+        key = (tuple(_dense._prep_key(st) for st in stages), d_x, getattr(layer, "_fold_gen", 0), N, E, self.on_keys, 0 if self._dict is None else self._dict.data_ptr(),
+               self.on_tables)
         if self._lay is not None and self._lay[0] == key:
             return self._lay[1]
         for st in stages:
@@ -150,10 +170,16 @@
         if not L.gsn_layer_fused_pack16_supported(ctypes.byref(ge), d_x, ctypes.byref(g0), ctypes.byref(g1)):
             raise ValueError("CountLayerStep: shape outside the packed-row layer kernel (every stage 128 wide, d_x + 4 <= 32, <= 16 edge-level columns)")
         prep = _dense._prepared("_pack16", ge, g0, g1, d_x, dev)
+        tabs = None
+        if self.on_tables:
+            tabs = torch.empty(int(L.gsn_layer_key_tables_words()), dtype=torch.float32, device=dev)
+            with _abi.device_guard(dev):
+                _abi.check(L.gsn_layer_key_tables_hip(prep.data_ptr(), self._dict.data_ptr(), self._dict.shape[0], tabs.data_ptr(), _abi.current_stream()),
+                           "gsn_layer_key_tables_hip")
         d_out = node_stages[1].weight.shape[0]
         flops = 2.0 * E * edge_stages[0].weight.shape[1] * edge_stages[0].weight.shape[0]
         flops += 2.0 * N * (node_stages[0].weight.shape[1] * node_stages[0].weight.shape[0] + node_stages[1].weight.shape[1] * d_out)
-        val = (ge, g0, g1, prep, keep, d_out, flops)
+        val = (ge, g0, g1, prep, keep, d_out, flops, tabs)
         self._lay = (key, val)
         self._bound = None
         return val
@@ -174,9 +200,10 @@
                              "<= 8 edge code classes)" % (d_x, w_ids, w_ef))
         keys = not self._force_packs and keys_path_ok(x_codes.n_classes, x_codes.clamp)
         self.on_keys = keys
+        self.on_tables = keys and tables_path_ok(x_codes.n_classes, x_codes.clamp) and _tables_switch()
         self._dict = node_dictionary(x_codes.n_classes, x_codes.clamp, dev) if keys else None
         b = self._buffers(N, E, G, dev, keys)
-        ge, g0, g1, prep, _keep, d_out, flops = self._layer_structs(b, N, E, d_x, w_ids + w_ef)
+        ge, g0, g1, prep, _keep, d_out, flops, tabs = self._layer_structs(b, N, E, d_x, w_ids + w_ef)
         if ids_out is None:
             ids_out = torch.empty((E, self.plan.n_cols), dtype=torch.int64, device=dev)
         y = out if out is not None else torch.empty((N, d_out), dtype=torch.float32, device=dev)
@@ -216,10 +243,11 @@
         L = _abi.lib()
         if keys:
             kref, dptr, drows = ctypes.byref(self._keys), self._dict.data_ptr(), self._dict.shape[0]
-            entry = "gsn_count_layer_step_keys_hip"
+            entry = "gsn_count_layer_step_tabs_hip"
+            tptr = tabs.data_ptr() if tabs is not None else None
 
             def call(ev_between):
-                return L.gsn_count_layer_step_keys_hip(ctypes.byref(c), ctypes.byref(l), kref, dptr, drows, ev_between, _abi.current_stream())
+                return L.gsn_count_layer_step_tabs_hip(ctypes.byref(c), ctypes.byref(l), kref, dptr, drows, tptr, ev_between, _abi.current_stream())
         else:
             entry = "gsn_count_layer_step_hip"
 
diff --git a/include/gsn_abi.h b/include/gsn_abi.h
--- a/include/gsn_abi.h
+++ b/include/gsn_abi.h
@@ -262,6 +262,11 @@
 int gsn_layer_keys_byte_table(uint16_t *dst);
 int gsn_count_layer_step_keys_hip(const gsn_count_call *count, const gsn_layer_pack16_call *layer, const gsn_count_keys *keys,
                                   const uint16_t *node_dict, int64_t dict_rows, void *event_between, void *stream);
+int64_t gsn_layer_key_tables_words(void);
+int64_t gsn_layer_key_tables_max_rows(void);
+int gsn_layer_key_tables_hip(const void *prepared, const uint16_t *node_dict, int64_t dict_rows, float *tabs, void *stream);
+int gsn_count_layer_step_tabs_hip(const gsn_count_call *count, const gsn_layer_pack16_call *layer, const gsn_count_keys *keys,
+                                  const uint16_t *node_dict, int64_t dict_rows, const float *tabs, void *event_between, void *stream);
 
 int64_t gsn_linear_f16x3_kpad(int64_t k_total);
 int64_t gsn_linear_f16x3_mpad(int64_t m_rows);
```

Measured after the change: 136.5 million graphs/s, median of 6. 1.02x the previous value.
